# hkust-vgd/scanobjectnn

Hardware: AMD Instinct MI355X
Metric: point-clouds/sec fwd+bwd at B×2048×3, 15-cls (higher is better)
Workload: dtype f32

## Files before the change

### include/pcops.h

```cpp
#ifndef PCOPS_H
#define PCOPS_H

#ifdef __cplusplus
extern "C" {
#endif

typedef void *pcops_stream_t;

typedef struct pcops_rows {
    const void *blocks;
    const int *block_start;
    const int *rows;
} pcops_rows_t;

typedef enum pcops_status {
    PCOPS_OK = 0,
    PCOPS_ERR_NULL_POINTER = -1,
    PCOPS_ERR_BAD_SHAPE = -2,
    PCOPS_ERR_BAD_ARGUMENT = -3,
    PCOPS_ERR_UNSUPPORTED = -4,
    PCOPS_ERR_LAUNCH = -5
} pcops_status;

const char *pcops_strerror(int status);
// ... 230 lines not shown
int pcops_cloud_bias_rows(long long rows);
int pcops_cloud_bias_fwd(long long rows, int rows_per_group, int c, const float *Q, const float *Ctr, float *Y,
                         float *stats_partial, const float *stat_pivot, pcops_stream_t stream);
int pcops_cloud_bias_bwd(long long rows, int rows_per_group, int c, const float *G, const float *Y, const float *p, const float *q,
                         const float *t, float *dQ, float *dCtr, float *partial, pcops_stream_t stream);
int pcops_edge_first_rows(void);
int pcops_edge_first_supported(int b, int n, int m, int s, int c);
int pcops_edge_first_moments(int b, int n, int m, int s, const float *xyz, const int *idx, float *moments_partial,
                             float *edge_rows, pcops_stream_t stream);
int pcops_edge_first_wgrad(int b, int n, int m, int s, int c, const float *G, const float *xyz, const int *idx,
                           float *wpartial, pcops_stream_t stream);
int pcops_mlp_bwd_fused_edge_groups(long long M, int K, int N, int S, int gram);
int pcops_mlp_bwd_fused_edge(long long M, int K, int N, const float *Yprev, const float *a_scale, const float *a_shift,
                                  const float *Y, const float *p, const float *q, const float *t, const float *gpool,
                                  const unsigned char *argmax, int S, const float *W, float *partial, float *dW, float *db,
                                  float *stats_partial, const float *edge_rows, float *edge_stats, pcops_stream_t stream);

int pcops_mlp_bwd_fused_gw_groups(long long M, int K, int N, int S);
int pcops_mlp_bwd_fused_gw(long long M, int K, int N, const float *Yprev, const float *a_scale, const float *a_shift,
                           const float *Y, const float *p, const float *q, const float *t, const float *gpool,
                           const unsigned char *argmax, int S, const float *W, const float *bias, float *partial, float *dW,
                           float *db, float *Gprev, float *stats_partial, pcops_stream_t stream);
int pcops_mlp_bwd_fused_edge_gw(long long M, int K, int N, const float *Yprev, const float *a_scale, const float *a_shift,
                                const float *Y, const float *p, const float *q, const float *t, const float *gpool,
                                const unsigned char *argmax, int S, const float *W, const float *bias, float *partial,
                                float *dW, float *db, float *stats_partial, const float *edge_rows, float *edge_stats,
                                pcops_stream_t stream);
int pcops_edge_first_layer_grads(int P1, const float *wpartial, int P2, const float *moments_partial, int c, const float *W,
                                 const float *bias, const float *p, const float *q, const float *t, const float *sumG,
                                 const float *mean, long long rows, float *dW, float *dbias, pcops_stream_t stream);
int pcops_xyz_first_layer_grads(int P1, const float *xyz_stats, int P2, const float *moments, int C,
                                const float *Wxyz, const float *bias, const float *p, const float *q, const float *t,
                                const float *sumG, const float *mean, long long rows, float *dWxyz, float *dbias,
                                pcops_stream_t stream);

int pcops_adam_step(long long n, float *p, const float *g, float *m, float *v, float beta1, float beta2, float lr_t,
                    float epsilon, pcops_stream_t stream);
int pcops_gather_stack_rows_supported(int b, int n, int m, int s, int has_q, int nlayers, const int *widths);
int pcops_sa_scatter_rows_supported(int n, int m, int s, int c);
unsigned long long pcops_rows_max_blocks(int b, int m, int s);
int pcops_rows_plan(int b, int m, int s, const int *pts_cnt, void *blocks, int *block_start, int *rows,
                    pcops_stream_t stream);
int pcops_mlp_gemm_fwd_rows(int M, int K, int N, const float *X, int ldx, const float *pro_scale,
                            const float *pro_shift, const float *W, const float *bias, float *Y,
                            float *stats_partial, const float *stat_pivot, const pcops_rows_t *rows,
                            pcops_stream_t stream);
int pcops_mlp_gemm_fwd_xyz_rows(int M, int K, int N, const float *off4, const float *xyzw, const float *pro_scale,
                                const float *pro_shift, const float *W, const float *bias, float *Y,
                                float *stats_partial, const float *stat_pivot, const pcops_rows_t *rows,
                                pcops_stream_t stream);
int pcops_mlp_gemm_dgrad_rows(int M, int K, int Nout, const float *G, const float *Y, const float *p,
                              const float *q, const float *t, const float *gpool, const unsigned char *argmax,
                              int S, const float *pool_scale, const float *pool_shift, const float *Wt,
                              const float *Yprev, const float *prev_scale, const float *prev_shift, float *Gprev,
                              float *stats_partial, const pcops_rows_t *rows, pcops_stream_t stream);
int pcops_mlp_gemm_dgrad_xyz_rows(int M, int K, int Nout, const float *G, const float *Y, const float *p,
                                  const float *q, const float *t, const float *gpool, const unsigned char *argmax,
                                  int S, const float *pool_scale, const float *pool_shift, const float *Wt,
                                  const float *off4, const float *xyzw, const float *prev_scale,
                                  const float *prev_shift, float *Gprev, float *stats_partial, float *xyz_stats,
                                  const pcops_rows_t *rows, pcops_stream_t stream);
int pcops_mlp_wgrad_rows(long long M, int K, int N, const float *X, int ldx, const float *a_scale,
                         const float *a_shift, const float *G, const float *Y, const float *p, const float *q,
                         const float *t, const float *gpool, const unsigned char *argmax, int S,
                         const float *pool_scale, const float *pool_shift, float *partial, float *dW, float *db,
                         const pcops_rows_t *rows, pcops_stream_t stream);
int pcops_mlp_wgrad_xyz_rows(long long M, int K, int N, const float *off4, const float *xyzw, const float *a_scale,
                             const float *a_shift, const float *G, const float *Y, const float *p, const float *q,
                             const float *t, const float *gpool, const unsigned char *argmax, int S,
                             const float *pool_scale, const float *pool_shift, float *partial, float *dW, float *db,
                             const pcops_rows_t *rows, pcops_stream_t stream);
int pcops_mlp_gemm_fwd_pool_rows_supported(int M, int K, int N);
int pcops_mlp_gemm_fwd_pool_rows(int M, int K, int N, const float *X, int ldx, const float *pro_scale,
                                 const float *pro_shift, const float *W, const float *bias, const float *gamma,
                                 float *Y, float *stats_partial, const float *stat_pivot, float *ypart,
                                 unsigned char *ppart, const pcops_rows_t *rows, pcops_stream_t stream);
int pcops_mlp_pool_combine_rows(long long G, int C, const float *ypart, const unsigned char *ppart,
                                const float *gamma, const float *scale, const float *shift,
                                const pcops_rows_t *rows, float *out, unsigned char *argmax, float *ysel,
                                pcops_stream_t stream);
int pcops_mlp_bn_relu_maxpool_rows(long long G, int C, const float *Y, const float *scale, const float *shift,
                                   const pcops_rows_t *rows, float *out, unsigned char *argmax, float *ysel,
                                   pcops_stream_t stream);
int pcops_sa_gather_fwd_rows(int b, int n, int m, int s, int c, const float *Q, const float *Ctr, const float *xyz,
                             const float *new_xyz, const float *Wxyz, const float *bias, const int *idx, float *Y,
                             float *off4, float *stats_partial, const float *stat_pivot, float *moments,
                             const pcops_rows_t *rows, pcops_stream_t stream);
int pcops_sa_scatter_bwd_rows(int b, int n, int m, int s, int c, const float *G, const float *Y, const float *p,
                              const float *q, const float *t, const float *gpool, const unsigned char *argmax,
                              const float *pool_scale, const float *pool_shift, const int *idx, const float *xyz,
                              const float *new_xyz, float *dQ, float *dCtr, float *wpartial, float *dWxyz,
                              float *dbias, const float *fwd_Q, const float *fwd_Ctr, const float *fwd_Wxyz,
                              const float *fwd_bias, void *workspace, const pcops_rows_t *rows,
                              pcops_stream_t stream);

int pcops_edge_ld_supported(int b, int n, int m, int s, int c);
int pcops_edge_pool_fwd_ld(int b, int n, int m, int s, int c, const float *Q, int ldq, const float *Ctr, int ldc,
                           const int *idx, const float *gamma, float *SQ, float *qsel, unsigned char *arg,
                           float *stats_partial, const float *stat_pivot, pcops_stream_t stream);
int pcops_edge_pool_out_ld(long long groups, int c, const float *qsel, const float *Ctr, int ldc, const float *scale,
                           const float *shift, float *out, float *ysel, pcops_stream_t stream);
int pcops_edge_pool_out_ld2(long long groups, int c, const float *qsel, const float *Ctr, int ldc, const float *scale,
                            const float *shift, float *out, float *ysel, float *out2, int ld2, pcops_stream_t stream);
int pcops_edge_pool_bwd_ld(int b, int n, int m, int s, int c, const float *Q, int ldq, const float *Ctr, int ldc,
                           const int *idx, const float *gpool, const float *ysel, const float *SQ,
                           const unsigned char *arg, const float *scale, const float *shift, const float *p,
                           const float *q, const float *t, float *dQ, int lddq, float *dCtr, int lddc, void *workspace,
                           pcops_stream_t stream);
int pcops_sa_gather_fwd_ld(int b, int n, int m, int s, int c, const float *Q, int ldq, const float *Ctr, int ldc,
                           const int *idx, float *Y, float *stats_partial, const float *stat_pivot,
                           pcops_stream_t stream);
int pcops_sa_scatter_bwd_ld(int b, int n, int m, int s, int c, const float *G, const float *p, const float *q,
                            const float *t, const int *idx, const float *Q, int ldq, const float *Ctr, int ldc,
                            float *dQ, int lddq, float *dCtr, int lddc, void *workspace, pcops_stream_t stream);

int pcops_edge_weights_fwd(int c, int cp, int kp, const float *W1, const float *b1, float *Wcat, float *bcat,
                           pcops_stream_t stream);
int pcops_edge_weights_bwd(int c, int cp, const float *dWcat, const float *dbcat, float *dW1, float *db1,
                           pcops_stream_t stream);

int pcops_fc_bn_fwd(int R, int C, const float *x, const float *gamma, const float *beta, float *moving_mean,
                    float *moving_var, int training, float decay, float eps, int unbiased_moving_var, int relu,
                    float *y, float *save_mean, float *save_rstd, pcops_stream_t stream);
int pcops_fc_bn_bwd(int R, int C, const float *dy, const float *x, const float *y, const float *gamma,
                    const float *save_mean, const float *save_rstd, int training, int relu, float *dx,
                    float *dgamma, float *dbeta, pcops_stream_t stream);

int pcops_softmax_ce_blocks(int R);
int pcops_softmax_ce(int R, int C, const float *logits, const int *labels, float label_smoothing, float *loss,
                     float *dlogits, pcops_stream_t stream);
int pcops_three_nn_weights(int b, int n, const float *dist, float *weight, pcops_stream_t stream);

int pcops_transform3_fwd(int b, int n, const float *x, const float *T, float *out, pcops_stream_t stream);
int pcops_transform3_bwd(int b, int n, const float *x, const float *T, const float *grad_out, float *dT, float *dx,
                         pcops_stream_t stream);

int pcops_spider_taylor_fwd(long long rows, int t, const float *delta, const float *theta, const float *tbias, float *g,
                            pcops_stream_t stream);
unsigned long long pcops_spider_taylor_bwd_workspace_bytes(long long rows, int t);
int pcops_spider_taylor_bwd(long long rows, int t, const float *delta, const float *dg, float *dtheta, float *dtbias,
                            void *workspace, pcops_stream_t stream);
int pcops_spider_conv_fwd(int b, int n, int c, int k, int t, int o, const float *feat, const int *idx, const float *g,
                          const float *w, const float *bias, float *y, pcops_stream_t stream);
unsigned long long pcops_spider_conv_wgrad_workspace_bytes(int b, int n, int c, int k, int t, int o);
int pcops_spider_conv_wgrad(int b, int n, int c, int k, int t, int o, const float *feat, const int *idx, const float *g,
                            const float *dy, float *dw, float *dbias, void *workspace, pcops_stream_t stream);
int pcops_spider_conv_dgrad(int b, int n, int c, int k, int t, int o, const float *feat, const int *idx, const float *g,
                            const float *w, const float *dy, float *dfeat_grouped, float *dg, pcops_stream_t stream);

unsigned long long pcops_group_norm_relu_workspace_bytes(int b, int c);
int pcops_group_norm_relu_fwd(int b, int n, int c, int groups, float eps, const float *x, const float *gamma,
                              const float *beta, float *y, float *mean, float *rstd, pcops_stream_t stream);
int pcops_group_norm_relu_bwd(int b, int n, int c, int groups, const float *dout, const float *x, const float *y,
                              const float *gamma, const float *mean, const float *rstd, float *dx, float *dgamma,
                              float *dbeta, void *workspace, pcops_stream_t stream);

#ifdef __cplusplus
}
#endif
#endif
```

### scanobjectnn_amd/_lib.py

```python
import ctypes as C
import os
import weakref

import torch

_HERE = os.path.dirname(os.path.abspath(__file__))
LIB_PATH = os.environ.get("PCOPS_LIB") or os.path.join(_HERE, "libpcops.so")

_I, _F, _P, _U64, _LL = C.c_int, C.c_float, C.c_void_p, C.c_ulonglong, C.c_longlong
ABI_VERSION = 4

SIGNATURES = {
    "pcops_farthest_point_sample": ([_I, _I, _I, _P, _P, _P], True),
    "pcops_prob_sample": ([_I, _I, _I, _P, _P, _P, _P], True),
    "pcops_gather_point": ([_I, _I, _I, _P, _P, _P], True),
    "pcops_gather_point_grad": ([_I, _I, _I, _P, _P, _P], True),
    "pcops_query_ball_point": ([_I, _I, _I, _F, _I, _P, _P, _P, _P], True),
    "pcops_query_ball_point_multi": ([_I, _I, _I, _I, _P, _P, _P, _P, _P, _P], True),
    "pcops_group_point": ([_I, _I, _I, _I, _I, _P, _P, _P], True),
    "pcops_group_point_grad": ([_I, _I, _I, _I, _I, _P, _P, _P], True),
    "pcops_selection_sort": ([_I, _I, _I, _I, _P, _P, _P], True),
    "pcops_three_nn": ([_I, _I, _I, _P, _P, _P, _P], True),
    "pcops_three_interpolate": ([_I, _I, _I, _I, _P, _P, _P, _P], True),
    "pcops_three_interpolate_grad": ([_I, _I, _I, _I, _P, _P, _P, _P], True),
    "pcops_pairwise_distance": ([_I, _I, _I, _P, _P], True),
    "pcops_knn_topk": ([_I, _I, _I, _P, _P], True),
    "pcops_knn_graph": ([_I, _I, _I, _I, _P, _P], True),
    "pcops_knn_graph_seeded": ([_I, _I, _I, _I, _P, _P, _P], True),
    "pcops_edge_feature": ([_I, _I, _I, _I, _P, _P, _P], True),
    "pcops_edge_feature_grad": ([_I, _I, _I, _I, _P, _P, _P], True),
    "pcops_mlp_gemm_fwd": ([_I, _I, _I, _P, _I, _P, _P, _P, _P, _P, _P, _P], True),
    "pcops_mlp_bn_finalize": ([_I, _I, _LL, _P, _P, _P, _P, _P, _F, _F, _I, _P, _P, _P, _P, _P, _P], True),
    "pcops_mlp_bn_eval_coeffs": ([_I, _P, _P, _P, _P, _F, _P, _P], True),
    "pcops_mlp_bn_relu_maxpool": ([_LL, _I, _I, _P, _P, _P, _P, _P, _P], True),
    "pcops_mlp_gemm_fwd_pool": ([_I, _I, _I, _I, _P, _I, _P, _P, _P, _P, _P, _P, _P, _P, _P, _P], True),
    "pcops_mlp_pool_select": ([_LL, _I, _P, _P, _P, _P], True),
    "pcops_mlp_bn_relu_apply": ([_LL, _I, _P, _P, _P, _P], True),
    "pcops_mlp_relu_mask_stats": ([_LL, _I, _P, _P, _P, _P, _P, _P], True),
    "pcops_mlp_pool_bwd_stats": ([_LL, _I, _P, _P, _P, _P, _P, _P], True),
    "pcops_mlp_pool_bwd_stats_sum": ([_LL, _I, _P, _LL, _P, _LL, _P, _P, _P, _P, _P], True),
    "pcops_mlp_bn_bwd_coeffs": ([_I, _I, _LL, _P, _P, _P, _P, _P, _P, _P, _P, _P, _P], True),
    "pcops_mlp_gemm_dgrad": ([_I, _I, _I, _P, _P, _P, _P, _P, _P, _P, _I, _P, _P, _P, _P, _P, _P, _P, _P], True),
    "pcops_mlp_wgrad": ([_LL, _I, _I, _P, _I, _P, _P, _P, _P, _P, _P, _P, _P, _P, _I, _P, _P, _P, _P, _P], True),
    "pcops_mlp_transpose": ([_I, _I, _P, _P], True),
    "pcops_small_gemm": ([_I, _I, _I, _P, _I, _P, _I, _P, _I], True),
    "pcops_small_gemm_ex": ([_I, _I, _I, _P, _I, _I, _P, _I, _I, _P, _P, _I], True),
    "pcops_mlp_dy_apply": ([_LL, _I] + [_P] * 6, True),
    "pcops_small_gemm_colsum": ([_I, _I, _I, _P, _I, _I, _P, _I, _I, _P, _P, _I, _P], True),
    "pcops_small_gemm_pair": ([_P], True),
    "pcops_mlp_pool_top_prep": ([_I, _I] + [_P] * 8, True),
    "pcops_mlp_pool_top_finish": ([_I, _I, _LL] + [_P] * 10, True),
    "pcops_mlp_pool_top_addend": ([_I, _I, _I, _I] + [_P] * 9, True),
    "pcops_mlp_gemm_dgrad_top": ([_I, _I] + [_P] * 6 + [_LL] + [_P] * 3, True),
    "pcops_mlp_gram": ([_LL, _I, _P, _I, _P, _P, _P, _P, _P], True),
    "pcops_mlp_pool_top_wsparse": ([_I, _I, _I, _I] + [_P] * 11, True),
    "pcops_sa_gather_fwd": ([_I, _I, _I, _I, _I, _P, _P, _P, _P, _P, _P, _P, _P, _P, _P, _P, _P], True),
    "pcops_mlp_gemm_fwd_xyz": ([_I, _I, _I, _P, _P, _P, _P, _P, _P, _P, _P, _P], True),
    "pcops_mlp_gemm_dgrad_xyz": ([_I, _I, _I, _P, _P, _P, _P, _P, _P, _P, _I, _P, _P, _P, _P, _P, _P, _P, _P, _P, _P], True),
    "pcops_mlp_wgrad_xyz": ([_LL, _I, _I, _P, _P, _P, _P, _P, _P, _P, _P, _P, _P, _P, _I, _P, _P, _P, _P, _P], True),
    "pcops_edge_pool_fwd": ([_I, _I, _I, _I, _I, _P, _P, _P, _P, _P, _P, _P, _P, _P], True),
    "pcops_edge_pool_out": ([_LL, _I, _P, _P, _P, _P, _P, _P], True),
    "pcops_edge_pool_bwd": ([_I, _I, _I, _I, _I] + [_P] * 15, True),
    "pcops_xyz_first_layer_grads": ([_I, _P, _I, _P, _I, _P, _P, _P, _P, _P, _P, _P, _LL, _P, _P], True),
    "pcops_cloud_bias_fwd": ([_LL, _I, _I, _P, _P, _P, _P, _P], True),
    "pcops_cloud_bias_bwd": ([_LL, _I, _I, _P, _P, _P, _P, _P, _P, _P, _P], True),
    "pcops_edge_first_moments": ([_I, _I, _I, _I, _P, _P, _P, _P], True),
    "pcops_mlp_bwd_fused_edge": ([_LL, _I, _I, _P, _P, _P, _P, _P, _P, _P, _P, _P, _I, _P, _P, _P, _P, _P, _P, _P], True),
    "pcops_edge_first_wgrad": ([_I, _I, _I, _I, _I, _P, _P, _P, _P], True),
    "pcops_edge_first_layer_grads": ([_I, _P, _I, _P, _I, _P, _P, _P, _P, _P, _P, _P, _LL, _P, _P], True),
    "pcops_sa_scatter_bwd": ([_I, _I, _I, _I, _I] + [_P] * 22, True),
    "pcops_rows_plan": ([_I, _I, _I, _P, _P, _P, _P], True),
    "pcops_mlp_gemm_fwd_rows": ([_I, _I, _I, _P, _I, _P, _P, _P, _P, _P, _P, _P, _P], True),
    "pcops_mlp_gemm_fwd_xyz_rows": ([_I, _I, _I, _P, _P, _P, _P, _P, _P, _P, _P, _P, _P], True),
    "pcops_mlp_gemm_dgrad_rows": ([_I, _I, _I, _P, _P, _P, _P, _P, _P, _P, _I, _P, _P, _P, _P, _P, _P, _P, _P, _P], True),
    "pcops_mlp_gemm_dgrad_xyz_rows": ([_I, _I, _I, _P, _P, _P, _P, _P, _P, _P, _I, _P, _P, _P, _P, _P, _P, _P, _P, _P, _P, _P], True),
    "pcops_mlp_bwd_fused": ([_LL, _I, _I, _P, _P, _P, _P, _P, _P, _P, _P, _P, _P, _I, _P, _P, _P, _P, _P, _P], True),
    "pcops_mlp_bwd_fused_rows": ([_LL, _I, _I, _P, _P, _P, _P, _P, _P, _P, _P, _P, _P, _I, _P, _P, _P, _P, _P, _P, _P], True),
    "pcops_adam_step": ([_LL, _P, _P, _P, _P, _F, _F, _F, _F], True),
    "pcops_mlp_bwd_fused_gw": ([_LL, _I, _I] + [_P] * 9 + [_I] + [_P] * 7, True),
    "pcops_mlp_bwd_fused_edge_gw": ([_LL, _I, _I] + [_P] * 9 + [_I] + [_P] * 8, True),
    "pcops_mlp_bwd_fused_xyz_rows": ([_LL, _I, _I, _P, _P, _P, _P, _P, _P, _P, _P, _P, _P, _P, _I, _P, _P, _P, _P, _P, _P, _P], True),
    "pcops_mlp_wgrad_rows": ([_LL, _I, _I, _P, _I, _P, _P, _P, _P, _P, _P, _P, _P, _P, _I, _P, _P, _P, _P, _P, _P], True),
    "pcops_mlp_wgrad_xyz_rows": ([_LL, _I, _I, _P, _P, _P, _P, _P, _P, _P, _P, _P, _P, _P, _I, _P, _P, _P, _P, _P, _P], True),
    "pcops_mlp_bn_relu_maxpool_rows": ([_LL, _I, _P, _P, _P, _P, _P, _P, _P], True),
    "pcops_mlp_gemm_fwd_pool_rows": ([_I, _I, _I, _P, _I, _P, _P, _P, _P, _P, _P, _P, _P, _P, _P, _P], True),
    "pcops_mlp_pool_combine_rows": ([_LL, _I, _P, _P, _P, _P, _P, _P, _P, _P, _P], True),
    "pcops_sa_gather_fwd_rows": ([_I, _I, _I, _I, _I, _P, _P, _P, _P, _P, _P, _P, _P, _P, _P, _P, _P, _P], True),
    "pcops_sa_scatter_bwd_rows": ([_I, _I, _I, _I, _I] + [_P] * 23, True),
    "pcops_knn_point": ([_I, _I, _I, _I, _I, _P, _P, _P, _P], True),
    "pcops_knn_point_dist": ([_I, _I, _I, _I, _P, _P, _P], True),
    "pcops_scatter_rows_sorted": ([_I, _I, _I, _I, _I, _I, _P, _P, _P, _P, _I, _P], True),
    "pcops_edge_feature_grad_central": ([_I, _I, _I, _I, _P, _P], True),
    "pcops_edge_pool_fwd_ld": ([_I, _I, _I, _I, _I, _P, _I, _P, _I, _P, _P, _P, _P, _P, _P, _P], True),
    "pcops_edge_pool_out_ld": ([_LL, _I, _P, _P, _I, _P, _P, _P, _P], True),
    "pcops_edge_pool_out_ld2": ([_LL, _I, _P, _P, _I, _P, _P, _P, _P, _P, _I], True),
    "pcops_edge_pool_bwd_ld": ([_I, _I, _I, _I, _I, _P, _I, _P, _I] + [_P] * 10 + [_P, _I, _P, _I, _P], True),
    "pcops_sa_gather_fwd_ld": ([_I, _I, _I, _I, _I, _P, _I, _P, _I, _P, _P, _P, _P], True),
    "pcops_sa_scatter_bwd_ld": ([_I, _I, _I, _I, _I, _P, _P, _P, _P, _P, _P, _I, _P, _I, _P, _I, _P, _I, _P], True),
    "pcops_edge_weights_fwd": ([_I, _I, _I, _P, _P, _P, _P], True),
    "pcops_edge_weights_bwd": ([_I, _I, _P, _P, _P, _P], True),
    "pcops_transform3_fwd": ([_I, _I, _P, _P, _P], True),
    "pcops_transform3_bwd": ([_I, _I, _P, _P, _P, _P, _P], True),
    "pcops_fc_bn_fwd": ([_I, _I, _P, _P, _P, _P, _P, _I, _F, _F, _I, _I, _P, _P, _P], True),
    "pcops_fc_bn_bwd": ([_I, _I, _P, _P, _P, _P, _P, _P, _I, _I, _P, _P, _P], True),
    "pcops_softmax_ce": ([_I, _I, _P, _P, _F, _P, _P], True),
    "pcops_three_nn_weights": ([_I, _I, _P, _P], True),
    "pcops_spider_taylor_fwd": ([_LL, _I, _P, _P, _P, _P], True),
    "pcops_spider_taylor_bwd": ([_LL, _I, _P, _P, _P, _P, _P], True),
    "pcops_spider_conv_fwd": ([_I] * 6 + [_P] * 6, True),
    "pcops_spider_conv_wgrad": ([_I] * 6 + [_P] * 7, True),
    "pcops_spider_conv_dgrad": ([_I] * 6 + [_P] * 7, True),
    "pcops_group_norm_relu_fwd": ([_I, _I, _I, _I, _F] + [_P] * 6, True),
    "pcops_group_norm_relu_bwd": ([_I, _I, _I, _I] + [_P] * 10, True),
}
PLAIN = {
    "pcops_strerror": ([_I], C.c_char_p),
    "pcops_abi_version": ([], _I),
    "pcops_softmax_ce_blocks": ([_I], _I),
    "pcops_farthest_point_sample_workspace_bytes": ([_I, _I], _U64),
    "pcops_mlp_stats_rows": ([_I], _I),
    "pcops_mlp_reduce_workspace_bytes": ([_I], _U64),
    "pcops_mlp_gemm_fwd_pool_supported": ([_I, _I, _I, _I], _I),
    "pcops_mlp_xyz_supported": ([_I, _I, _I], _I),
    "pcops_mlp_bwd_stats_rows": ([_LL], _I),
    "pcops_mlp_bwd_pool_stats_rows": ([_LL], _I),
    "pcops_mlp_wgrad_splits": ([_LL, _I, _I], _I),
    "pcops_mlp_bwd_fused_groups": ([_LL, _I, _I, _I, _I], _I),
    "pcops_mlp_bwd_fused_gw_groups": ([_LL, _I, _I, _I], _I),
    "pcops_mlp_bwd_fused_edge_groups": ([_LL, _I, _I, _I, _I], _I),
    "pcops_gather_stack_rows_supported": ([_I, _I, _I, _I, _I, _I, _P], _I),
    "pcops_sa_scatter_rows_supported": ([_I, _I, _I, _I], _I),
    "pcops_sa_gather_stats_rows": ([_LL], _I),
    "pcops_sa_gather_fwd_stats_rows": ([_I] * 9, _I),
    "pcops_sa_scatter_rows": ([_I, _I], _I),
    "pcops_edge_pool_stats_rows": ([_LL], _I),
    "pcops_edge_pool_fwd_stats_rows": ([_I] * 5, _I),
    "pcops_edge_ld_supported": ([_I] * 5, _I),
    "pcops_edge_first_rows": ([], _I),
    "pcops_cloud_bias_supported": ([_LL, _I, _I], _I),
    "pcops_cloud_bias_rows": ([_LL], _I),
    "pcops_edge_first_supported": ([_I] * 5, _I),
    "pcops_sa_scatter_workspace_bytes": ([_I, _I, _I, _I], _U64),
    "pcops_rows_max_blocks": ([_I, _I, _I], _U64),
    "pcops_mlp_gemm_fwd_pool_rows_supported": ([_I, _I, _I], _I),
    "pcops_scatter_rows_workspace_bytes": ([_I, _I, _I], _U64),
    "pcops_knn_point_supported": ([_I], _I),
    "pcops_scatter_rows_sorted_max_ndst": ([], _I),
    "pcops_scatter_rows_sorted_supported": ([_I, _I], _I),
    "pcops_mlp_pool_top_supported": ([_I, _I, _I, _I], _I),
    "pcops_knn_graph_path": ([_I, _I, _I, _I, _P], _I),
    "pcops_last_launch_pipe": ([], _I),
    "pcops_last_launch_plan": ([_P, _I], _I),
    "pcops_set_option": ([_I, _I], _I),
    "pcops_get_option": ([_I], _I),
    "pcops_set_deterministic": ([_I], None),
    "pcops_get_deterministic": ([], _I),
    "pcops_spider_taylor_bwd_workspace_bytes": ([_LL, _I], _U64),
    "pcops_spider_conv_wgrad_workspace_bytes": ([_I] * 6, _U64),
    "pcops_group_norm_relu_workspace_bytes": ([_I, _I], _U64),
}


class GemmProblem(C.Structure):
    _fields_ = [("M", C.c_int), ("K", C.c_int), ("N", C.c_int), ("A", C.c_void_p), ("lda", C.c_int), ("transA", C.c_int),
                ("B", C.c_void_p), ("ldb", C.c_int), ("transB", C.c_int), ("bias", C.c_void_p), ("C", C.c_void_p),
                ("ldc", C.c_int), ("colsum", C.c_void_p)]


def small_gemm_pair(p0, p1):
    arr = (GemmProblem * 2)(GemmProblem(*p0), GemmProblem(*p1))
    lib = load()
    stream = torch.cuda.current_stream().cuda_stream
    shape = tuple(int(v) for v in p0[:3]) + tuple(int(v) for v in p1[:3])
    for h in _hooks:
        h("pcops_small_gemm_pair", "pre", shape)
    status = lib.pcops_small_gemm_pair(arr, stream)
    for h in _hooks:
        h("pcops_small_gemm_pair", "post", shape)
    if status != 0:
        raise PcopsError("pcops_small_gemm_pair failed: %s (status %d)" % (strerror(status), status))


class RowsT(C.Structure):
    _fields_ = [("blocks", C.c_void_p), ("block_start", C.c_void_p), ("rows", C.c_void_p)]


class Rows:
    by_struct = weakref.WeakValueDictionary()

    def __init__(self, pts_cnt, nsample):
        b, m = pts_cnt.shape
        lib = load()
        nb = int(lib.pcops_rows_max_blocks(b, m, int(nsample)))
        dev = pts_cnt.device
        self.blocks = torch.empty((nb, 4), dtype=torch.int32, device=dev)
        self.block_start = torch.empty(b * m + 1, dtype=torch.int32, device=dev)
        self.rows = torch.empty(1, dtype=torch.int32, device=dev)
        call("pcops_rows_plan", b, m, int(nsample), pts_cnt.data_ptr(), self.blocks.data_ptr(),
             self.block_start.data_ptr(), self.rows.data_ptr())
        self.struct = RowsT(self.blocks.data_ptr(), self.block_start.data_ptr(), self.rows.data_ptr())
        self.full_rows = b * m * int(nsample)
        Rows.by_struct[id(self.struct)] = self

    def num_rows(self):
        return int(self.rows.item())

    @property
    def ref(self):
        return C.byref(self.struct)


_lib = None


class PcopsError(RuntimeError):
    pass


def load():
    global _lib
    if _lib is not None:
        return _lib
    if not os.path.exists(LIB_PATH):
        raise PcopsError(
            "libpcops.so is missing (%s). Build it with `python -c 'import __graft_entry__ as g; "
            "g.build()'` or `make -C scanobjectnn_amd/csrc`. There is no CPU fallback." % LIB_PATH)
    lib = C.CDLL(LIB_PATH)
    for name, (argtypes, _) in SIGNATURES.items():
        fn = getattr(lib, name)
        fn.argtypes = list(argtypes) + [_P]
        fn.restype = _I
    for name, (argtypes, restype) in PLAIN.items():
# ... 99 lines not shown
```

### scanobjectnn_amd/csrc/mlp.hip

```cpp
#include <stdlib.h>

#include "common.h"
#include <type_traits>

#ifndef PCOPS_MLP_PART
#define PCOPS_MLP_PART (-1)
#endif
#define PCOPS_PART(p_) (PCOPS_MLP_PART < 0 || PCOPS_MLP_PART == (p_))
#define PCOPS_HIDDEN __attribute__((visibility("hidden")))

#ifndef PCOPS_BF_RM
#define PCOPS_BF_RM 1
#endif

namespace pcops_mlp {

typedef float f32x16 __attribute__((ext_vector_type(16)));
typedef float f32x4 __attribute__((ext_vector_type(4)));
typedef __bf16 bf16x8 __attribute__((ext_vector_type(8)));

typedef __bf16 bf16x2 __attribute__((ext_vector_type(2)));
typedef float f32x2 __attribute__((ext_vector_type(2)));
__device__ __forceinline__ void split3_pair(float a, float b, bf16x2 &h, bf16x2 &m, bf16x2 &l) {
    const f32x2 v = {a, b};
// ... 960 lines not shown
#pragma unroll 1
            for (int it = 0; it < nit; it += 2) {
                a1 = *reinterpret_cast<const float4 *>(arow + 8 * (it + 1));
#pragma unroll
                for (int nt = 0; nt < NT; ++nt) b1[nt] = bq[(2 * (it + 1)) * BN + 32 * nt];
                mfma16(a0, b0);
                const int nx = it + 2 < nit ? it + 2 : it + 1;
                a0 = *reinterpret_cast<const float4 *>(arow + 8 * nx);
#pragma unroll
                for (int nt = 0; nt < NT; ++nt) b0[nt] = bq[(2 * nx) * BN + 32 * nt];
                mfma16(a1, b1);
            }
            __builtin_amdgcn_fence(__ATOMIC_ACQUIRE, "wavefront");
            }
#ifdef PCOPS_PHASE_PROF
            {
                float sink_ = acc[NT - 1][15];
                asm volatile("" ::"v"(sink_));
                const unsigned long long n_ = PROF_T(); pf_mfma += n_ - pf_t; pf_t = n_;
            }
#endif
            }
            if (WST) {
                wstore((wt + 1) & 1);
                __syncthreads();
                ++wt;
            }
        }
        if (active) {
        if constexpr (BF3) {
#pragma unroll
            for (int i = 0; i < NT; ++i) acc[i] += sm[i];
        }
        if (POOL) pool_acc(acc, tile, sub, st);
        const long long row0 = tile * 32;
        const int erem = (int)((long long)M - row0 < 32 ? (long long)M - row0 : 32);
        const __amdgpu_buffer_rsrc_t rout = make_rsrc(a.Y + row0 * a.ldy, ((long long)M - row0) * a.ldy * 4);
        const bool ynt = a.nt_out != 0;
        const __amdgpu_buffer_rsrc_t rprev =
            make_rsrc(((EM == E_MASK || EM == E_MASKA) ? a.Yprev : a.Y) + row0 * a.ldy, ((long long)M - row0) * a.ldy * 4);
        auto epilogue = [&](auto full_) {
        constexpr bool FULL = decltype(full_)::value;
#pragma unroll
        for (int h = 0; h < EH; ++h) {
            const int ocq = h * BNH + ocl;
            const bool ocin = FULL || (n0 + ocq < N);
            const unsigned yvoff = ocin ? (unsigned)((lane / O4) * a.ldy + n0 + ocq) * 4u : kOOB;
            float4 py[is_mask(EM) ? NST : 1];
            float4 po[(EM == E_MASKX) ? NST : 1];
            if (EM == E_MASKX) {
                const __amdgpu_buffer_rsrc_t ro = make_rsrc(a.off4 + row0 * 4, ((long long)M - row0) * 16);
                const float4 xw0 = *reinterpret_cast<const float4 *>(&ecoef[2 * BN + ocq]);
                const float4 xw1 = *reinterpret_cast<const float4 *>(&ecoef[3 * BN + ocq]);
                const float4 xw2 = *reinterpret_cast<const float4 *>(&ecoef[4 * BN + ocq]);
                const float4 xb = *reinterpret_cast<const float4 *>(&ecoef[5 * BN + ocq]);
#pragma unroll
                for (int j = 0; j < NST; ++j) {
                    const float4 o = buf_load4(ro, (unsigned)(lane / O4) * 16u, (unsigned)j * (64 / O4) * 16u);
                    po[j] = o;
                    py[j] = make_float4(xyz_y(o, xw0.x, xw1.x, xw2.x, xb.x), xyz_y(o, xw0.y, xw1.y, xw2.y, xb.y),
                                        xyz_y(o, xw0.z, xw1.z, xw2.z, xb.z), xyz_y(o, xw0.w, xw1.w, xw2.w, xb.w));
                }
            }
            if (EM == E_MASK || EM == E_MASKA) {
#pragma unroll
                for (int j = 0; j < NST; ++j) py[j] = buf_load4(rprev, yvoff, (unsigned)j * yrowstep);
            }
            float4 pad[has_add(EM) ? NST : 1];
            if (has_add(EM)) {
                const __amdgpu_buffer_rsrc_t radd = make_rsrc(a.addend, a.add_bytes);
#pragma unroll
                for (int j = 0; j < NST; ++j) {
                    const int rr = (lane + 64 * j) / O4;
                    const int slot = (FULL || rr < erem) ? a.rowmap[row0 + rr] : -1;
                    const unsigned off = (slot >= 0 && ocin) ? ((unsigned)slot * (unsigned)a.add_ld + (unsigned)(n0 + ocq)) * 4u : kOOB;
                    pad[j] = buf_load4(radd, off, 0u);
                }
            }
            const float4 eb = *reinterpret_cast<const float4 *>(&ecoef[ocq]);
            const float4 em = *reinterpret_cast<const float4 *>(&ecoef[BN + ocq]);
            const float4 epv = EM == E_FWD ? *reinterpret_cast<const float4 *>(&ecoef[2 * BN + ocq])
                                           : make_float4(0.f, 0.f, 0.f, 0.f);
            float ew[2] = {1.f, 1.f};
            if (EM == E_FWD && compact) {
                const int nblk = (M + kBlk - 1) / kBlk;
#pragma unroll
                for (int hb = 0; hb < 2; ++hb) {
                    long long bi = tile * 2 + hb;
                    bi = bi < nblk ? bi : nblk - 1;
                    const RowBlock rb = uniform_block(a.blocks, bi);
                    ew[hb] = rb.w;
                }
            }
            __builtin_amdgcn_wave_barrier();
#pragma unroll
            for (int nt = 0; nt < NTH; ++nt)
#pragma unroll
                for (int v = 0; v < 16; ++v)
                    Aw[((v & 3) + 8 * (v >> 2) + 4 * (lane >> 5)) * LDW + 32 * nt + (lane & 31)] = acc[h * NTH + nt][v];
            __builtin_amdgcn_fence(__ATOMIC_RELEASE, "wavefront");
            __builtin_amdgcn_wave_barrier();
#pragma unroll
            for (int j = 0; j < NST; ++j) {
                if (FULL && j % 2 == 0) __builtin_amdgcn_sched_barrier(0);
                const int r = (lane + 64 * j) / O4;
                float4 o = *reinterpret_cast<const float4 *>(&Aw[r * LDW + ocl]);
                if (FULL || (r < erem && ocin)) {
                    if (EM == E_FWD) {
                        if (compact && j % (O4 / 4) == 0) {
                            const float w = lane < O4 ? ew[j / (O4 / 4)] : 1.f;
                            const float4 wo = make_float4(w * o.x, w * o.y, w * o.z, w * o.w);
                            s1[h][0] += wo.x; s1[h][1] += wo.y; s1[h][2] += wo.z; s1[h][3] += wo.w;
                            s2[h][0] = fmaf(wo.x, o.x, s2[h][0]); s2[h][1] = fmaf(wo.y, o.y, s2[h][1]);
                            s2[h][2] = fmaf(wo.z, o.z, s2[h][2]); s2[h][3] = fmaf(wo.w, o.w, s2[h][3]);
                        } else {
                        s1[h][0] += o.x; s1[h][1] += o.y; s1[h][2] += o.z; s1[h][3] += o.w;
                        s2[h][0] = fmaf(o.x, o.x, s2[h][0]); s2[h][1] = fmaf(o.y, o.y, s2[h][1]);
                        s2[h][2] = fmaf(o.z, o.z, s2[h][2]); s2[h][3] = fmaf(o.w, o.w, s2[h][3]);
                        }
                        if (POOL) {
                            o.x = fmaf(o.x, em.x, epv.x); o.y = fmaf(o.y, em.y, epv.y);
                            o.z = fmaf(o.z, em.z, epv.z); o.w = fmaf(o.w, em.w, epv.w);
                        } else {
                            o.x += epv.x; o.y += epv.y; o.z += epv.z; o.w += epv.w;
                        }
                    } else if (EM == E_PLAINA) {
                        const float4 vc = *reinterpret_cast<const float4 *>(&ecoef[2 * BN + ocq]);
                        o.x += pad[j].x + vc.x; o.y += pad[j].y + vc.y; o.z += pad[j].z + vc.z; o.w += pad[j].w + vc.w;
                    } else if (is_mask(EM)) {
                        const float4 yp = py[j];
                        if (EM == E_MASKA) {
                            const float4 vc = *reinterpret_cast<const float4 *>(&ecoef[2 * BN + ocq]);
                            o.x += pad[j].x + vc.x; o.y += pad[j].y + vc.y; o.z += pad[j].z + vc.z; o.w += pad[j].w + vc.w;
                        }
                        o.x = fmaf(yp.x, eb.x, em.x) > 0.f ? o.x : 0.f;
                        o.y = fmaf(yp.y, eb.y, em.y) > 0.f ? o.y : 0.f;
                        o.z = fmaf(yp.z, eb.z, em.z) > 0.f ? o.z : 0.f;
                        o.w = fmaf(yp.w, eb.w, em.w) > 0.f ? o.w : 0.f;
                        s1[h][0] += o.x; s1[h][1] += o.y; s1[h][2] += o.z; s1[h][3] += o.w;
                        s2[h][0] = fmaf(o.x, yp.x, s2[h][0]); s2[h][1] = fmaf(o.y, yp.y, s2[h][1]);
                        s2[h][2] = fmaf(o.z, yp.z, s2[h][2]); s2[h][3] = fmaf(o.w, yp.w, s2[h][3]);
                        if (EM == E_MASKX) {
                            const float4 of = po[j];
                            const float ov[4] = {o.x, o.y, o.z, o.w};
#pragma unroll
                            for (int e = 0; e < 4; ++e) {
                                sx[h][0][e] = fmaf(of.x, ov[e], sx[h][0][e]);
                                sx[h][1][e] = fmaf(of.y, ov[e], sx[h][1][e]);
                                sx[h][2][e] = fmaf(of.z, ov[e], sx[h][2][e]);
                            }
                        }
                    }
                }
                if ((EM != E_MASKX && !(EM == E_FWD && POOL)) || a.Y)
                    buf_store4(rout, yvoff, (unsigned)j * yrowstep, o, ynt);
            }
            __builtin_amdgcn_fence(__ATOMIC_ACQUIRE, "wavefront");
        }
        };
        if (EM != E_MASKX && erem == 32 && n0 + BN <= N) epilogue(std::true_type{});
        else epilogue(std::false_type{});
        }
#ifdef PCOPS_PHASE_PROF
        if (active) { const unsigned long long n_ = PROF_T(); pf_epi += n_ - pf_t; ++pf_tiles; }
#endif
        st = nst;
        sub = nsub;
        ++round;
    }
#ifdef PCOPS_PHASE_PROF
    if (lane == 0) {
        atomicAdd(&g_phase_prof[0], pf_stage);
        atomicAdd(&g_phase_prof[1], pf_mfma);
        atomicAdd(&g_phase_prof[2], pf_epi);
        atomicAdd(&g_phase_prof[3], PROF_T() - pf_start);
        atomicAdd(&g_phase_prof[4], pf_tiles);
        atomicAdd(&g_phase_prof[5], 1ull);
    }
#endif

    if (EM != E_PLAIN && EM != E_PLAINA && a.stats) {
#pragma unroll
        for (int h = 0; h < EH; ++h) {
#pragma unroll
            for (int e = 0; e < 4; ++e) {
#pragma unroll
                for (int off = 32; off >= O4; off >>= 1) {
                    s1[h][e] += __shfl_xor(s1[h][e], off, 64);
                    s2[h][e] += __shfl_xor(s2[h][e], off, 64);
                }
            }
            if (lane < O4) {
#pragma unroll
                for (int e = 0; e < 4; ++e) {
                    red[(wave * 2 + 0) * BN + h * BNH + ocl + e] = POOL ? s1[h][e] * ecoef[BN + h * BNH + ocl + e] : s1[h][e];
                    red[(wave * 2 + 1) * BN + h * BNH + ocl + e] = s2[h][e];
                }
            }
        }
        __syncthreads();
        for (int i = tid; i < 2 * BN; i += NTHR) {
            const int which = i / BN, c = i % BN;
            if (n0 + c < N) {
                float v = 0.f;
#pragma unroll
                for (int w = 0; w < WAVES; ++w) v += red[(w * 2 + which) * BN + c];
                a.stats[((long long)rowgrp * 2 + which) * N + n0 + c] = v;
            }
        }
    }
    if (EM == E_MASKX && a.xstats) {
#pragma unroll
        for (int i = 0; i < 3; ++i) {
            __syncthreads();
#pragma unroll
            for (int h = 0; h < EH; ++h) {
// ... 2318 lines not shown
        } else if constexpr (DW3) {
#pragma unroll
            for (int y = 0; y < TN; ++y) {
                const int sn = (cn * TN + y) * 32 + li, nn = 4 * (sn % D4) + sn / D4;
#pragma unroll
                for (int v = 0; v < 16; ++v) {
                    const int sk = ck * 32 + (v & 3) + 8 * (v >> 2) + 4 * half, kk = 4 * (sk % A4) + sk / A4;
                    if (kk < K && nn < N) out[(long long)kk * N + nn] = accw[y][v] + smw[y][v];
                }
            }
        } else {
#pragma unroll
        for (int y = 0; y < TN; ++y) {
            const int nn = (cn * TN + y) * 32 + li;
#pragma unroll
            for (int v = 0; v < 16; ++v) {
                const int kk = ck * 32 + (v & 3) + 8 * (v >> 2) + 4 * half;
                if (kk < K && nn < N) out[(long long)kk * N + nn] = accw[y][v];
            }
        }
        }
#pragma unroll
        for (int b = 0; b < 2; ++b) {
            s1[b] += __shfl_xor(s1[b], 16, 64); s1[b] += __shfl_xor(s1[b], 32, 64);
            s2[b] += __shfl_xor(s2[b], 16, 64); s2[b] += __shfl_xor(s2[b], 32, 64);
        }
#pragma unroll
        for (int b = 0; b < (NX ? 2 : 1); ++b)
#pragma unroll
            for (int i = 0; i < NX; ++i) {
                sx[b][i] += __shfl_xor(sx[b][i], 16, 64);
                sx[b][i] += __shfl_xor(sx[b][i], 32, 64);
            }
        __syncthreads();
        constexpr int NSR = 2 + (NX > 3 ? NX : 3);
        float *sst = buf + 256 * 4;
        if (lane < 16) {
#pragma unroll
            for (int b = 0; b < 2; ++b) {
                sst[(rh * NSR + 0) * KB + 32 * cbp + 16 * b + c16] = s1[b];
                sst[(rh * NSR + 1) * KB + 32 * cbp + 16 * b + c16] = s2[b];
                if (NX) {
#pragma unroll
                    for (int i = 0; i < NX; ++i) sst[(rh * NSR + 2 + i) * KB + 32 * cbp + 16 * b + c16] = sx[b][i];
                }
            }
        }
        if (a.dbpart) {
            const float *sdb = buf;
            for (int c = tid; c < NB; c += 256) {
                const int quad = c >> 2, e = c & 3;
                float sum = 0.f;
                for (int r = quad; r < 256; r += D4) sum += sdb[r * 4 + e];
                if (c < N) a.dbpart[(long long)grp * N + c] = sum;
            }
        }
        if constexpr (GW) {
            const float *sxs = buf + 2048;
            for (int c = tid; c < KB; c += 256) {
                const int quad = c >> 2, e = c & 3;
                float sum = 0.f;
                for (int r = quad; r < 256; r += A4) sum += sxs[r * 4 + e];
                if (c < K) a.xsum_part[(long long)grp * K + c] = sum;
            }
        }
        __syncthreads();
        for (int i = tid; i < (2 + NX) * KB; i += 256) {
            const int which = i / KB, c = i % KB;
            const float v = sst[which * KB + c] + sst[(NSR + which) * KB + c];
            if (c < K) {
                if (which < 2) a.gstats[((long long)grp * 2 + which) * K + c] = v;
                else a.xstats[((long long)grp * NX + which - 2) * K + c] = v;
            }
        }
    }
}

struct GramArgs {
    long long M;
    int K, ldx;
    const float *X, *asc, *ash;
    float *part;
    float *xpart;
};

constexpr int gram_blocks(int nbk) { return nbk * (nbk + 1) / 2; }
constexpr int gram_row_of(int u, int nbk) {
    int i = 0, left = u;
    while (left >= nbk - i) { left -= nbk - i; ++i; }
    return i;
}
constexpr int gram_col_of(int u, int nbk) {
    int i = 0, left = u;
    while (left >= nbk - i) { left -= nbk - i; ++i; }
    return i + left;
}

template <int U, int NBK>
struct GramBlk {
    static constexpr int i = gram_row_of(U, NBK), j = gram_col_of(U, NBK);
};
template <int NBK, int U0, typename AccT, int... B>
__device__ __forceinline__ void gram_mfma_step(AccT &acc, const float (&f)[NBK], std::integer_sequence<int, B...>) {
    ((acc[B] = __builtin_amdgcn_mfma_f32_32x32x2f32(f[GramBlk<U0 + B, NBK>::i], f[GramBlk<U0 + B, NBK>::j], acc[B], 0, 0, 0)), ...);
}
template <int NBK, int U0, typename AccT, int... B>
__device__ __forceinline__ void gram_store(const AccT &acc, float *out, int K, int half, int li,
                                           std::integer_sequence<int, B...>) {
    auto one = [&](auto b_) {
        constexpr int b = decltype(b_)::value;
        constexpr int bi = GramBlk<U0 + b, NBK>::i, bj = GramBlk<U0 + b, NBK>::j;
        const int nn = 32 * bj + li;
#pragma unroll
        for (int v = 0; v < 16; ++v) {
            const int kk = 32 * bi + (v & 3) + 8 * (v >> 2) + 4 * half;
            if (kk < K && nn < K) out[(long long)kk * K + nn] = acc[b][v];
        }
    };
    (one(std::integral_constant<int, B>{}), ...);
}

template <int NBK, bool BNRELU>
__global__ __launch_bounds__(512, 1) void gram_full_kernel(GramArgs a) {
    constexpr int KP = 32 * NBK, RS = 32, LD = KP + 4;
    constexpr int NU = gram_blocks(NBK), PER = (NU + 3) / 4;
    constexpr int K4 = KP / 4, NV = RS * K4 / 256;
    extern __shared__ __attribute__((aligned(16))) float lds[];
    const int tid = threadIdx.x, lane = tid & 63;
    const int wave = __builtin_amdgcn_readfirstlane(tid >> 6);
    const int K = a.K;
    const long long M = a.M;
    const int grp = blockIdx.x, ngrp = gridDim.x;
    float *coef = lds;
    float *buf = coef + 2 * KP;
    for (int e = tid; e < KP; e += 512) {
        coef[e] = (BNRELU && e < K) ? a.asc[e] : 0.f;
        coef[KP + e] = (BNRELU && e < K) ? a.ash[e] : 0.f;
    }
    __syncthreads();
    const long long nstripes = (M + RS - 1) / RS;
    const long long cnt = grp < nstripes ? (nstripes - grp + ngrp - 1) / ngrp : 0;

    if (wave >= 4) {
        const int pt = tid - 256;
        float4 px[NV];
        float cs[NV][4];
#pragma unroll
        for (int j = 0; j < NV; ++j) cs[j][0] = cs[j][1] = cs[j][2] = cs[j][3] = 0.f;
        auto issue = [&](long long stripe) {
            const long long row0 = stripe * RS;
            const __amdgpu_buffer_rsrc_t rx = make_rsrc(a.X + row0 * a.ldx, (M - row0) * a.ldx * 4);
#pragma unroll
            for (int j = 0; j < NV; ++j) {
                const int e = pt + 256 * j, r = e / K4, c = (e % K4) * 4;
                px[j] = buf_load4(rx, c < K ? (unsigned)(r * a.ldx + c) * 4u : kOOB, 0u);
            }
        };
        auto stage = [&](long long stripe, float *dst) {
            const long long row0 = stripe * RS;
#pragma unroll
            for (int j = 0; j < NV; ++j) {
                const int e = pt + 256 * j, r = e / K4, c = (e % K4) * 4;
                float4 x = px[j];
                if (BNRELU) {
                    const float4 sc = *reinterpret_cast<const float4 *>(&coef[c]);
                    const float4 sh = *reinterpret_cast<const float4 *>(&coef[KP + c]);
                    x.x = fmaxf(fmaf(x.x, sc.x, sh.x), 0.f); x.y = fmaxf(fmaf(x.y, sc.y, sh.y), 0.f);
                    x.z = fmaxf(fmaf(x.z, sc.z, sh.z), 0.f); x.w = fmaxf(fmaf(x.w, sc.w, sh.w), 0.f);
                    if (!(c < K && row0 + r < M)) x = make_float4(0.f, 0.f, 0.f, 0.f);
                }
                cs[j][0] += x.x; cs[j][1] += x.y; cs[j][2] += x.z; cs[j][3] += x.w;
                *reinterpret_cast<float4 *>(&dst[r * LD + c]) = x;
            }
        };
        if (cnt > 0) {
            issue(grp);
            stage(grp, buf);
            if (cnt > 1) issue(grp + ngrp);
        }
        __syncthreads();
        for (long long i = 0; i < cnt; ++i) {
            if (i + 1 < cnt) {
                stage(grp + (i + 1) * ngrp, buf + ((i + 1) & 1) * RS * LD);
                if (i + 2 < cnt) issue(grp + (i + 2) * ngrp);
            }
            __syncthreads();
        }
        float *scr = buf;
#pragma unroll
        for (int j = 0; j < NV; ++j)
            *reinterpret_cast<float4 *>(&scr[(pt + 256 * j) * 4]) = make_float4(cs[j][0], cs[j][1], cs[j][2], cs[j][3]);
        __syncthreads();
        for (int e = pt; e < K; e += 256) {
            float sum = 0.f;
            for (int idx = e >> 2; idx < 256 * NV; idx += K4) sum += scr[idx * 4 + (e & 3)];
            a.xpart[(long long)grp * K + e] = sum;
        }
        __syncthreads();
    } else {
        const int half = lane >> 5, li = lane & 31;
        auto run = [&](auto wv_) {
            constexpr int WV = decltype(wv_)::value;
            constexpr int U0 = WV * PER, U1 = (U0 + PER < NU) ? U0 + PER : NU;
            constexpr int NB_ = U1 > U0 ? U1 - U0 : 0;
            f32x16 acc[NB_ > 0 ? NB_ : 1];
#pragma unroll
            for (int b = 0; b < NB_; ++b)
#pragma unroll
                for (int v = 0; v < 16; ++v) acc[b][v] = 0.f;
            __syncthreads();
            for (long long i = 0; i < cnt; ++i) {
                const float *sb = buf + (i & 1) * RS * LD + half * LD + li;
                float fn[NBK];
#pragma unroll
                for (int c = 0; c < NBK; ++c) fn[c] = sb[32 * c];
#pragma unroll
                for (int it = 0; it < RS / 2; ++it) {
                    float f[NBK];
#pragma unroll
                    for (int c = 0; c < NBK; ++c) f[c] = fn[c];
                    if (it + 1 < RS / 2) {
#pragma unroll
                        for (int c = 0; c < NBK; ++c) fn[c] = sb[2 * (it + 1) * LD + 32 * c];
                    }
                    __builtin_amdgcn_sched_barrier(0);
                    gram_mfma_step<NBK, U0>(acc, f, std::make_integer_sequence<int, NB_>{});
                    __builtin_amdgcn_sched_barrier(0);
                }
                __syncthreads();
            }
            gram_store<NBK, U0>(acc, a.part + (long long)grp * K * K, K, half, li, std::make_integer_sequence<int, NB_>{});
            __syncthreads();
            __syncthreads();
        };
        if (wave == 0) run(std::integral_constant<int, 0>{});
        else if (wave == 1) run(std::integral_constant<int, 1>{});
        else if (wave == 2) run(std::integral_constant<int, 2>{});
        else run(std::integral_constant<int, 3>{});
    }
}

static __global__ __launch_bounds__(256) void mirror_lower_kernel(int K, float *__restrict__ g) {
    const int i = blockIdx.x, tid = threadIdx.x;
    for (int j = tid; j < i; j += 256) g[(long long)i * K + j] = g[(long long)j * K + i];
}

static bool gram_full_on() {
    static const bool on = [] {
        const char *e = getenv("PCOPS_GRAM_FULL");
        return !(e && e[0] == '0');
    }();
    return on;
}

// ... 488 lines not shown
            const int k = (i * 16 + q) * 4;
            if (i < kq && k < Kp) *reinterpret_cast<float4 *>(dst + k) = acc[i];
        }
    }
}

__global__ __launch_bounds__(256) void pool_top_wsparse_kernel(long long G, int S, int C, int Kp,
                                                               const float *__restrict__ gout,
                                                               const float *__restrict__ ysel,
                                                               const unsigned char *__restrict__ arg,
                                                               const float *__restrict__ sc, const float *__restrict__ sh,
                                                               const float *__restrict__ p,
                                                               const float *__restrict__ Yprev,
                                                               const float *__restrict__ psc, const float *__restrict__ psh,
                                                               float *__restrict__ Ssp, float *__restrict__ cfsum) {
    constexpr int KR = 8, U = 8;
    __shared__ float red[4][64 * KR + 1];
    const int lane = threadIdx.x & 63, wave = threadIdx.x >> 6;
    const int c = blockIdx.x;
    const float scc = sc[c], shc = sh[c], pc = p[c];
    const int kr = (Kp + 63) / 64;
    float asc[KR], ash[KR], acc[KR];
#pragma unroll
    for (int i = 0; i < KR; ++i) {
        const int k = lane + 64 * i;
        asc[i] = (k < Kp && psc) ? psc[k] : 1.f;
        ash[i] = (k < Kp && psc) ? psh[k] : 0.f;
        acc[i] = 0.f;
    }
    float csum = 0.f;
    const long long gq = (G + 3) / 4;
    const long long gend = (wave + 1) * gq < G ? (wave + 1) * gq : G;
    for (long long g0 = wave * gq; g0 < gend; g0 += 64) {
        const long long g = g0 + lane;
        float cf = 0.f;
        int row = 0;
        if (g < gend) {
            const long long e = g * C + c;
            cf = fmaf(ysel[e], scc, shc) > 0.f ? pc * gout[e] : 0.f;
            row = arg[e];
        }
        unsigned long long hits = __ballot(cf != 0.f);
        while (hits) {
            float w[U];
            long long r[U];
#pragma unroll
            for (int u = 0; u < U; ++u) {
                w[u] = 0.f;
                r[u] = 0;
                if (hits) {
                    const int l = __builtin_ctzll(hits);
                    hits &= hits - 1;
                    w[u] = __builtin_bit_cast(float, __builtin_amdgcn_readlane(__builtin_bit_cast(int, cf), l));
                    r[u] = (g0 + l) * S + __builtin_amdgcn_readlane(row, l);
                }
            }
#pragma unroll
            for (int i = 0; i < KR; ++i) {
                if (i >= kr) break;
                const int k = lane + 64 * i;
                float x[U];
#pragma unroll
                for (int u = 0; u < U; ++u) x[u] = (k < Kp) ? Yprev[r[u] * Kp + k] : 0.f;
#pragma unroll
                for (int u = 0; u < U; ++u) {
                    const float xv = psc ? fmaxf(fmaf(x[u], asc[i], ash[i]), 0.f) : x[u];
                    acc[i] = fmaf(w[u], xv, acc[i]);
                }
            }
#pragma unroll
            for (int u = 0; u < U; ++u) csum += w[u];
        }
    }
#pragma unroll
    for (int i = 0; i < KR; ++i) red[wave][lane + 64 * i] = acc[i];
    if (lane == 0) red[wave][64 * KR] = csum;
    __syncthreads();
    for (int k = threadIdx.x; k < Kp; k += 256)
        Ssp[(long long)k * C + c] = (red[0][k] + red[1][k]) + (red[2][k] + red[3][k]);
    if (threadIdx.x == 0)
        cfsum[c] = (red[0][64 * KR] + red[1][64 * KR]) + (red[2][64 * KR] + red[3][64 * KR]);
}

__device__ __forceinline__ void small_gemm_tile(int bx, int by, int M, int K, int N, const float *__restrict__ A, int lda,
                                                         const float *__restrict__ B, int ldb, float *__restrict__ C,
                                                         int ldc, int transA, int transB, const float *__restrict__ bias,
                                                         float *__restrict__ colsum) {
    __shared__ float As[4][32][17], Bs[4][16][33], red[4][32][33], cs[4][2][32];
    const int tid = threadIdx.x, lane = tid & 63, wave = tid >> 6;
    const int m0 = by * 32, n0 = bx * 32;
    const int kchunks = (K + 15) / 16;
    f32x16 acc;
#pragma unroll
    for (int v = 0; v < 16; ++v) acc[v] = 0.f;
    float ra[8], rb[8];
    auto fetch = [&](int ch) {
        const int k0 = ch * 16;
#pragma unroll
        for (int i = 0; i < 8; ++i) {
            const int e = lane + 64 * i;
            const int r = e >> 4, kk = e & 15;
            const long long ia = transA ? (long long)(k0 + kk) * lda + m0 + r : (long long)(m0 + r) * lda + k0 + kk;
            ra[i] = (ch < kchunks && m0 + r < M && k0 + kk < K) ? A[ia] : 0.f;
            const int kb = e >> 5, c = e & 31;
            const long long ib = transB ? (long long)(n0 + c) * ldb + k0 + kb : (long long)(k0 + kb) * ldb + n0 + c;
            rb[i] = (ch < kchunks && k0 + kb < K && n0 + c < N) ? B[ib] : 0.f;
        }
    };
    fetch(wave);
    const bool sums = colsum != nullptr && by == 0;
    float bsum = 0.f;
    for (int ch = wave; ch < kchunks; ch += 4) {
        __builtin_amdgcn_wave_barrier();
#pragma unroll
        for (int i = 0; i < 8; ++i) {
            const int e = lane + 64 * i;
            As[wave][e >> 4][e & 15] = ra[i];
            Bs[wave][e >> 5][e & 31] = rb[i];
        }
        if (sums) {
#pragma unroll
            for (int i = 0; i < 8; ++i) bsum += rb[i];
        }
        __builtin_amdgcn_fence(__ATOMIC_RELEASE, "wavefront");
        __builtin_amdgcn_wave_barrier();
        fetch(ch + 4);
#pragma unroll
        for (int st = 0; st < 8; ++st)
            acc = __builtin_amdgcn_mfma_f32_32x32x2f32(As[wave][lane & 31][2 * st + (lane >> 5)],
                                                       Bs[wave][2 * st + (lane >> 5)][lane & 31], acc, 0, 0, 0);
        __builtin_amdgcn_fence(__ATOMIC_ACQUIRE, "wavefront");
    }
#pragma unroll
    for (int v = 0; v < 16; ++v) red[wave][(v & 3) + 8 * (v >> 2) + 4 * (lane >> 5)][lane & 31] = acc[v];
    cs[wave][lane >> 5][lane & 31] = bsum;
    __syncthreads();
    if (sums && tid < 32 && n0 + tid < N)
        colsum[n0 + tid] = ((cs[0][0][tid] + cs[0][1][tid]) + (cs[1][0][tid] + cs[1][1][tid])) +
                           ((cs[2][0][tid] + cs[2][1][tid]) + (cs[3][0][tid] + cs[3][1][tid]));
    for (int e = tid; e < 32 * 32; e += 256) {
        const int r = e >> 5, c = e & 31;
        if (m0 + r < M && n0 + c < N)
            C[(long long)(m0 + r) * ldc + n0 + c] =
                ((red[0][r][c] + red[1][r][c]) + (red[2][r][c] + red[3][r][c])) + (bias ? bias[n0 + c] : 0.f);
    }
}

__global__ __launch_bounds__(256) void small_gemm_kernel(int M, int K, int N, const float *__restrict__ A, int lda,
                                                         const float *__restrict__ B, int ldb, float *__restrict__ C,
                                                         int ldc, int transA, int transB, const float *__restrict__ bias,
                                                         float *__restrict__ colsum) {
    small_gemm_tile(blockIdx.x, blockIdx.y, M, K, N, A, lda, B, ldb, C, ldc, transA, transB, bias, colsum);
}

struct SgProblem {
    int M, K, N, lda, ldb, ldc, transA, transB;
    const float *A, *B, *bias;
    float *C, *colsum;
};
__global__ __launch_bounds__(256) void small_gemm_pair_kernel(SgProblem p0, SgProblem p1, int tiles0, int gx0, int gx1) {
    const bool second = (int)blockIdx.x >= tiles0;
    const int t = second ? (int)blockIdx.x - tiles0 : (int)blockIdx.x, gx = second ? gx1 : gx0;
    small_gemm_tile(t % gx, t / gx, second ? p1.M : p0.M, second ? p1.K : p0.K, second ? p1.N : p0.N, second ? p1.A : p0.A,
                    second ? p1.lda : p0.lda, second ? p1.B : p0.B, second ? p1.ldb : p0.ldb, second ? p1.C : p0.C,
                    second ? p1.ldc : p0.ldc, second ? p1.transA : p0.transA, second ? p1.transB : p0.transB,
                    second ? p1.bias : p0.bias, second ? p1.colsum : p0.colsum);
}

#endif

template <int AM, int EM>
static int launch_gemm_ws_only(GemmArgs &a, hipStream_t st) {
    WsPlan pl;
    if (!(ws_enabled() && ws_plan(a, AM, &pl, ws_kind(EM)))) return PCOPS_ERR_UNSUPPORTED;
    int rc;
    if (AM == A_DYPOOL && a.blocks) rc = launch_gemm_ws<(AM == A_DYPOOL ? A_DYPOOLB : AM), EM>(a, pl, st);
    else if (AM == A_DYPOOL && a.S % 32 == 0) rc = launch_gemm_ws<(AM == A_DYPOOL ? A_DYPOOLU : AM), EM>(a, pl, st);
    else rc = launch_gemm_ws<AM, EM>(a, pl, st);
    return rc;
}

PCOPS_HIDDEN int wgrad_impl(WgradArgs &a, float *partial, float *dW, float *db, hipStream_t st);
PCOPS_HIDDEN int bwd_fused_launch(WgradArgs &a, bool xyz, int groups, float *partial, float *dW, float *db, hipStream_t st,
                                  bool side = false, const float *gw_bias = nullptr);
PCOPS_HIDDEN int gram_full_launch(GramArgs &g, int nbk, bool bnrelu, int gg, size_t lds, hipStream_t st);

static int wgrad_legacy_splits(long long M, int K, int N) {
    const int kb = (K + 63) / 64, nb = (N + 127) / 128;
    long long want = (1024 + (long long)kb * nb - 1) / ((long long)kb * nb);
    if (want < 1) want = 1;
    if (want > 512) want = 512;
    long long rows = (M + want - 1) / want;
    rows = ((rows + 7) / 8) * 8;
    if (rows < 8) rows = 8;
    return (int)((M + rows - 1) / rows);
}

#if PCOPS_PART(4)
int wgrad_impl(WgradArgs &a, float *partial, float *dW, float *db, hipStream_t st) {
    const long long M = a.M;
    const int K = a.K, N = a.N, ldx = a.ldx;
    const float *X = a.X, *G = a.G, *Y = a.Y, *gpool = a.gpool;
    const unsigned char *argmax = a.argmax;
    int splits;
    WsWgradPlan pl;
    PcWgradPlan pc;
    if (a.blocks && !(ws_enabled() && wgrad_pc_enabled() && wgrad_pc_plan(M, K, N, ldx, X, G, Y, gpool, argmax, &pc)))
        return PCOPS_ERR_UNSUPPORTED;
    const bool self = a.dmode == A_SELFD;
    if (self && !(ws_enabled() && wgrad_pc_enabled() && wgrad_pc_plan(M, K, N, ldx, X, G, Y, gpool, argmax, &pc, true)))
        return PCOPS_ERR_UNSUPPORTED;
    Bf3WgradPlan b3;
    pcops_note_pipe(0);
    if (ws_enabled() && wgrad_pc_enabled() && !self && a.amode != A_XYZ &&
        wgrad_bf3_plan(M, K, N, ldx, X, G, Y, gpool, argmax, &b3)) {
        pcops_note_pipe(1);
        pcops_note_plan(4, 1, 128, 0, a.blocks ? 4 : (a.dmode == A_DY ? 0 : (a.S % 32 == 0 ? 1 : 2)));
        splits = b3.groups;
        a.part = partial; a.dbpart = partial + (long long)splits * K * N;
        const dim3 grid(b3.groups, b3.kblocks, b3.nblocks);
        static const bool k96_on = [] { const char *e = getenv("PCOPS_WGRAD_BF3_K96"); return !(e && e[0] == '0'); }();
        const bool k96 = k96_on && K <= 96 && K % 4 == 0;
#define PCOPS_B3_LAUNCH(AM_, DM_)                                                                          \
    do {                                                                                                   \
        auto kern = (k96 && AM_ == A_BNRELU) ? wgrad_bf3_kernel<AM_, DM_, AM_ == A_BNRELU> : wgrad_bf3_kernel<AM_, DM_>;   \
        if (hipFuncSetAttribute(reinterpret_cast<const void *>(kern),                                      \
                                hipFuncAttributeMaxDynamicSharedMemorySize, 160 * 1024) != hipSuccess)     \
            return PCOPS_ERR_LAUNCH;                                                                       \
        hipLaunchKernelGGL(kern, grid, dim3(512), b3.lds, st, a);                                          \
    } while (0)
        if (a.amode == A_BNRELU && a.dmode == A_DY && a.blocks) PCOPS_B3_LAUNCH(A_BNRELU, A_DYW);
        else if (a.amode == A_PLAIN && a.dmode == A_DY && a.blocks) PCOPS_B3_LAUNCH(A_PLAIN, A_DYW);
        else if (a.amode == A_BNRELU && a.dmode != A_DY && a.blocks) PCOPS_B3_LAUNCH(A_BNRELU, A_DYPOOLB);
        else if (a.amode == A_PLAIN && a.dmode != A_DY && a.blocks) PCOPS_B3_LAUNCH(A_PLAIN, A_DYPOOLB);
        else if (a.amode == A_BNRELU && a.dmode == A_DY) PCOPS_B3_LAUNCH(A_BNRELU, A_DY);
        else if (a.amode == A_BNRELU && a.S % 32 == 0) PCOPS_B3_LAUNCH(A_BNRELU, A_DYPOOLU);
        else if (a.amode == A_BNRELU) PCOPS_B3_LAUNCH(A_BNRELU, A_DYPOOL);
        else if (a.dmode == A_DY) PCOPS_B3_LAUNCH(A_PLAIN, A_DY);
        else if (a.S % 32 == 0) PCOPS_B3_LAUNCH(A_PLAIN, A_DYPOOLU);
        else PCOPS_B3_LAUNCH(A_PLAIN, A_DYPOOL);
#undef PCOPS_B3_LAUNCH
    } else if (ws_enabled() && wgrad_pc_enabled() && wgrad_pc_plan(M, K, N, ldx, X, G, Y, gpool, argmax, &pc, self) &&
        (gpool || pc.tn == 4 || a.amode == A_XYZ || a.blocks || self ||
         !wgrad_ws_plan(M, K, N, ldx, X, G, Y, gpool, argmax, &pl))) {
        splits = pc.groups;
        a.part = partial; a.dbpart = partial + (long long)splits * K * N;
        const dim3 grid(pc.groups, pc.kblocks, pc.nblocks);
        pcops_note_plan(5, 0, 64 * pc.tn, 0, a.blocks ? 4 : (a.dmode == A_DY || self ? 0 : (a.S % 32 == 0 ? 1 : 2)));
#define PCOPS_PC_LAUNCH(TK_, TN_, AM_, DM_)                                                                \
    do {                                                                                                   \
        auto kern = wgrad_pc_kernel<TK_, TN_, AM_, DM_, K96_>;                                                \
        if (hipFuncSetAttribute(reinterpret_cast<const void *>(kern),                                      \
                                hipFuncAttributeMaxDynamicSharedMemorySize, 160 * 1024) != hipSuccess)     \
            return PCOPS_ERR_LAUNCH;                                                                       \
        hipLaunchKernelGGL(kern, grid, dim3(512), pc.lds, st, a);                                          \
    } while (0)
#define PCOPS_PC_MODES(TK_, TN_, K96V_)                                                                    \
    do {                                                                                                   \
        constexpr bool K96_ = K96V_;                                                                       \
        if (a.dmode == A_SELFD && a.amode == A_PLAIN) PCOPS_PC_LAUNCH(TK_, TN_, A_PLAIN, A_SELFD);         \
        else if (a.dmode == A_SELFD) PCOPS_PC_LAUNCH(TK_, TN_, A_BNRELU, A_SELFD);                         \
        else if (a.amode == A_XYZ && a.dmode == A_DY && a.blocks) PCOPS_PC_LAUNCH(TK_, TN_, A_XYZ, A_DYW); \
        else if (a.amode == A_BNRELU && a.dmode == A_DY && a.blocks) PCOPS_PC_LAUNCH(TK_, TN_, A_BNRELU, A_DYW); \
        else if (a.amode == A_PLAIN && a.dmode == A_DY && a.blocks) PCOPS_PC_LAUNCH(TK_, TN_, A_PLAIN, A_DYW);   \
        else if (a.amode == A_XYZ && a.dmode == A_DY) PCOPS_PC_LAUNCH(TK_, TN_, A_XYZ, A_DY);              \
        else if (a.amode == A_XYZ && a.blocks) PCOPS_PC_LAUNCH(TK_, TN_, A_XYZ, A_DYPOOLB);                \
        else if (a.amode == A_BNRELU && a.dmode != A_DY && a.blocks) PCOPS_PC_LAUNCH(TK_, TN_, A_BNRELU, A_DYPOOLB); \
        else if (a.amode == A_PLAIN && a.dmode != A_DY && a.blocks) PCOPS_PC_LAUNCH(TK_, TN_, A_PLAIN, A_DYPOOLB);   \
// ... 121 lines not shown
        } else {
            if (u) PCOPS_BFG_LAUNCH(2, A_DYPOOLU, false, false);
            else PCOPS_BFG_LAUNCH(2, A_DYPOOL, false, false);
        }
#undef PCOPS_BFG_LAUNCH
        int rcg = pcops_launch_status();
        if (rcg) return rcg;
        hipLaunchKernelGGL(bwd_fused_gw_finish_kernel, dim3(K, cdiv(N, 128)), dim3(128), 0, st, groups, K, N, a.part,
                           a.dbpart, a.gram_part, a.xsum_part, a.W, gw_bias, a.q, a.t, dW, db);
        return pcops_launch_status();
    }
#define PCOPS_BF_LAUNCH(TN_, DM_, X_)                                                                      \
    do {                                                                                                   \
        auto kern = dw3 ? bwd_fused_dw3_kernel<TN_, DM_, X_>()                                               \
                  : dx3 ? ((TN_ == 2 && nsk) ? bwd_fused_kernel<TN_, DM_, X_, TN_ == 2, true>                  \
                                              : bwd_fused_kernel<TN_, DM_, X_, false, true>)                    \
                        : ((TN_ == 2 && nsk) ? bwd_fused_kernel<TN_, DM_, X_, TN_ == 2> : bwd_fused_kernel<TN_, DM_, X_>);                                                      \
        if (hipFuncSetAttribute(reinterpret_cast<const void *>(kern),                                      \
                                hipFuncAttributeMaxDynamicSharedMemorySize, 160 * 1024) != hipSuccess)     \
            return PCOPS_ERR_LAUNCH;                                                                       \
        hipLaunchKernelGGL(kern, dim3(groups), dim3(512), lds, st, a);                                     \
    } while (0)
#define PCOPS_BF_MODES(TN_, X_)                                                                            \
    do {                                                                                                   \
        if (!pooled && a.blocks) PCOPS_BF_LAUNCH(TN_, A_DYW, X_);                                          \
        else if (a.blocks) PCOPS_BF_LAUNCH(TN_, A_DYPOOLB, X_);                                            \
        else if (!pooled) PCOPS_BF_LAUNCH(TN_, A_DY, X_);                                                  \
        else if (a.S % 32 == 0) PCOPS_BF_LAUNCH(TN_, A_DYPOOLU, X_);                                       \
        else PCOPS_BF_LAUNCH(TN_, A_DYPOOL, X_);                                                           \
    } while (0)
    if (side) {
#define PCOPS_BF_SIDE(TN_)                                                                                 \
    do {                                                                                                   \
        auto kern = dw3 ? bwd_fused_dw3_side_kernel<TN_>()                                                 \
                  : dx3 ? bwd_fused_kernel<TN_, A_DYPOOL, false, false, true, true>                        \
                        : bwd_fused_kernel<TN_, A_DYPOOL, false, false, false, true>;                      \
        if (hipFuncSetAttribute(reinterpret_cast<const void *>(kern),                                      \
                                hipFuncAttributeMaxDynamicSharedMemorySize, 160 * 1024) != hipSuccess)     \
            return PCOPS_ERR_LAUNCH;                                                                       \
        hipLaunchKernelGGL(kern, dim3(groups), dim3(512), lds, st, a);                                     \
    } while (0)
        if (tn == 1) PCOPS_BF_SIDE(1);
        else PCOPS_BF_SIDE(2);
#undef PCOPS_BF_SIDE
    } else
    if (tn == 1 && xyz) PCOPS_BF_MODES(1, true);
    else if (tn == 1) PCOPS_BF_MODES(1, false);
    else if (xyz) PCOPS_BF_MODES(2, true);
    else PCOPS_BF_MODES(2, false);
#undef PCOPS_BF_MODES
#undef PCOPS_BF_LAUNCH
    int rc = pcops_launch_status();
    if (rc) return rc;
    const long long L = (long long)K * N;
    hipLaunchKernelGGL(sum_partials2_kernel, dim3(cdiv(L, 64) + (db ? cdiv(N, 64) : 0)), dim3(1024), 0, st, groups, L,
                       partial, dW, (long long)N, a.dbpart, db);
    return pcops_launch_status();
}

int gram_full_launch(GramArgs &g, int nbk, bool bnrelu, int gg, size_t lds, hipStream_t st) {
#define PCOPS_GRAM_LAUNCH(NBK_)                                                                            \
    do {                                                                                                   \
        auto kern = bnrelu ? gram_full_kernel<NBK_, true> : gram_full_kernel<NBK_, false>;               \
        if (hipFuncSetAttribute(reinterpret_cast<const void *>(kern),                                      \
                                hipFuncAttributeMaxDynamicSharedMemorySize, 160 * 1024) != hipSuccess)     \
            return PCOPS_ERR_LAUNCH;                                                                       \
        hipLaunchKernelGGL(kern, dim3(gg), dim3(512), lds, st, g);                                         \
    } while (0)
        switch (nbk) {
            case 1: PCOPS_GRAM_LAUNCH(1); break;
            case 2: PCOPS_GRAM_LAUNCH(2); break;
            case 3: PCOPS_GRAM_LAUNCH(3); break;
            case 4: PCOPS_GRAM_LAUNCH(4); break;
            case 5: PCOPS_GRAM_LAUNCH(5); break;
            case 6: PCOPS_GRAM_LAUNCH(6); break;
            case 7: PCOPS_GRAM_LAUNCH(7); break;
            case 8: PCOPS_GRAM_LAUNCH(8); break;
            case 9: PCOPS_GRAM_LAUNCH(9); break;
            default: PCOPS_GRAM_LAUNCH(10); break;
        }
#undef PCOPS_GRAM_LAUNCH
    return PCOPS_OK;
}
#endif

#if PCOPS_PART(0)
extern "C" {

int pcops_mlp_stats_rows(int M) {
    const int tiles = (M + kBM - 1) / kBM;
    int tpb = 1;
    while (tiles / tpb > 512) tpb *= 2;
    return (tiles + tpb - 1) / tpb;
}

unsigned long long pcops_mlp_reduce_workspace_bytes(int N) {
    return (unsigned long long)kRedSlices * 2 * (unsigned long long)N * sizeof(double);
}

static int rows_ok(const pcops_rows_t *rows) {
    if (!rows) return PCOPS_OK;
    PCOPS_REQUIRE_PTR(rows->blocks); PCOPS_REQUIRE_PTR(rows->block_start); PCOPS_REQUIRE_PTR(rows->rows);
    if (reinterpret_cast<uintptr_t>(rows->blocks) & 15) return PCOPS_ERR_UNSUPPORTED;
    return PCOPS_OK;
}
#define PCOPS_ROWS(args_, rows_)                                                      \
    do {                                                                              \
        const int rrc_ = rows_ok(rows_);                                              \
        if (rrc_) return rrc_;                                                        \
        if (rows_) {                                                                  \
            (args_).blocks = static_cast<const RowBlock *>((rows_)->blocks);          \
            (args_).Mdev = (rows_)->rows;                                             \
        }                                                                             \
    } while (0)

int pcops_mlp_gemm_fwd_rows(int M, int K, int N, const float *X, int ldx, const float *pro_scale,
                            const float *pro_shift, const float *W, const float *bias, float *Y,
                            float *stats_partial, const float *stat_pivot, const pcops_rows_t *rows,
                            pcops_stream_t stream) {
    PCOPS_REQUIRE_SHAPE(M >= 0 && K >= 1 && N >= 1 && ldx >= K);
    if (M == 0) return PCOPS_OK;
    PCOPS_REQUIRE_PTR(X); PCOPS_REQUIRE_PTR(W); PCOPS_REQUIRE_PTR(Y);
    PCOPS_REQUIRE_ARG((pro_scale == nullptr) == (pro_shift == nullptr));
    if (pro_scale) PCOPS_REQUIRE_SHAPE(K % 4 == 0);
    GemmArgs a = {};
    a.M = M; a.K = K; a.N = N; a.X = X; a.ldx = ldx; a.v0 = pro_scale; a.v1 = pro_shift;
    a.W = W; a.bias = bias; a.Y = Y; a.ldy = N; a.stats = stats_partial; a.pivot = stats_partial ? stat_pivot : nullptr;
    PCOPS_ROWS(a, rows);
    if (pro_scale) return launch_gemm<A_BNRELU, E_FWD>(a, as_stream(stream));
    return launch_gemm<A_PLAIN, E_FWD>(a, as_stream(stream));
}

int pcops_mlp_gemm_fwd(int M, int K, int N, const float *X, int ldx, const float *pro_scale,
                       const float *pro_shift, const float *W, const float *bias, float *Y,
                       float *stats_partial, const float *stat_pivot, pcops_stream_t stream) {
    return pcops_mlp_gemm_fwd_rows(M, K, N, X, ldx, pro_scale, pro_shift, W, bias, Y, stats_partial, stat_pivot, nullptr,
                                   stream);
}

static int pool_s4_sub(int S) {
    if (S % 32 == 0 || S % 4 != 0 || S < 8 || S > 255) return 0;
    int l = S;
    while (l % 32 != 0) l += S;
    if (l > 256) return 0;
    const int inv = 65536 / S + 1;
    for (int r = 0; r <= l; ++r)
        if (((r * inv) >> 16) != r / S) return 0;
    return l / 32;
}
static bool pool_s4_enabled() {
    static const bool on = [] { const char *e = getenv("PCOPS_POOL_S4"); return !(e && e[0] == '0'); }();
    return on;
}
static void set_pool_group(GemmArgs &a, int S) {
    const int sub4 = pool_s4_sub(S);
    a.pool_sub = sub4 ? sub4 : S / 32;
    a.pool_s4 = sub4 ? S : 0;
    a.pool_inv = sub4 ? 65536 / S + 1 : 0;
}
static bool fwd_pool_shape_ok(int M, int K, int N, int S) {
    const int sub4 = pool_s4_enabled() ? pool_s4_sub(S) : 0;
    if (sub4) {
        if (M % (32 * sub4) != 0) return false;
    } else if (S < 32 || S > 256 || S % 32 != 0 || M % S != 0) {
        return false;
    }
    GemmArgs a = {};
    a.M = M; a.K = K; a.N = N; a.ldx = K; a.ldy = N;
    set_pool_group(a, S);
    WsPlan pl;
    if (!(ws_enabled() && ws_plan(a, A_BNRELU, &pl, 1))) return false;
    return !sub4 || pl.bf3;
}

int pcops_mlp_gemm_fwd_pool_supported(int M, int K, int N, int S) { return fwd_pool_shape_ok(M, K, N, S) ? 1 : 0; }

int pcops_mlp_gemm_fwd_pool(int M, int K, int N, int S, const float *X, int ldx, const float *pro_scale,
                            const float *pro_shift, const float *W, const float *bias, const float *gamma,
                            float *Y, float *stats_partial, const float *stat_pivot, float *ysel,
                            unsigned char *argsel, pcops_stream_t stream) {
    PCOPS_REQUIRE_SHAPE(M >= 1 && K >= 1 && N >= 1 && ldx >= K && S >= 1);
    PCOPS_REQUIRE_PTR(X); PCOPS_REQUIRE_PTR(W);
    PCOPS_REQUIRE_ARG((pro_scale == nullptr) == (pro_shift == nullptr));
    PCOPS_REQUIRE_PTR(gamma); PCOPS_REQUIRE_PTR(ysel); PCOPS_REQUIRE_PTR(argsel);
    if (!fwd_pool_shape_ok(M, K, N, S) || ldx != K) return PCOPS_ERR_UNSUPPORTED;
    if ((reinterpret_cast<uintptr_t>(ysel) & 15) || (reinterpret_cast<uintptr_t>(argsel) & 3))
        return PCOPS_ERR_UNSUPPORTED;
    GemmArgs a = {};
    a.M = M; a.K = K; a.N = N; a.X = X; a.ldx = ldx; a.v0 = pro_scale; a.v1 = pro_shift;
    a.W = W; a.bias = bias; a.Y = Y; a.ldy = N; a.stats = stats_partial; a.pivot = stats_partial ? stat_pivot : nullptr;
    set_pool_group(a, S);
    a.pgamma = gamma; a.ysel = ysel; a.psel = argsel;
    WsPlan pl;
    if (!ws_plan(a, A_BNRELU, &pl)) return PCOPS_ERR_UNSUPPORTED;
    if (!pro_scale) return launch_gemm<A_PLAIN, E_FWD>(a, as_stream(stream));
    return launch_gemm<A_BNRELU, E_FWD>(a, as_stream(stream));
}

int pcops_mlp_gemm_fwd_pool_rows(int M, int K, int N, const float *X, int ldx, const float *pro_scale,
                                 const float *pro_shift, const float *W, const float *bias, const float *gamma,
                                 float *Y, float *stats_partial, const float *stat_pivot, float *ypart,
                                 unsigned char *ppart, const pcops_rows_t *rows, pcops_stream_t stream) {
    PCOPS_REQUIRE_SHAPE(M >= 1 && K >= 1 && N >= 1 && ldx >= K);
    PCOPS_REQUIRE_PTR(X); PCOPS_REQUIRE_PTR(W); PCOPS_REQUIRE_PTR(Y); PCOPS_REQUIRE_PTR(pro_scale);
    PCOPS_REQUIRE_PTR(pro_shift); PCOPS_REQUIRE_PTR(gamma); PCOPS_REQUIRE_PTR(ypart); PCOPS_REQUIRE_PTR(ppart);
    PCOPS_REQUIRE_PTR(rows);
    if (ldx != K || (reinterpret_cast<uintptr_t>(ypart) & 15) || (reinterpret_cast<uintptr_t>(ppart) & 3))
        return PCOPS_ERR_UNSUPPORTED;
    GemmArgs a = {};
    a.M = M; a.K = K; a.N = N; a.X = X; a.ldx = ldx; a.v0 = pro_scale; a.v1 = pro_shift;
    a.W = W; a.bias = bias; a.Y = Y; a.ldy = N; a.stats = stats_partial; a.pivot = stats_partial ? stat_pivot : nullptr;
    a.pool_sub = 1; a.pgamma = gamma; a.ysel = ypart; a.psel = ppart;
    PCOPS_ROWS(a, rows);
    WsPlan pl;
    if (!(ws_enabled() && ws_plan(a, A_BNRELU, &pl))) return PCOPS_ERR_UNSUPPORTED;
    return launch_gemm<A_BNRELU, E_FWD>(a, as_stream(stream));
}

int pcops_mlp_gemm_fwd_pool_rows_supported(int M, int K, int N) {
    GemmArgs a = {};
    a.M = M; a.K = K; a.N = N; a.ldx = K; a.ldy = N; a.pool_sub = 1;
    WsPlan pl;
    return ws_enabled() && ws_plan(a, A_BNRELU, &pl) ? 1 : 0;
}

int pcops_mlp_pool_combine_rows(long long G, int C, const float *ypart, const unsigned char *ppart,
                                const float *gamma, const float *scale, const float *shift,
                                const pcops_rows_t *rows, float *out, unsigned char *argmax, float *ysel,
                                pcops_stream_t stream) {
    PCOPS_REQUIRE_SHAPE(G >= 0 && C >= 1);
    if (G == 0) return PCOPS_OK;
    PCOPS_REQUIRE_PTR(ypart); PCOPS_REQUIRE_PTR(ppart); PCOPS_REQUIRE_PTR(gamma); PCOPS_REQUIRE_PTR(scale);
    PCOPS_REQUIRE_PTR(shift); PCOPS_REQUIRE_PTR(out); PCOPS_REQUIRE_PTR(rows);
    const int rrc = rows_ok(rows);
    if (rrc) return rrc;
    const long long total = G * C;
    const unsigned grid = cdiv(total, 256) < 16384u ? cdiv(total, 256) : 16384u;
    hipLaunchKernelGGL(pool_combine_rows_kernel, dim3(grid), dim3(256), 0, as_stream(stream), total, C, ypart, ppart,
                       gamma, scale, shift, rows->block_start, out, argmax, ysel);
    return pcops_launch_status();
}

int pcops_mlp_pool_select(long long G, int C, const float *ysel, const float *scale, const float *shift,
                          float *out, pcops_stream_t stream) {
    PCOPS_REQUIRE_SHAPE(G >= 0 && C >= 1);
    if (G == 0) return PCOPS_OK;
    PCOPS_REQUIRE_PTR(ysel); PCOPS_REQUIRE_PTR(scale); PCOPS_REQUIRE_PTR(shift); PCOPS_REQUIRE_PTR(out);
    const long long total = G * C;
    const unsigned grid = cdiv(total, 256) < 16384u ? cdiv(total, 256) : 16384u;
    hipLaunchKernelGGL(pool_select_kernel, dim3(grid), dim3(256), 0, as_stream(stream), total, C, ysel, scale,
                       shift, out);
    return pcops_launch_status();
}

int pcops_mlp_bn_finalize(int P, int N, long long R, const float *stats_partial, const float *stat_pivot,
                          void *workspace, const float *gamma, const float *beta, float eps, float decay,
                          int unbiased_moving_var, float *moving_mean, float *moving_var, float *mean,
                          float *rstd, float *scale, float *shift, pcops_stream_t stream) {
    PCOPS_REQUIRE_SHAPE(P >= 1 && N >= 1 && R >= 1);
    PCOPS_REQUIRE_PTR(stats_partial); PCOPS_REQUIRE_PTR(workspace); PCOPS_REQUIRE_PTR(gamma);
    PCOPS_REQUIRE_PTR(beta); PCOPS_REQUIRE_PTR(mean); PCOPS_REQUIRE_PTR(rstd); PCOPS_REQUIRE_PTR(scale);
    PCOPS_REQUIRE_PTR(shift);
    PCOPS_REQUIRE_ARG((moving_mean == nullptr) == (moving_var == nullptr));
    hipStream_t st = as_stream(stream);
    if (P <= kFusedRows) {
        hipLaunchKernelGGL(bn_finalize_fused_kernel, dim3((N + 31) / 32), dim3(1024), 0, st, P, N, (double)R,
                           stats_partial, stat_pivot, gamma, beta, eps, decay, unbiased_moving_var, moving_mean, moving_var, mean,
                           rstd, scale, shift);
        return pcops_launch_status();
    }
    double *ws = static_cast<double *>(workspace);
    int rc = reduce_stats(P, N, stats_partial, ws, st);
    if (rc) return rc;
    hipLaunchKernelGGL(bn_finalize_kernel, dim3((N + 255) / 256), dim3(256), 0, st, N, (double)R, ws, stat_pivot,
                       gamma, beta, eps, decay, unbiased_moving_var, moving_mean, moving_var, mean, rstd, scale, shift);
    return pcops_launch_status();
}

int pcops_mlp_bn_eval_coeffs(int N, const float *gamma, const float *beta, const float *moving_mean,
                             const float *moving_var, float eps, float *scale, float *shift,
                             pcops_stream_t stream) {
    PCOPS_REQUIRE_SHAPE(N >= 1);
    PCOPS_REQUIRE_PTR(gamma); PCOPS_REQUIRE_PTR(beta); PCOPS_REQUIRE_PTR(moving_mean);
    PCOPS_REQUIRE_PTR(moving_var); PCOPS_REQUIRE_PTR(scale); PCOPS_REQUIRE_PTR(shift);
    hipLaunchKernelGGL(bn_eval_coeffs_kernel, dim3((N + 255) / 256), dim3(256), 0, as_stream(stream), N, gamma,
                       beta, moving_mean, moving_var, eps, scale, shift);
    return pcops_launch_status();
// ... 476 lines not shown
                         const float *t, const float *gpool, const unsigned char *argmax, int S,
                         const float *pool_scale, const float *pool_shift, float *partial, float *dW, float *db,
                         const pcops_rows_t *rows, pcops_stream_t stream) {
    PCOPS_REQUIRE_SHAPE(M >= 1 && K >= 1 && N >= 1 && ldx >= K);
    PCOPS_REQUIRE_PTR(X); PCOPS_REQUIRE_PTR(Y); PCOPS_REQUIRE_PTR(p); PCOPS_REQUIRE_PTR(q); PCOPS_REQUIRE_PTR(t);
    PCOPS_REQUIRE_PTR(partial); PCOPS_REQUIRE_PTR(dW);
    if (!gpool) PCOPS_REQUIRE_PTR(G);
    WgradArgs a = {};
    a.M = M; a.K = K; a.N = N;
    a.amode = a_scale ? A_BNRELU : A_PLAIN; a.X = X; a.ldx = ldx; a.asc = a_scale; a.ash = a_shift;
    a.dmode = gpool ? A_DYPOOL : A_DY; a.G = G; a.Y = Y; a.ldy = N; a.p = p; a.q = q; a.t = t;
    a.dsc = pool_scale; a.dsh = pool_shift; a.gpool = gpool; a.argmax = argmax; a.S = S > 0 ? S : 1;
    PCOPS_ROWS(a, rows);
    return wgrad_impl(a, partial, dW, db, as_stream(stream));
}

int pcops_mlp_wgrad_xyz(long long M, int K, int N, const float *off4, const float *xyzw, const float *a_scale,
                        const float *a_shift, const float *G, const float *Y, const float *p, const float *q,
                        const float *t, const float *gpool, const unsigned char *argmax, int S,
                        const float *pool_scale, const float *pool_shift, float *partial, float *dW, float *db,
                        pcops_stream_t stream) {
    return pcops_mlp_wgrad_xyz_rows(M, K, N, off4, xyzw, a_scale, a_shift, G, Y, p, q, t, gpool, argmax, S, pool_scale,
                                    pool_shift, partial, dW, db, nullptr, stream);
}

int pcops_mlp_wgrad_xyz_rows(long long M, int K, int N, const float *off4, const float *xyzw, const float *a_scale,
                             const float *a_shift, const float *G, const float *Y, const float *p, const float *q,
                             const float *t, const float *gpool, const unsigned char *argmax, int S,
                             const float *pool_scale, const float *pool_shift, float *partial, float *dW, float *db,
                             const pcops_rows_t *rows, pcops_stream_t stream) {
    PCOPS_REQUIRE_SHAPE(M >= 1 && K >= 1 && N >= 1);
    PCOPS_REQUIRE_PTR(off4); PCOPS_REQUIRE_PTR(xyzw); PCOPS_REQUIRE_PTR(a_scale); PCOPS_REQUIRE_PTR(a_shift);
    PCOPS_REQUIRE_PTR(Y); PCOPS_REQUIRE_PTR(p); PCOPS_REQUIRE_PTR(q); PCOPS_REQUIRE_PTR(t);
    PCOPS_REQUIRE_PTR(partial); PCOPS_REQUIRE_PTR(dW);
    if (!gpool) PCOPS_REQUIRE_PTR(G);
    if (reinterpret_cast<uintptr_t>(off4) & 15) return PCOPS_ERR_UNSUPPORTED;
    WgradArgs a = {};
    a.M = M; a.K = K; a.N = N;
    a.amode = A_XYZ; a.X = nullptr; a.ldx = K; a.asc = a_scale; a.ash = a_shift;
    a.off4 = off4; a.xw = xyzw; a.xw_ld = K;
    a.dmode = gpool ? A_DYPOOL : A_DY; a.G = G; a.Y = Y; a.ldy = N; a.p = p; a.q = q; a.t = t;
    a.dsc = pool_scale; a.dsh = pool_shift; a.gpool = gpool; a.argmax = argmax; a.S = S > 0 ? S : 1;
    PCOPS_ROWS(a, rows);
    return wgrad_impl(a, partial, dW, db, as_stream(stream));
}

static bool dgrad_top_plan(int M, int Kp, WsPlan *pl) {
    GemmArgs a = {};
    a.M = M; a.K = Kp; a.N = Kp; a.ldx = Kp; a.ldy = Kp;
    return ws_enabled() && Kp % 64 == 0 && Kp <= 512 && ws_plan(a, A_BNRELU, pl);
}

int pcops_mlp_pool_top_supported(int M, int Kp, int N, int S) {
    WsPlan pl;
    PcWgradPlan pc;
    if (S < 1 || S > 256 || M % S != 0 || N % 4 != 0 || N > 1024) return 0;
    if (!dgrad_top_plan(M, Kp, &pl)) return 0;
    if (!(wgrad_pc_enabled() && wgrad_pc_plan(M, Kp, Kp, Kp, nullptr, nullptr, nullptr, nullptr, nullptr, &pc, true))) return 0;
    const long long slots = (long long)(M / S) * (S < N ? S : N);
    return slots * Kp * 4 < (long long)kOOB ? 1 : 0;
}

int pcops_mlp_pool_top_addend(int M, int Kp, int N, int S, const float *gout, const float *ysel,
                            const unsigned char *argmax, const float *pool_scale, const float *pool_shift,
                            const float *p, const float *Wt, float *addend, int *rowmap, pcops_stream_t stream) {
    PCOPS_REQUIRE_SHAPE(M >= 1 && S >= 1 && S <= 256 && M % S == 0 && Kp % 4 == 0 && N >= 1 && N <= 65535);
    PCOPS_REQUIRE_PTR(gout); PCOPS_REQUIRE_PTR(ysel); PCOPS_REQUIRE_PTR(argmax); PCOPS_REQUIRE_PTR(pool_scale);
    PCOPS_REQUIRE_PTR(pool_shift); PCOPS_REQUIRE_PTR(p); PCOPS_REQUIRE_PTR(Wt); PCOPS_REQUIRE_PTR(addend);
    PCOPS_REQUIRE_PTR(rowmap);
    if (reinterpret_cast<uintptr_t>(Wt) & 15 || reinterpret_cast<uintptr_t>(addend) & 15) return PCOPS_ERR_UNSUPPORTED;
    if (N > 1024 || Kp > 512) return PCOPS_ERR_UNSUPPORTED;
    if (M / S <= 512)
        hipLaunchKernelGGL(pool_top_addend_kernel<1024>, dim3(M / S), dim3(1024), 0, as_stream(stream), S, N, Kp,
                           S < N ? S : N, gout, ysel, argmax, pool_scale, pool_shift, p, Wt, addend, rowmap);
    else
        hipLaunchKernelGGL(pool_top_addend_kernel<256>, dim3(M / S), dim3(256), 0, as_stream(stream), S, N, Kp,
                           S < N ? S : N, gout, ysel, argmax, pool_scale, pool_shift, p, Wt, addend, rowmap);
    return pcops_launch_status();
}

int pcops_mlp_gemm_dgrad_top(int M, int Kp, const float *Yprev, const float *prev_scale, const float *prev_shift,
                             const float *Mq, const float *vconst, const float *addend, long long addend_rows,
                             const int *rowmap, float *Gprev, float *stats_partial, pcops_stream_t stream) {
    PCOPS_REQUIRE_SHAPE(M >= 1 && Kp >= 1);
    PCOPS_REQUIRE_PTR(Yprev); PCOPS_REQUIRE_PTR(Mq);
    PCOPS_REQUIRE_PTR(vconst); PCOPS_REQUIRE_PTR(addend); PCOPS_REQUIRE_PTR(rowmap); PCOPS_REQUIRE_PTR(Gprev);
    PCOPS_REQUIRE_ARG((prev_scale == nullptr) == (prev_shift == nullptr));
    WsPlan pl;
    if (!dgrad_top_plan(M, Kp, &pl)) return PCOPS_ERR_UNSUPPORTED;
    GemmArgs a = {};
    a.M = M; a.K = Kp; a.N = Kp; a.X = Yprev; a.ldx = Kp; a.v0 = prev_scale; a.v1 = prev_shift;
    a.W = Mq; a.Y = Gprev; a.ldy = Kp; a.Yprev = Yprev; a.msc = prev_scale; a.msh = prev_shift;
    a.stats = stats_partial; a.addend = addend; a.rowmap = rowmap; a.add_ld = Kp; a.vconst = vconst;
    a.add_bytes = addend_rows * Kp * 4;
    if (addend_rows < 1 || a.add_bytes >= (long long)kOOB) return PCOPS_ERR_UNSUPPORTED;
    if (!prev_scale) {
        a.stats = nullptr;
        return launch_gemm_ws_only<A_PLAIN, E_PLAINA>(a, as_stream(stream));
    }
    return launch_gemm_ws_only<A_BNRELU, E_MASKA>(a, as_stream(stream));
}

int pcops_mlp_gram(long long M, int Kp, const float *Yprev, int ldx, const float *a_scale, const float *a_shift,
                   float *partial, float *gram, float *xsum, pcops_stream_t stream) {
    PCOPS_REQUIRE_SHAPE(M >= 1 && Kp >= 1 && ldx >= Kp);
    PCOPS_REQUIRE_PTR(Yprev); PCOPS_REQUIRE_PTR(partial); PCOPS_REQUIRE_PTR(gram);
    PCOPS_REQUIRE_ARG((a_scale == nullptr) == (a_shift == nullptr));
    const int gg = gram_full_groups(M, Kp, ldx, Yprev);
    pcops_note_pipe(0);
    if (gg > 0) {
        hipStream_t st = as_stream(stream);
        GramArgs g = {M, Kp, ldx, Yprev, a_scale, a_shift, partial, partial + (long long)gg * Kp * Kp};
        const int nbk = (Kp + 31) / 32;
        const size_t lds = (size_t)(2 * 32 * nbk + 2 * 32 * (32 * nbk + 4)) * sizeof(float);
        {
            const int rcl = gram_full_launch(g, nbk, a_scale != nullptr, gg, lds, st);
            if (rcl) return rcl;
        }
        int rc = pcops_launch_status();
        if (rc) return rc;
        const long long L = (long long)Kp * Kp;
        hipLaunchKernelGGL(sum_partials2_kernel, dim3(cdiv(L, 64) + (xsum ? cdiv(Kp, 64) : 0)), dim3(1024), 0, st, gg, L,
                           partial, gram, (long long)Kp, g.xpart, xsum);
        hipLaunchKernelGGL(mirror_lower_kernel, dim3(Kp), dim3(256), 0, st, Kp, gram);
        return pcops_launch_status();
    }
    WgradArgs a = {};
    a.M = M; a.K = Kp; a.N = Kp;
    a.amode = a_scale ? A_BNRELU : A_PLAIN; a.X = Yprev; a.ldx = ldx; a.asc = a_scale; a.ash = a_shift;
    a.dmode = A_SELFD; a.G = Yprev; a.Y = Yprev; a.ldy = ldx; a.p = a_scale; a.q = a_scale; a.t = a_shift; a.S = 1;
    return wgrad_impl(a, partial, gram, xsum, as_stream(stream));
}

int pcops_mlp_pool_top_wsparse(int M, int Kp, int N, int S, const float *gout, const float *ysel,
                               const unsigned char *argmax, const float *pool_scale, const float *pool_shift,
                               const float *p, const float *Yprev, const float *prev_scale, const float *prev_shift,
                               float *Ssp, float *cfsum, pcops_stream_t stream) {
    PCOPS_REQUIRE_SHAPE(M >= 1 && S >= 1 && S <= 256 && M % S == 0 && Kp >= 1 && Kp <= 512 && N >= 1);
    PCOPS_REQUIRE_PTR(gout); PCOPS_REQUIRE_PTR(ysel); PCOPS_REQUIRE_PTR(argmax); PCOPS_REQUIRE_PTR(pool_scale);
    PCOPS_REQUIRE_PTR(pool_shift); PCOPS_REQUIRE_PTR(p); PCOPS_REQUIRE_PTR(Yprev);
    PCOPS_REQUIRE_ARG((prev_scale == nullptr) == (prev_shift == nullptr));
    PCOPS_REQUIRE_PTR(Ssp); PCOPS_REQUIRE_PTR(cfsum);
    hipLaunchKernelGGL(pool_top_wsparse_kernel, dim3(N), dim3(256), 0, as_stream(stream), (long long)(M / S), S, N,
                       Kp, gout, ysel, argmax, pool_scale, pool_shift, p, Yprev, prev_scale, prev_shift, Ssp, cfsum);
    return pcops_launch_status();
}

int pcops_mlp_dy_apply(long long M, int N, const float *G, const float *Y, const float *p, const float *q, const float *t,
                       float *out, pcops_stream_t stream) {
    PCOPS_REQUIRE_SHAPE(M >= 0 && N >= 4 && N % 4 == 0);
    if (M == 0) return PCOPS_OK;
    PCOPS_REQUIRE_PTR(G); PCOPS_REQUIRE_PTR(Y); PCOPS_REQUIRE_PTR(p); PCOPS_REQUIRE_PTR(q); PCOPS_REQUIRE_PTR(t); PCOPS_REQUIRE_PTR(out);
    PCOPS_REQUIRE_ARG(((uintptr_t)G | (uintptr_t)Y | (uintptr_t)p | (uintptr_t)q | (uintptr_t)t | (uintptr_t)out) % 16 == 0);
    const long long total4 = M * (N / 4);
    const unsigned grid = (unsigned)(cdiv(total4, 256) < 8192 ? cdiv(total4, 256) : 8192);
    hipLaunchKernelGGL(dy_apply_kernel, dim3(grid), dim3(256), 0, as_stream(stream), total4, N / 4,
                       reinterpret_cast<const float4 *>(G), reinterpret_cast<const float4 *>(Y),
                       reinterpret_cast<const float4 *>(p), reinterpret_cast<const float4 *>(q),
                       reinterpret_cast<const float4 *>(t), reinterpret_cast<float4 *>(out));
    return pcops_launch_status();
}

int pcops_mlp_pool_top_prep(int Kp, int N, const float *W, const float *b, const float *q, const float *t, float *Wt,
                            float *Wq, float *u, float *v, pcops_stream_t stream) {
    PCOPS_REQUIRE_SHAPE(Kp >= 1 && N >= 1);
    PCOPS_REQUIRE_PTR(W); PCOPS_REQUIRE_PTR(b); PCOPS_REQUIRE_PTR(q); PCOPS_REQUIRE_PTR(t);
    PCOPS_REQUIRE_PTR(Wt); PCOPS_REQUIRE_PTR(Wq); PCOPS_REQUIRE_PTR(u);
    const int gx = (N + 31) / 32;
    hipLaunchKernelGGL(pool_top_prep_kernel, dim3(gx, (Kp + 31) / 32 + (v ? ((Kp + 7) / 8 + gx - 1) / gx : 0)), dim3(256), 0,
                       as_stream(stream), Kp, N, W, b, q, t, Wt, Wq, u, v);
    return pcops_launch_status();
}

int pcops_mlp_pool_top_finish(int Kp, int N, long long M, float *dW, const float *Ssp, const float *xsum, const float *u,
                              const float *cfsum, const float *q, const float *W, const float *b, const float *t,
                              float *db, pcops_stream_t stream) {
    PCOPS_REQUIRE_SHAPE(Kp >= 1 && N >= 1 && M >= 1);
    PCOPS_REQUIRE_PTR(dW); PCOPS_REQUIRE_PTR(Ssp); PCOPS_REQUIRE_PTR(xsum); PCOPS_REQUIRE_PTR(u); PCOPS_REQUIRE_PTR(cfsum);
    PCOPS_REQUIRE_PTR(q); PCOPS_REQUIRE_PTR(W); PCOPS_REQUIRE_PTR(b); PCOPS_REQUIRE_PTR(t); PCOPS_REQUIRE_PTR(db);
    hipLaunchKernelGGL(pool_top_finish_kernel, dim3((N + 255) / 256, 8 + (Kp + 7) / 8), dim3(256), 0, as_stream(stream), Kp, N,
                       (float)M, dW, Ssp, xsum, u, cfsum, q, W, b, t, db);
    return pcops_launch_status();
}

int pcops_small_gemm(int M, int K, int N, const float *A, int lda, const float *B, int ldb, float *C, int ldc,
                     pcops_stream_t stream) {
    return pcops_small_gemm_ex(M, K, N, A, lda, 0, B, ldb, 0, nullptr, C, ldc, stream);
}

int pcops_small_gemm_ex(int M, int K, int N, const float *A, int lda, int transA, const float *B, int ldb, int transB,
                        const float *bias, float *C, int ldc, pcops_stream_t stream) {
    return pcops_small_gemm_colsum(M, K, N, A, lda, transA, B, ldb, transB, bias, C, ldc, nullptr, stream);
}

int pcops_small_gemm_colsum(int M, int K, int N, const float *A, int lda, int transA, const float *B, int ldb, int transB,
                            const float *bias, float *C, int ldc, float *colsum, pcops_stream_t stream) {
    PCOPS_REQUIRE_SHAPE(M >= 1 && K >= 1 && N >= 1 && lda >= (transA ? M : K) && ldb >= (transB ? K : N) && ldc >= N);
    PCOPS_REQUIRE_PTR(A); PCOPS_REQUIRE_PTR(B); PCOPS_REQUIRE_PTR(C);
    pcops_note_pipe(0);
    hipLaunchKernelGGL(small_gemm_kernel, dim3((N + 31) / 32, (M + 31) / 32), dim3(256), 0, as_stream(stream), M, K, N, A,
                       lda, B, ldb, C, ldc, transA ? 1 : 0, transB ? 1 : 0, bias, colsum);
    return pcops_launch_status();
}

int pcops_small_gemm_pair(const pcops_gemm_problem_t *p, pcops_stream_t stream) {
    PCOPS_REQUIRE_PTR(p);
    SgProblem q[2];
    int tiles[2], gx[2];
    for (int i = 0; i < 2; ++i) {
        const pcops_gemm_problem_t &a = p[i];
        PCOPS_REQUIRE_SHAPE(a.M >= 1 && a.K >= 1 && a.N >= 1 && a.lda >= (a.transA ? a.M : a.K) && a.ldb >= (a.transB ? a.K : a.N) &&
                            a.ldc >= a.N);
        PCOPS_REQUIRE_PTR(a.A); PCOPS_REQUIRE_PTR(a.B); PCOPS_REQUIRE_PTR(a.C);
        q[i] = SgProblem{a.M, a.K, a.N, a.lda, a.ldb, a.ldc, a.transA ? 1 : 0, a.transB ? 1 : 0, a.A, a.B, a.bias, a.C, a.colsum};
        gx[i] = (a.N + 31) / 32;
        tiles[i] = gx[i] * ((a.M + 31) / 32);
    }
    pcops_note_pipe(0);
    hipLaunchKernelGGL(small_gemm_pair_kernel, dim3(tiles[0] + tiles[1]), dim3(256), 0, as_stream(stream), q[0], q[1], tiles[0],
                       gx[0], gx[1]);
    return pcops_launch_status();
}

#ifdef PCOPS_PHASE_PROF
int pcops_debug_phase_prof(unsigned long long *out) {
    if (hipDeviceSynchronize() != hipSuccess) return PCOPS_ERR_LAUNCH;
    if (hipMemcpyFromSymbol(out, HIP_SYMBOL(g_phase_prof), sizeof(unsigned long long) * 8) != hipSuccess) return PCOPS_ERR_LAUNCH;
    unsigned long long z[8] = {0, 0, 0, 0, 0, 0, 0, 0};
    if (hipMemcpyToSymbol(HIP_SYMBOL(g_phase_prof), z, sizeof(z)) != hipSuccess) return PCOPS_ERR_LAUNCH;
    return PCOPS_OK;
// ... 14 lines not shown
```

### scanobjectnn_amd/fused_mlp.py

```python
import os

import torch

from . import _lib
from . import dist as _dist


def _f32(n, dev):
    return torch.empty(n, dtype=torch.float32, device=dev)


class _VecArena:

    def __init__(self, widths, per_width, dev):
        total = sum(((n + 3) // 4 * 4) * per_width for n in widths)
        alloc = torch.empty if all(n % 4 == 0 for n in widths) else torch.zeros
        self.buf = alloc(total, dtype=torch.float32, device=dev)
        self.off = 0

    def take(self, n):
        n4 = (n + 3) // 4 * 4
        v = self.buf[self.off:self.off + n4]
        self.off += n4
        return v
# ... 15 lines not shown
        lib = _lib.load()
        rref = rows.ref if rows is not None else None
        identity = bool(int(pool) & 2)
        qc = bool(int(pool) & 4)
        direct = bool(int(pool) & 8)
        pool = bool(int(pool) & 1)
        gather = idx is not None
        need_grad = any(ctx.needs_input_grad)
        sync = training and _dist.sync_bn_active()
        dev = idx.device if gather else a0.device
        layers = [tensors[6 * i:6 * i + 6] for i in range(L)]
        if gather:
            B, M, _ = idx.shape
            Nsrc = a0.shape[1] if a0 is not None else xyz.shape[1]
            C1 = layers[0][2].shape[0]
            R, K0 = B * M * S, None
            if qc:
                assert ctr is None and rows is None and M == Nsrc and new_xyz is None
                assert direct or (xyz is None and wxyz is None and bias is None)
                assert not direct or (xyz is not None and wxyz is not None and tuple(wxyz.shape) == (6, C1) and L >= 2
                                      and not ctx.needs_input_grad[0])
                assert a0.shape[2] == 2 * C1 and a0.is_contiguous()
        else:
            R, K0 = a0.shape
        Ys, means, rstds, scales, shifts, Ws = [], [], [], [], [], []
        src, ld, sc_prev, sh_prev, K = a0, K0, None, None, K0
        vecs = _VecArena([l[2].shape[0] for l in layers], 4, dev)
        ws = _workspace(max(l[2].shape[0] for l in layers), dev) if training else None
        pooled_raw = pooled_parts = None
        pool_top = False
        virt = (gather and a0 is None and ctr is None and wxyz is not None and (L >= 3 or (L == 2 and not pool))
                and not sync and (training or not need_grad)
                and bool(lib.pcops_mlp_xyz_supported(R, C1, layers[1][0].shape[-1])))
        if rows is not None and gather and a0 is None and not virt:
            rows = rref = None
        off4 = xyzw = mom = None
        if virt:
            off4 = _f32((R, 4), dev)
            mom = _f32((lib.pcops_sa_gather_stats_rows(B * M), 9), dev) if training else None
            xyzw = torch.cat([wxyz.detach(), (bias.detach() if bias is not None
                                              else torch.zeros(C1, dtype=torch.float32, device=dev)).view(1, C1)]).contiguous()
        for li, (w, b, gamma, beta, mm, mv) in enumerate(layers):
            piv = mm.data_ptr() if (training and STAT_PIVOT) else None
            if li == 0 and gather and qc:
                N = C1
                Y = _f32((R, N), dev)
                P = lib.pcops_sa_gather_fwd_stats_rows(B, Nsrc, M, S, N, 1, 1, 0, 0)
                part = _f32((P, 2, N), dev) if training else None
                _lib.call("pcops_sa_gather_fwd_ld", B, Nsrc, M, S, N, a0.data_ptr(), 2 * N, a0.data_ptr() + 4 * N, 2 * N,
                          idx.data_ptr(), Y.data_ptr(), _p(part), piv)
                if direct and need_grad:
                    mom = _f32((lib.pcops_edge_first_rows(), 27), dev)
                    N1 = layers[1][0].shape[-1]
                    if (EDGE_DIRECT_FUSED and BWD_FUSED and L == 2 and pool
                            and lib.pcops_mlp_bwd_fused_edge_groups(R, N, N1, S, 0)):
                        ctx.edge_rows = _f32((R, 8), dev)
                    _lib.call("pcops_edge_first_moments", B, Nsrc, M, S, xyz.data_ptr(), idx.data_ptr(), mom.data_ptr(),
                              _p(getattr(ctx, "edge_rows", None)))
                W2 = None
            elif (li == 0 and gather and identity and CLOUD_BIAS and a0 is not None and ctr is not None and xyz is None
                    and wxyz is None and bias is None and rows is None and M == 1 and Nsrc == S and a0.is_contiguous()
                    and lib.pcops_cloud_bias_supported(R, S, C1)):
                N = C1
                Y = _f32((R, N), dev)
                P = lib.pcops_cloud_bias_rows(R)
                part = _f32((P, 2, N), dev) if training else None
                _lib.call("pcops_cloud_bias_fwd", R, S, N, a0.data_ptr(), ctr.data_ptr(), Y.data_ptr(), _p(part), piv)
                W2 = None
                ctx.cloud_bias = True
            elif li == 0 and gather:
                N = C1
                Y = None if virt else _f32((R, N), dev)
                other = wxyz is not None or bias is not None or off4 is not None
                P = lib.pcops_sa_gather_fwd_stats_rows(B, Nsrc, M, S, N, int(a0 is not None), int(ctr is not None),
                                                        int(other), int(rref is not None))
                part = _f32((P, 2, N), dev) if training else None
                _lib.call("pcops_sa_gather_fwd_rows", B, Nsrc, M, S, N, _p(a0), _p(ctr), _p(xyz), _p(new_xyz),
                          _p(wxyz), _p(bias), idx.data_ptr(), _p(Y), _p(off4), _p(part), piv, _p(mom), rref)
                W2 = None
            else:
                N = w.shape[-1]
                W2 = w.detach().reshape(-1, N)
                assert W2.shape[0] == K and W2.is_contiguous()
                Y = _f32((R, N), dev)
                P = lib.pcops_mlp_stats_rows(R)
                part = _f32((P, 2, N), dev) if training else None
                if li == 1 and virt:
                    _lib.call("pcops_mlp_gemm_fwd_xyz_rows", R, K, N, off4.data_ptr(), xyzw.data_ptr(), sc_prev.data_ptr(),
                              sh_prev.data_ptr(), W2.data_ptr(), b.data_ptr(), Y.data_ptr(), _p(part), piv, rref)
                elif (rows is not None and pool and li == L - 1 and sc_prev is not None and ld == K and FUSE_POOL_ROWS
                        and lib.pcops_mlp_gemm_fwd_pool_rows_supported(R, K, N)):
                    nbk = rows.blocks.shape[0]
                    pooled_parts = (_f32((nbk, N), dev), torch.empty((nbk, N), dtype=torch.uint8, device=dev))
                    _lib.call("pcops_mlp_gemm_fwd_pool_rows", R, K, N, src.data_ptr(), ld, sc_prev.data_ptr(),
                              sh_prev.data_ptr(), W2.data_ptr(), b.data_ptr(), gamma.data_ptr(), Y.data_ptr(),
                              _p(part), piv, pooled_parts[0].data_ptr(), pooled_parts[1].data_ptr(), rref)
                elif rows is not None:
                    _lib.call("pcops_mlp_gemm_fwd_rows", R, K, N, src.data_ptr(), ld, _p(sc_prev), _p(sh_prev),
                              W2.data_ptr(), b.data_ptr(), Y.data_ptr(), _p(part), piv, rref)
                elif (pool and li == L - 1 and ld == K and lib.pcops_mlp_gemm_fwd_pool_supported(R, K, N, S)
                        and (sc_prev is not None or li == 0)):
                    G = R // S
                    pooled_raw = (_f32((G, N), dev), torch.empty((G, N), dtype=torch.uint8, device=dev))
                    pool_top = need_grad and _pool_top_ok(lib, R, K, N, S, li, gather, K0, rows, virt and li == 1,
                                                          b is not None)
                    if not need_grad or pool_top:
                        Y = None
                    _lib.call("pcops_mlp_gemm_fwd_pool", R, K, N, S, src.data_ptr(), ld, _p(sc_prev),
                              _p(sh_prev), W2.data_ptr(), b.data_ptr(), gamma.data_ptr(), _p(Y),
                              _p(part), piv, pooled_raw[0].data_ptr(), pooled_raw[1].data_ptr())
                else:
                    _lib.call("pcops_mlp_gemm_fwd", R, K, N, src.data_ptr(), ld, _p(sc_prev), _p(sh_prev),
                              W2.data_ptr(), b.data_ptr(), Y.data_ptr(), _p(part), piv)
            scale, shift = vecs.take(N), vecs.take(N)
            if training:
                mean, rstd = vecs.take(N), vecs.take(N)
                Pf, Rf, piv_fin = P, R, piv
                if sync:
                    part, Rf = _dist.allreduce_stat_partials(part, R, mm if piv is not None else None)
                    Pf, piv_fin = part.shape[0], None
                _lib.call("pcops_mlp_bn_finalize", Pf, N, Rf, part.data_ptr(), piv_fin, ws.data_ptr(), gamma.data_ptr(),
                          beta.data_ptr(), float(eps), float(decay), int(unbiased), mm.data_ptr(), mv.data_ptr(),
                          mean.data_ptr(), rstd.data_ptr(), scale.data_ptr(), shift.data_ptr())
                means.append(mean)
                rstds.append(rstd)
            else:
                _lib.call("pcops_mlp_bn_eval_coeffs", N, gamma.data_ptr(), beta.data_ptr(), mm.data_ptr(),
                          mv.data_ptr(), float(eps), scale.data_ptr(), shift.data_ptr())
                if need_grad:
                    means.append(mm.detach().clone())
                    rstds.append(torch.rsqrt(mv.detach() + float(eps)))
            Ys.append(Y)
            scales.append(scale)
            shifts.append(shift)
            Ws.append(W2)
            src, ld, sc_prev, sh_prev, K = Y, N, scale, shift, N

        C = K
        argmax = ysel = None
        if pool:
            G = R // S
            out = _f32((G, C), dev)
            if pooled_parts is not None:
                argmax = torch.empty((G, C), dtype=torch.uint8, device=dev)
                ysel = _f32((G, C), dev)
                _lib.call("pcops_mlp_pool_combine_rows", G, C, pooled_parts[0].data_ptr(), pooled_parts[1].data_ptr(),
                          layers[-1][2].data_ptr(), scales[-1].data_ptr(), shifts[-1].data_ptr(), rref,
                          out.data_ptr(), argmax.data_ptr(), ysel.data_ptr())
            elif pooled_raw is not None:
                ysel, argmax = pooled_raw
                _lib.call("pcops_mlp_pool_select", G, C, ysel.data_ptr(), scales[-1].data_ptr(),
                          shifts[-1].data_ptr(), out.data_ptr())
            else:
                argmax = torch.empty((G, C), dtype=torch.uint8, device=dev) if (training or need_grad) else None
                ysel = _f32((G, C), dev) if (training or need_grad) else None
                if rows is not None:
                    _lib.call("pcops_mlp_bn_relu_maxpool_rows", G, C, Ys[-1].data_ptr(), scales[-1].data_ptr(),
                              shifts[-1].data_ptr(), rref, out.data_ptr(), _p(argmax), _p(ysel))
                else:
                    _lib.call("pcops_mlp_bn_relu_maxpool", G, S, C, Ys[-1].data_ptr(), scales[-1].data_ptr(),
                              shifts[-1].data_ptr(), out.data_ptr(), _p(argmax), _p(ysel))
        else:
            out = _f32((R, C), dev)
            _lib.call("pcops_mlp_bn_relu_apply", R, C, Ys[-1].data_ptr(), scales[-1].data_ptr(),
                      shifts[-1].data_ptr(), out.data_ptr())
        if training or need_grad:
            ctx.saved = (a0, ctr, idx, xyz, new_xyz, wxyz, bias, Ys, means, rstds, scales, shifts, Ws,
                         [l[2] for l in layers], argmax, ysel, off4, xyzw, mom)
            ctx.biases = [l[1] for l in layers]
            ctx.meta = (S, pool, L, R, K0, gather, identity, bool(training), bool(sync))
            ctx.qc = qc
            ctx.direct = gather and qc and direct
            ctx.rows = rows
            ctx.pool_top = pool_top
            if TRACE is not None:
                TRACE.append(ctx)
        return out

# ... 50 lines not shown
            grads[6 * l + 2] = dgamma
            grads[6 * l + 3] = dbeta
            pooled = pool and l == L - 1
            gp = gmask.data_ptr() if pooled else None
            am = argmax.data_ptr() if pooled else None
            psc = scales[l].data_ptr() if pooled else None
            psh = shifts[l].data_ptr() if pooled else None
            Gptr = None if (pooled or Gm is None) else Gm.data_ptr()

            if l == 0 and gather and virt:
                dwxyz = _f32((3, N), dev)
                dbias = _f32(N, dev) if bias is not None else None
                _lib.call("pcops_xyz_first_layer_grads", xstats.shape[0], xstats.data_ptr(), mom.shape[0], mom.data_ptr(),
                          N, wxyz.data_ptr(), _p(bias), p.data_ptr(), q.data_ptr(), t.data_ptr(), dbeta.data_ptr(),
                          means[0].data_ptr(), R, dwxyz.data_ptr(), _p(dbias))
                break
            if l == 0 and gather and getattr(ctx, "direct", False):
                B, M, _ = idx.shape
                if xstats is not None:
                    wpart, P1 = xstats, xstats.shape[0]
                else:
                    P1 = lib.pcops_edge_first_rows()
                    wpart = _f32((P1, 6, N), dev)
                    _lib.call("pcops_edge_first_wgrad", B, a0.shape[1], M, S, N, Gptr, xyz.data_ptr(), idx.data_ptr(),
                              wpart.data_ptr())
                dwxyz = _f32((6, N), dev)
                dbias = _f32(N, dev) if bias is not None else None
                _lib.call("pcops_edge_first_layer_grads", P1, wpart.data_ptr(), mom.shape[0], mom.data_ptr(), N,
                          wxyz.data_ptr(), _p(bias), p.data_ptr(), q.data_ptr(), t.data_ptr(), dbeta.data_ptr(),
                          means[0].data_ptr(), R, dwxyz.data_ptr(), _p(dbias))
                break
            if l == 0 and gather and getattr(ctx, "qc", False):
                B, M, _ = idx.shape
                Nsrc = a0.shape[1]
                d0 = _f32((B, Nsrc, 2 * N), dev)
                wsp = torch.empty(int(lib.pcops_sa_scatter_workspace_bytes(B, Nsrc, M, S)) // 4, dtype=torch.int32, device=dev)
                _lib.call("pcops_sa_scatter_bwd_ld", B, Nsrc, M, S, N, Gptr, p.data_ptr(), q.data_ptr(), t.data_ptr(),
                          idx.data_ptr(), a0.data_ptr(), 2 * N, a0.data_ptr() + 4 * N, 2 * N, d0.data_ptr(), 2 * N,
                          d0.data_ptr() + 4 * N, 2 * N, wsp.data_ptr())
                break
            if l == 0 and gather and getattr(ctx, "cloud_bias", False) and Gptr is not None:
                B, M, _ = idx.shape
                d0 = _f32((B, a0.shape[1], N), dev) if ctx.needs_input_grad[0] else None
                d1 = _f32((B, M, N), dev)
                scratch = _f32((lib.pcops_cloud_bias_rows(R), N), dev)
                _lib.call("pcops_cloud_bias_bwd", R, S, N, Gptr, Ys[0].data_ptr(), p.data_ptr(), q.data_ptr(), t.data_ptr(),
                          _p(d0), d1.data_ptr(), scratch.data_ptr())
                break
            if l == 0 and gather:
                B, M, _ = idx.shape
                Nsrc = a0.shape[1] if a0 is not None else xyz.shape[1]
                d0 = _f32((B, Nsrc, N), dev) if (a0 is not None and ctx.needs_input_grad[0]) else None
                d1 = _f32((B, M, N), dev) if ctr is not None else None
                dwxyz = _f32((3, N), dev) if wxyz is not None else None
                dbias = _f32(N, dev) if bias is not None else None
                wpart = _f32(lib.pcops_sa_scatter_rows(B, M) * 4 * N, dev) if (wxyz is not None or bias is not None) else None
                wsp = None
                d0_out = d0
                if d0 is not None and identity and not pooled:
                    if TAIL_FOLD and N % 4 == 0:
                        d0_out = _f32((B, Nsrc, N), dev)
                        _lib.call("pcops_mlp_dy_apply", B * Nsrc, N, Gm.data_ptr(), Ys[0].data_ptr(), p.data_ptr(),
                                  q.data_ptr(), t.data_ptr(), d0_out.data_ptr())
                    else:
                        d0_out = torch.addcmul(t[:N], Gm, p[:N]).addcmul_(Ys[0], q[:N]).view(B, Nsrc, N)
                    d0 = None
                if d0 is not None:
                    wsp = torch.empty(int(lib.pcops_sa_scatter_workspace_bytes(B, Nsrc, M, S)) // 4,
                                      dtype=torch.int32, device=dev)
                _lib.call("pcops_sa_scatter_bwd_rows", B, Nsrc, M, S, N, Gptr, _p(Ys[0]), p.data_ptr(),
                          q.data_ptr(), t.data_ptr(), gp, am, psc, psh, idx.data_ptr(),
                          _p(xyz) if wxyz is not None else None, _p(new_xyz) if wxyz is not None else None,
                          _p(d0), _p(d1), _p(wpart), _p(dwxyz), _p(dbias), _p(a0), _p(ctr), _p(wxyz), _p(bias),
                          _p(wsp), rref)
                d0 = d0_out
                break

            K = Ws[l].shape[0]
            xyz_prev = virt and l == 1
            if pooled and ctx.pool_top:
                prev = (Ys[l - 1], scales[l - 1], shifts[l - 1]) if l > 0 else (a0, None, None)
                Gm, part = _pool_top_backward(R, K, N, S, Ws[l], ctx.biases[l].detach(), p, q, t, grad_out, ysel,
                                              argmax, scales[l], shifts[l], prev[0], prev[1], prev[2], grads, l, dev,
                                              l > 0 or ctx.needs_input_grad[0])
                P = lib.pcops_mlp_stats_rows(R)
                if l == 0:
                    d0 = Gm
                continue
            fused_groups = 0
            if BWD_FUSED and l > 0 and Ws[l].data_ptr() % 16 == 0:
                fused_groups = lib.pcops_mlp_bwd_fused_groups(R, K, N, S if pooled else 0, 1 if pooled else 0)
            if fused_groups:
                edge_rows = getattr(ctx, "edge_rows", None) if (l == 1 and pooled and getattr(ctx, "direct", False)) else None
                if edge_rows is not None and lib.pcops_mlp_bwd_fused_edge_groups(R, K, N, S, 0) != fused_groups:
                    edge_rows = None
                gw = (pooled and rows is None and not xyz_prev and
                      (lib.pcops_mlp_bwd_fused_edge_groups(R, K, N, S, 1) if edge_rows is not None
                       else lib.pcops_mlp_bwd_fused_gw_groups(R, K, N, S)) == fused_groups)
                scratch = _f32(fused_groups * (K * N + N + ((K * K + K) if gw else 0)), dev)
                dW, db = _f32((K, N), dev), _f32(N, dev)
                P = fused_groups
                part = _f32((P, 2, K), dev)
                bl = ctx.biases[l]
                if edge_rows is not None:
                    xstats = _f32((P, 6, K), dev)
                    if gw:
                        _lib.call("pcops_mlp_bwd_fused_edge_gw", R, K, N, Ys[0].data_ptr(), scales[0].data_ptr(),
                                  shifts[0].data_ptr(), Ys[l].data_ptr(), p.data_ptr(), q.data_ptr(), t.data_ptr(), gp, am, S,
                                  Ws[l].data_ptr(), _p(bl), scratch.data_ptr(), dW.data_ptr(), db.data_ptr(), part.data_ptr(),
                                  edge_rows.data_ptr(), xstats.data_ptr())
                    else:
                        _lib.call("pcops_mlp_bwd_fused_edge", R, K, N, Ys[0].data_ptr(), scales[0].data_ptr(),
                                  shifts[0].data_ptr(), Ys[l].data_ptr(), p.data_ptr(), q.data_ptr(), t.data_ptr(), gp, am, S,
                                  Ws[l].data_ptr(), scratch.data_ptr(), dW.data_ptr(), db.data_ptr(), part.data_ptr(),
                                  edge_rows.data_ptr(), xstats.data_ptr())
                    grads[6 * l + 0] = dW
                    grads[6 * l + 1] = db
                    Gm = None
                    continue
                if gw:
                    Gprev = _f32((R, K), dev)
                    _lib.call("pcops_mlp_bwd_fused_gw", R, K, N, Ys[l - 1].data_ptr(), scales[l - 1].data_ptr(),
                              shifts[l - 1].data_ptr(), Ys[l].data_ptr(), p.data_ptr(), q.data_ptr(), t.data_ptr(),
                              gp, am, S, Ws[l].data_ptr(), _p(bl), scratch.data_ptr(), dW.data_ptr(), db.data_ptr(),
                              Gprev.data_ptr(), part.data_ptr())
                    grads[6 * l + 0] = dW
                    grads[6 * l + 1] = db
                    Gm = Gprev
                    continue
                if xyz_prev:
                    xstats = _f32((P, 3, K), dev)
                    _lib.call("pcops_mlp_bwd_fused_xyz_rows", R, K, N, off4.data_ptr(), xyzw.data_ptr(),
                              scales[0].data_ptr(), shifts[0].data_ptr(), Gptr, Ys[l].data_ptr(), p.data_ptr(),
                              q.data_ptr(), t.data_ptr(), gp, am, S, Ws[l].data_ptr(), scratch.data_ptr(),
                              dW.data_ptr(), db.data_ptr(), part.data_ptr(), xstats.data_ptr(), rref)
                    grads[6 * l + 0] = dW
                    grads[6 * l + 1] = db
                    Gm = None
                    continue
                Gprev = _f32((R, K), dev)
                _lib.call("pcops_mlp_bwd_fused_rows", R, K, N, Ys[l - 1].data_ptr(), scales[l - 1].data_ptr(),
                          shifts[l - 1].data_ptr(), Gptr, Ys[l].data_ptr(), p.data_ptr(), q.data_ptr(), t.data_ptr(),
                          gp, am, S, Ws[l].data_ptr(), scratch.data_ptr(), dW.data_ptr(), db.data_ptr(),
                          Gprev.data_ptr(), part.data_ptr(), rref)
                grads[6 * l + 0] = dW
                grads[6 * l + 1] = db
                Gm = Gprev
                continue
            if l == 0:
                src, ld, asc, ash = a0, K0, None, None
            elif not xyz_prev:
                src, ld, asc, ash = Ys[l - 1], Ys[l - 1].shape[1], scales[l - 1].data_ptr(), shifts[l - 1].data_ptr()
            splits = lib.pcops_mlp_wgrad_splits(R, K, N)
            scratch = _f32(splits * (K * N + N), dev)
            dW, db = _f32((K, N), dev), _f32(N, dev)
            if xyz_prev:
                _lib.call("pcops_mlp_wgrad_xyz_rows", R, K, N, off4.data_ptr(), xyzw.data_ptr(), scales[0].data_ptr(),
                          shifts[0].data_ptr(), Gptr, Ys[l].data_ptr(), p.data_ptr(), q.data_ptr(), t.data_ptr(), gp, am,
                          S, psc, psh, scratch.data_ptr(), dW.data_ptr(), db.data_ptr(), rref)
            else:
                _lib.call("pcops_mlp_wgrad_rows", R, K, N, src.data_ptr(), ld, asc, ash, Gptr, Ys[l].data_ptr(),
                          p.data_ptr(), q.data_ptr(), t.data_ptr(), gp, am, S, psc, psh, scratch.data_ptr(),
                          dW.data_ptr(), db.data_ptr(), rref)
            grads[6 * l + 0] = dW
            grads[6 * l + 1] = db
            if l > 0 or ctx.needs_input_grad[0]:
                Wt = _f32((N, K), dev)
                _lib.call("pcops_mlp_transpose", K, N, Ws[l].data_ptr(), Wt.data_ptr())
                Gprev = None if xyz_prev else _f32((R, K), dev)
                if xyz_prev:
                    P = lib.pcops_mlp_stats_rows(R)
                    part = _f32((P, 2, K), dev)
                    xstats = _f32((P, 3, K), dev)
                    _lib.call("pcops_mlp_gemm_dgrad_xyz_rows", R, N, K, Gptr, Ys[l].data_ptr(), p.data_ptr(), q.data_ptr(),
                              t.data_ptr(), gp, am, S, psc, psh, Wt.data_ptr(), off4.data_ptr(), xyzw.data_ptr(),
                              scales[0].data_ptr(), shifts[0].data_ptr(), None, part.data_ptr(), xstats.data_ptr(),
                              rref)
                elif l > 0:
                    P = lib.pcops_mlp_stats_rows(R)
                    part = _f32((P, 2, K), dev)
                    _lib.call("pcops_mlp_gemm_dgrad_rows", R, N, K, Gptr, Ys[l].data_ptr(), p.data_ptr(), q.data_ptr(),
                              t.data_ptr(), gp, am, S, psc, psh, Wt.data_ptr(), Ys[l - 1].data_ptr(),
                              scales[l - 1].data_ptr(), shifts[l - 1].data_ptr(), Gprev.data_ptr(),
                              part.data_ptr(), rref)
                else:
                    _lib.call("pcops_mlp_gemm_dgrad", R, N, K, Gptr, Ys[l].data_ptr(), p.data_ptr(), q.data_ptr(),
                              t.data_ptr(), gp, am, S, psc, psh, Wt.data_ptr(), None, None, None,
                              Gprev.data_ptr(), None)
                    d0 = Gprev
                Gm = Gprev

        out = [d0 if ctx.needs_input_grad[0] else None, d1, None, None, None, dwxyz, dbias,
               None, None, None, None, None, None, None, None]
        for i in range(L):
            out.extend(grads[6 * i:6 * i + 4])
            out.extend([None, None])
        return tuple(out)


def _pool_top_ok(lib, R, K, N, S, l, gather, K0, rows, xyz_prev, has_bias):
    return bool(POOL_TOP and rows is None and not xyz_prev and S >= 64 and N >= 2 * K
                and (l > 0 or (not gather and K0 == K)) and has_bias
                and lib.pcops_mlp_pool_top_supported(R, K, N, S))


def _pool_top_backward(R, K, N, S, W, b, p, q, t, grad_out, ysel, argmax, sc, sh, Yprev, psc, psh, grads, l, dev,
                       need_dx=True):
    lib = _lib.load()
    Wt = _f32((N, K), dev)
    if TAIL_FOLD:
        Wq, u = _f32((K, N), dev), _f32(N, dev)
        v = _f32(K, dev) if need_dx else None
        _lib.call("pcops_mlp_pool_top_prep", K, N, W.data_ptr(), b.data_ptr(), q.data_ptr(), t.data_ptr(), Wt.data_ptr(),
                  Wq.data_ptr(), u.data_ptr(), _p(v))
    else:
        _lib.call("pcops_mlp_transpose", K, N, W.data_ptr(), Wt.data_ptr())
        Wq = W * q[:N]
        u = torch.addcmul(t[:N], q[:N], b)
    Gprev = part = None
    splits = lib.pcops_mlp_wgrad_splits(R, K, K)
    scratch = _f32(splits * (K * K + K), dev)
    gram, xsum = _f32((K, K), dev), _f32(K, dev)
    _lib.call("pcops_mlp_gram", R, K, Yprev.data_ptr(), K, _p(psc), _p(psh), scratch.data_ptr(),
              gram.data_ptr(), xsum.data_ptr())
    dW = _f32((K, N), dev)
    paired = TAIL_FOLD and need_dx
    if paired:
        Mq = _f32((K, K), dev)
        _lib.small_gemm_pair((K, N, K, Wq.data_ptr(), N, 0, Wt.data_ptr(), K, 0, None, Mq.data_ptr(), K, None),
                             (K, K, N, gram.data_ptr(), K, 0, Wq.data_ptr(), N, 0, None, dW.data_ptr(), N, None))
    if need_dx:
        if not paired:
            Mq = _f32((K, K), dev)
            _lib.call("pcops_small_gemm", K, N, K, Wq.data_ptr(), N, Wt.data_ptr(), K, Mq.data_ptr(), K)
        if not TAIL_FOLD:
            v = _f32(K, dev)
            _lib.call("pcops_small_gemm", 1, N, K, u.data_ptr(), N, Wt.data_ptr(), K, v.data_ptr(), K)
        G = R // S
        addend = _f32((G * min(S, N), K), dev)
        rowmap = torch.empty(R, dtype=torch.int32, device=dev)
        _lib.call("pcops_mlp_pool_top_addend", R, K, N, S, grad_out.data_ptr(), ysel.data_ptr(), argmax.data_ptr(),
                  sc.data_ptr(), sh.data_ptr(), p.data_ptr(), Wt.data_ptr(), addend.data_ptr(), rowmap.data_ptr())
        Gprev = _f32((R, K), dev)
        part = _f32((lib.pcops_mlp_stats_rows(R), 2, K), dev) if psc is not None else None
        _lib.call("pcops_mlp_gemm_dgrad_top", R, K, Yprev.data_ptr(), _p(psc), _p(psh), Mq.data_ptr(),
                  v.data_ptr(), addend.data_ptr(), addend.shape[0], rowmap.data_ptr(), Gprev.data_ptr(), _p(part))
    Ssp, cfsum = _f32((K, N), dev), _f32(N, dev)
    _lib.call("pcops_mlp_pool_top_wsparse", R, K, N, S, grad_out.data_ptr(), ysel.data_ptr(), argmax.data_ptr(),
              sc.data_ptr(), sh.data_ptr(), p.data_ptr(), Yprev.data_ptr(), _p(psc), _p(psh),
              Ssp.data_ptr(), cfsum.data_ptr())
    if not paired:
        _lib.call("pcops_small_gemm", K, K, N, gram.data_ptr(), K, Wq.data_ptr(), N, dW.data_ptr(), N)
    if TAIL_FOLD:
        db = _f32(N, dev)
        _lib.call("pcops_mlp_pool_top_finish", K, N, R, dW.data_ptr(), Ssp.data_ptr(), xsum.data_ptr(), u.data_ptr(),
                  cfsum.data_ptr(), q.data_ptr(), W.data_ptr(), b.data_ptr(), t.data_ptr(), db.data_ptr())
        grads[6 * l + 0] = dW
        grads[6 * l + 1] = db
    else:
        xw = _f32(N, dev)
        _lib.call("pcops_small_gemm", 1, K, N, xsum.data_ptr(), K, W.data_ptr(), N, xw.data_ptr(), N)
        grads[6 * l + 0] = torch.addr(dW.add_(Ssp), xsum, u)
        grads[6 * l + 1] = cfsum + q[:N] * (xw + float(R) * b) + float(R) * t[:N]
    return Gprev, part


class _SmallLinear(torch.autograd.Function):

    @staticmethod
    def forward(ctx, x, w, b):
        R, K = x.shape
        N = w.shape[1]
        y = torch.empty((R, N), dtype=torch.float32, device=x.device)
        _lib.call("pcops_small_gemm_ex", R, K, N, x.data_ptr(), K, 0, w.data_ptr(), N, 0, _p(b), y.data_ptr(), N)
        ctx.save_for_backward(x, w)
        ctx.has_bias = b is not None
        return y

    @staticmethod
    @torch.autograd.function.once_differentiable
    def backward(ctx, gy):
        x, w = ctx.saved_tensors
        R, K = x.shape
        N = w.shape[1]
        gy = gy.contiguous()
        dx = dw = db = None
        want_db = ctx.has_bias and ctx.needs_input_grad[2]
        if TAIL_FOLD and ctx.needs_input_grad[0] and ctx.needs_input_grad[1]:
            dx = torch.empty((R, K), dtype=torch.float32, device=x.device)
            dw = torch.empty((K, N), dtype=torch.float32, device=x.device)
            db = torch.empty(N, dtype=torch.float32, device=x.device) if want_db else None
            _lib.small_gemm_pair((R, N, K, gy.data_ptr(), N, 0, w.data_ptr(), N, 1, None, dx.data_ptr(), K, None),
                                 (K, R, N, x.data_ptr(), K, 1, gy.data_ptr(), N, 0, None, dw.data_ptr(), N, _p(db)))
            return dx, dw, db
        if ctx.needs_input_grad[0]:
            dx = torch.empty((R, K), dtype=torch.float32, device=x.device)
            _lib.call("pcops_small_gemm_ex", R, N, K, gy.data_ptr(), N, 0, w.data_ptr(), N, 1, None, dx.data_ptr(), K)
        if ctx.needs_input_grad[1]:
            dw = torch.empty((K, N), dtype=torch.float32, device=x.device)
            if want_db and TAIL_FOLD:
                db = torch.empty(N, dtype=torch.float32, device=x.device)
            _lib.call("pcops_small_gemm_colsum", K, R, N, x.data_ptr(), K, 1, gy.data_ptr(), N, 0, None, dw.data_ptr(), N,
                      _p(db))
        if want_db and db is None:
            db = gy.sum(dim=0)
        return dx, dw, db


class _SplitRows(torch.autograd.Function):

    @staticmethod
    def forward(ctx, w, k):
        ctx.k, ctx.rows = int(k), w.shape[0]
        return w[:k], w[k:]

    @staticmethod
    def backward(ctx, ga, gb):
        k, n = ctx.k, ctx.rows
        if ga is None and gb is None:
            return None, None
        like = ga if ga is not None else gb
        if ga is None:
            ga = like.new_zeros((k,) + tuple(like.shape[1:]))
        if gb is None:
            gb = like.new_zeros((n - k,) + tuple(like.shape[1:]))
        return torch.cat([ga, gb], dim=0), None


def split_rows(w, k):
    if not TAIL_FOLD or not w.requires_grad:
        return w[:k], w[k:]
    return _SplitRows.apply(w, int(k))

# ... 291 lines not shown
        Nsrc, C = Q.shape[1], (Q.shape[2] // 2 if qc else Q.shape[2])
        dev = Q.device
        G = B * M
        P = lib.pcops_mlp_bwd_pool_stats_rows(G)
        part = _f32((P, 2, C), dev)
        if fold:
            grad_out = _f32((G, C), dev)
            gb = given[1] if len(given) == 2 else None
            _lib.call("pcops_mlp_pool_bwd_stats_sum", G, C, given[0].data_ptr(), lds_[0], _p(gb), lds_[1] if gb is not None else 0,
                      ysel.data_ptr(), scale.data_ptr(), shift.data_ptr(), part.data_ptr(), grad_out.data_ptr())
        else:
            grad_out = grad_out.contiguous()
            _lib.call("pcops_mlp_pool_bwd_stats", G, C, grad_out.data_ptr(), ysel.data_ptr(), scale.data_ptr(),
                      shift.data_ptr(), part.data_ptr(), None)
        vecs = _VecArena([C], 3, dev)
        p, q, t = vecs.take(C), vecs.take(C), vecs.take(C)
        dgamma, dbeta = _f32(C, dev), _f32(C, dev)
        ws = _workspace(C, dev)
        _lib.call("pcops_mlp_bn_bwd_coeffs", P, C, G * S, part.data_ptr(), ws.data_ptr(), gamma.data_ptr(),
                  mean.data_ptr(), rstd.data_ptr(), dgamma.data_ptr(), dbeta.data_ptr(), p.data_ptr(), q.data_ptr(),
                  t.data_ptr())
        if sync:
            gpart, Rg = _dist.allreduce_stat_partials(part, G * S)
            junk = _f32(2 * C, dev)
            _lib.call("pcops_mlp_bn_bwd_coeffs", gpart.shape[0], C, Rg, gpart.data_ptr(), ws.data_ptr(), gamma.data_ptr(),
                      mean.data_ptr(), rstd.data_ptr(), junk.data_ptr(), junk[C:].data_ptr(), p.data_ptr(),
                      q.data_ptr(), t.data_ptr())
        if not training:
            q.zero_()
            t.zero_()
        wsp = torch.empty(int(lib.pcops_sa_scatter_workspace_bytes(B, Nsrc, M, S)) // 4, dtype=torch.int32, device=dev)
        if qc:
            dQC = _f32((B, Nsrc, 2 * C), dev)
            _lib.call("pcops_edge_pool_bwd_ld", B, Nsrc, M, S, C, Q.data_ptr(), 2 * C, Q.data_ptr() + 4 * C, 2 * C,
                      idx.data_ptr(), grad_out.data_ptr(), ysel.data_ptr(), SQ.data_ptr(), arg.data_ptr(), scale.data_ptr(),
                      shift.data_ptr(), p.data_ptr(), q.data_ptr(), t.data_ptr(), dQC.data_ptr(), 2 * C,
                      dQC.data_ptr() + 4 * C, 2 * C, wsp.data_ptr())
            return dQC, None, None, dgamma, dbeta, None, None, None, None, None, None, None, None
        dQ, dCtr = _f32((B, Nsrc, C), dev), _f32((B, M, C), dev)
        _lib.call("pcops_edge_pool_bwd", B, Nsrc, M, S, C, Q.data_ptr(), Ctr.data_ptr(), idx.data_ptr(),
                  grad_out.data_ptr(), ysel.data_ptr(), SQ.data_ptr(), arg.data_ptr(), scale.data_ptr(), shift.data_ptr(),
                  p.data_ptr(), q.data_ptr(), t.data_ptr(), dQ.data_ptr(), dCtr.data_ptr(), wsp.data_ptr())
        return dQ, dCtr, None, dgamma, dbeta, None, None, None, None, None, None, None, None


def edge_conv_pool_supported(C, S):
    return C in (32, 64, 128) or C % 256 == 0 and S <= 256


def fused_supported(x, widths, bn, activation_relu):
    if not (bn and activation_relu and x.is_cuda and x.dtype == torch.float32):
        return False
    if any(w % 32 != 0 for w in widths):
        return False
    return True


def _flat(layer_tensors, first_gather):
    flat = []
    for i, (w, b, gamma, beta, mm, mv) in enumerate(layer_tensors):
        if i == 0 and first_gather:
            flat.extend([None, None, gamma, beta, mm, mv])
        else:
            flat.extend([w.reshape(-1, w.shape[-1]), b, gamma, beta, mm, mv])
    return flat


def mlp_stack(x, S, pool, training, decay, eps, unbiased, layer_tensors):
    x2d = x.reshape(-1, x.shape[-1]).contiguous()
    return FusedMLPStack.apply(x2d, None, None, None, None, None, None, int(S), bool(pool), bool(training),
                               float(decay), float(eps), bool(unbiased), None, len(layer_tensors),
                               *_flat(layer_tensors, False))


TRACE = None
STAT_PIVOT = os.environ.get("PCOPS_STAT_PIVOT", "1") != "0"
FUSE_POOL_ROWS = os.environ.get("PCOPS_FUSE_POOL_ROWS", "1") != "0"
BWD_FUSED = os.environ.get("PCOPS_BWD_FUSED", "1") != "0"
CLOUD_BIAS = os.environ.get("PCOPS_CLOUD_BIAS", "1") != "0"
CLOUD_POINT = os.environ.get("PCOPS_CLOUD_POINT", "1") != "0"
EDGE_DIRECT = os.environ.get("PCOPS_EDGE_DIRECT", "1") != "0"
EDGE_DIRECT_FUSED = os.environ.get("PCOPS_EDGE_DIRECT_FUSED", "1") != "0"
POOL_TOP = os.environ.get("PCOPS_POOL_TOP", "1") != "0"
TAIL_FOLD = os.environ.get("PCOPS_TAIL_FOLD", "1") != "0"
COMPACT_MIN_S = int(os.environ.get("PCOPS_COMPACT_MIN_S", "48"))
EDGE_QC = os.environ.get("PCOPS_EDGE_QC", "1") != "0"


def _compactable(idx, pool, L, widths, Q, Ctr, xyz, wxyz, identity_idx):
    B, M, S = idx.shape
    if not (COMPACT_MIN_S and pool and not identity_idx and Ctr is None and L >= 2 and S >= COMPACT_MIN_S):
        return False
    if B * M * S < 32768 or any(w % 32 for w in widths) or _dist.sync_bn_active():
        return False
    if Q is None and not (wxyz is not None and L >= 3):
        return False
    import ctypes
    n = Q.shape[1] if Q is not None else xyz.shape[1]
    arr = (ctypes.c_int * L)(*[int(w) for w in widths])
    return bool(_lib.load().pcops_gather_stack_rows_supported(B, n, M, S, 1 if Q is not None else 0, L, arr))


def edge_qc_supported(b, n, s, c):
    return bool(EDGE_QC and _lib.load().pcops_edge_ld_supported(int(b), int(n), int(n), int(s), int(c))
                and not _dist.sync_bn_active())


def edge_direct_supported(b, n, k, c_in, c1, n_layers, x):
    if not (EDGE_DIRECT and c_in == 3 and n_layers >= 2) or (torch.is_grad_enabled() and x.requires_grad):
        return False
    return bool(_lib.load().pcops_edge_first_supported(b, n, n, k, c1))


def gather_mlp_stack(idx, pool, training, decay, eps, unbiased, layer_tensors, Q=None, Ctr=None, xyz=None,
                     new_xyz=None, wxyz=None, bias=None, identity_idx=False, pts_cnt=None, QC=None, cat_slot=None,
                     direct=None):
    c = lambda t: t.contiguous() if t is not None else None
    S = idx.shape[2]
    if QC is not None:
        assert Q is None and Ctr is None and xyz is None and wxyz is None and bias is None
        if len(layer_tensors) == 1 and pool:
            _w, _b, gamma, beta, mm, mv = layer_tensors[0]
            if cat_slot is not None:
                return EdgeConvPool.apply(QC.contiguous(), None, idx.contiguous(), gamma, beta, mm, mv, bool(training),
                                          float(decay), float(eps), bool(unbiased), cat_slot[0], int(cat_slot[1]))
            return EdgeConvPool.apply(QC.contiguous(), None, idx.contiguous(), gamma, beta, mm, mv, bool(training),
                                      float(decay), float(eps), bool(unbiased))
        if direct is not None:
            x3, w1, b1 = direct
            assert not QC.requires_grad and not x3.requires_grad and len(layer_tensors) >= 2
            return FusedMLPStack.apply(QC.contiguous(), None, idx.contiguous(), x3.contiguous(), None, w1.contiguous(), b1,
                                       int(S), int(bool(pool)) | 4 | 8, bool(training), float(decay), float(eps),
                                       bool(unbiased), None, len(layer_tensors), *_flat(layer_tensors, True))
        return FusedMLPStack.apply(QC.contiguous(), None, idx.contiguous(), None, None, None, None, int(S),
                                   int(bool(pool)) | 4, bool(training), float(decay), float(eps), bool(unbiased), None,
                                   len(layer_tensors), *_flat(layer_tensors, True))
    if torch.is_grad_enabled() and any(t is not None and t.requires_grad for t in (xyz, new_xyz)):
        raise RuntimeError("gather_mlp_stack: xyz / new_xyz require grad; use the unfused grouped path "
                           "(pointnet_util falls back to it automatically)")
    if (len(layer_tensors) == 1 and pool and Q is not None and Ctr is not None and xyz is None and wxyz is None
            and bias is None and S <= 256 and edge_conv_pool_supported(Q.shape[-1], S)
            and 256 % (Q.shape[-1] // 4) == 0 and Q.shape[1] <= 16384):
        _w, _b, gamma, beta, mm, mv = layer_tensors[0]
        return EdgeConvPool.apply(c(Q), c(Ctr), idx.contiguous(), gamma, beta, mm, mv, bool(training), float(decay),
                                  float(eps), bool(unbiased))
    rows = None
    if pts_cnt is not None and _compactable(idx, pool, len(layer_tensors), [l[2].shape[0] for l in layer_tensors],
                                            Q, Ctr, xyz, wxyz, identity_idx):
        rows = _lib.Rows(pts_cnt.contiguous(), S)
    return FusedMLPStack.apply(c(Q), c(Ctr), idx.contiguous(), c(xyz.detach()) if xyz is not None else None,
                               c(new_xyz.detach()) if new_xyz is not None else None, c(wxyz), c(bias), int(S),
                               int(bool(pool)) | (2 if identity_idx else 0), bool(training), float(decay), float(eps),
                               bool(unbiased), rows, len(layer_tensors), *_flat(layer_tensors, True))
```

Measured before the change: 26750.

## Extend pool-top sparse backward to compacted row-block layout

Adds row-compacted variants of the pool-top backward path: addend, dgrad-top, Gram and sparse-wgrad kernels that take per-block row weights from the compact row descriptor. When that path is taken, the forward pass skips materialising the last-layer output Y. The aim is to let compacted grouped stacks use the algebraic Gram/sparse-argmax backward instead of the full dense backward. The cost is more kernel complexity, a weighted-row correction in the GEMM epilogue, and a new partial-sum workspace.

```diff
diff --git a/include/pcops.h b/include/pcops.h
--- a/include/pcops.h
+++ b/include/pcops.h
@@ -336,6 +336,23 @@
 int pcops_mlp_bn_relu_maxpool_rows(long long G, int C, const float *Y, const float *scale, const float *shift,
                                    const pcops_rows_t *rows, float *out, unsigned char *argmax, float *ysel,
                                    pcops_stream_t stream);
+int pcops_mlp_pool_top_rows_supported(int M, int Kp, int N, int S);
+unsigned long long pcops_mlp_pool_top_wsparse_rows_partial(int Kp, int N);
+int pcops_mlp_pool_top_addend_rows(int M, int Kp, int N, int S, const float *gout, const float *ysel,
+                                   const unsigned char *argmax, const float *pool_scale, const float *pool_shift,
+                                   const float *p, const float *Wt, float *addend, int *rowmap, const pcops_rows_t *rows,
+                                   pcops_stream_t stream);
+int pcops_mlp_gemm_dgrad_top_rows(int M, int Kp, const float *Yprev, const float *prev_scale, const float *prev_shift,
+                                  const float *Mq, const float *vconst, const float *addend, long long addend_rows,
+                                  const int *rowmap, float *Gprev, float *stats_partial, const pcops_rows_t *rows,
+                                  pcops_stream_t stream);
+int pcops_mlp_gram_rows(long long M, int Kp, const float *Yprev, int ldx, const float *a_scale, const float *a_shift,
+                        float *partial, float *gram, float *xsum, const pcops_rows_t *rows, pcops_stream_t stream);
+int pcops_mlp_pool_top_wsparse_rows(int M, int Kp, int N, int S, const float *gout, const float *ysel,
+                                    const unsigned char *argmax, const float *pool_scale, const float *pool_shift,
+                                    const float *p, const float *Yprev, const float *prev_scale, const float *prev_shift,
+                                    float *Ssp, float *cfsum, float *partial, const pcops_rows_t *rows,
+                                    pcops_stream_t stream);
 int pcops_sa_gather_fwd_rows(int b, int n, int m, int s, int c, const float *Q, const float *Ctr, const float *xyz,
                              const float *new_xyz, const float *Wxyz, const float *bias, const int *idx, float *Y,
                              float *off4, float *stats_partial, const float *stat_pivot, float *moments,
diff --git a/scanobjectnn_amd/_lib.py b/scanobjectnn_amd/_lib.py
--- a/scanobjectnn_amd/_lib.py
+++ b/scanobjectnn_amd/_lib.py
@@ -54,6 +54,10 @@
     "pcops_mlp_gemm_dgrad_top": ([_I, _I] + [_P] * 6 + [_LL] + [_P] * 3, True),
     "pcops_mlp_gram": ([_LL, _I, _P, _I, _P, _P, _P, _P, _P], True),
     "pcops_mlp_pool_top_wsparse": ([_I, _I, _I, _I] + [_P] * 11, True),
+    "pcops_mlp_pool_top_addend_rows": ([_I, _I, _I, _I] + [_P] * 10, True),
+    "pcops_mlp_gemm_dgrad_top_rows": ([_I, _I] + [_P] * 6 + [_LL] + [_P] * 4, True),
+    "pcops_mlp_gram_rows": ([_LL, _I, _P, _I, _P, _P, _P, _P, _P, _P], True),
+    "pcops_mlp_pool_top_wsparse_rows": ([_I, _I, _I, _I] + [_P] * 13, True),
     "pcops_sa_gather_fwd": ([_I, _I, _I, _I, _I, _P, _P, _P, _P, _P, _P, _P, _P, _P, _P, _P, _P], True),
     "pcops_mlp_gemm_fwd_xyz": ([_I, _I, _I, _P, _P, _P, _P, _P, _P, _P, _P, _P], True),
     "pcops_mlp_gemm_dgrad_xyz": ([_I, _I, _I, _P, _P, _P, _P, _P, _P, _P, _I, _P, _P, _P, _P, _P, _P, _P, _P, _P, _P], True),
@@ -148,6 +152,8 @@
     "pcops_scatter_rows_sorted_max_ndst": ([], _I),
     "pcops_scatter_rows_sorted_supported": ([_I, _I], _I),
     "pcops_mlp_pool_top_supported": ([_I, _I, _I, _I], _I),
+    "pcops_mlp_pool_top_rows_supported": ([_I, _I, _I, _I], _I),
+    "pcops_mlp_pool_top_wsparse_rows_partial": ([_I, _I], _U64),
     "pcops_knn_graph_path": ([_I, _I, _I, _I, _P], _I),
     "pcops_last_launch_pipe": ([], _I),
     "pcops_last_launch_plan": ([_P, _I], _I),
diff --git a/scanobjectnn_amd/csrc/mlp.hip b/scanobjectnn_amd/csrc/mlp.hip
--- a/scanobjectnn_amd/csrc/mlp.hip
+++ b/scanobjectnn_amd/csrc/mlp.hip
@@ -1066,7 +1066,7 @@
             const float4 epv = EM == E_FWD ? *reinterpret_cast<const float4 *>(&ecoef[2 * BN + ocq])
                                            : make_float4(0.f, 0.f, 0.f, 0.f);
             float ew[2] = {1.f, 1.f};
-            if (EM == E_FWD && compact) {
+            if ((EM == E_FWD || has_add(EM)) && compact) {
                 const int nblk = (M + kBlk - 1) / kBlk;
 #pragma unroll
                 for (int hb = 0; hb < 2; ++hb) {
@@ -1110,12 +1110,24 @@
                         }
                     } else if (EM == E_PLAINA) {
                         const float4 vc = *reinterpret_cast<const float4 *>(&ecoef[2 * BN + ocq]);
+                        if (compact && j % (O4 / 4) == 0) {
+                            const float w = lane < O4 ? ew[j / (O4 / 4)] : 1.f;
+                            o.x = w * (o.x + vc.x) + pad[j].x; o.y = w * (o.y + vc.y) + pad[j].y;
+                            o.z = w * (o.z + vc.z) + pad[j].z; o.w = w * (o.w + vc.w) + pad[j].w;
+                        } else {
                         o.x += pad[j].x + vc.x; o.y += pad[j].y + vc.y; o.z += pad[j].z + vc.z; o.w += pad[j].w + vc.w;
+                        }
                     } else if (is_mask(EM)) {
                         const float4 yp = py[j];
                         if (EM == E_MASKA) {
                             const float4 vc = *reinterpret_cast<const float4 *>(&ecoef[2 * BN + ocq]);
+                            if (compact && j % (O4 / 4) == 0) {
+                                const float w = lane < O4 ? ew[j / (O4 / 4)] : 1.f;
+                                o.x = w * (o.x + vc.x) + pad[j].x; o.y = w * (o.y + vc.y) + pad[j].y;
+                                o.z = w * (o.z + vc.z) + pad[j].z; o.w = w * (o.w + vc.w) + pad[j].w;
+                            } else {
                             o.x += pad[j].x + vc.x; o.y += pad[j].y + vc.y; o.z += pad[j].z + vc.z; o.w += pad[j].w + vc.w;
+                            }
                         }
                         o.x = fmaf(yp.x, eb.x, em.x) > 0.f ? o.x : 0.f;
                         o.y = fmaf(yp.y, eb.y, em.y) > 0.f ? o.y : 0.f;
@@ -3600,6 +3612,8 @@
     const float *X, *asc, *ash;
     float *part;
     float *xpart;
+    const RowBlock *blocks;
+    const int *Mdev;
 };
 
 constexpr int gram_blocks(int nbk) { return nbk * (nbk + 1) / 2; }
@@ -3638,7 +3652,7 @@
     (one(std::integral_constant<int, B>{}), ...);
 }
 
-template <int NBK, bool BNRELU>
+template <int NBK, bool BNRELU, bool ROWS = false>
 __global__ __launch_bounds__(512, 1) void gram_full_kernel(GramArgs a) {
     constexpr int KP = 32 * NBK, RS = 32, LD = KP + 4;
     constexpr int NU = gram_blocks(NBK), PER = (NU + 3) / 4;
@@ -3647,7 +3661,7 @@
     const int tid = threadIdx.x, lane = tid & 63;
     const int wave = __builtin_amdgcn_readfirstlane(tid >> 6);
     const int K = a.K;
-    const long long M = a.M;
+    const long long M = ROWS ? (long long)__builtin_amdgcn_readfirstlane(*a.Mdev) : a.M;
     const int grp = blockIdx.x, ngrp = gridDim.x;
     float *coef = lds;
     float *buf = coef + 2 * KP;
@@ -3676,6 +3690,16 @@
         };
         auto stage = [&](long long stripe, float *dst) {
             const long long row0 = stripe * RS;
+            float sw[2] = {1.f, 1.f};
+            if (ROWS) {
+                const long long nblk = (M + kBlk - 1) / kBlk;
+#pragma unroll
+                for (int hb = 0; hb < 2; ++hb) {
+                    long long bi = stripe * 2 + hb;
+                    bi = bi < nblk ? bi : nblk - 1;
+                    sw[hb] = sqrtf(uniform_block(a.blocks, bi).w);
+                }
+            }
 #pragma unroll
             for (int j = 0; j < NV; ++j) {
                 const int e = pt + 256 * j, r = e / K4, c = (e % K4) * 4;
@@ -3687,7 +3711,14 @@
                     x.z = fmaxf(fmaf(x.z, sc.z, sh.z), 0.f); x.w = fmaxf(fmaf(x.w, sc.w, sh.w), 0.f);
                     if (!(c < K && row0 + r < M)) x = make_float4(0.f, 0.f, 0.f, 0.f);
                 }
+                if (ROWS && (r & (kBlk - 1)) == 0) {
+                    const float w = sw[r / kBlk];
+                    x.x *= w; x.y *= w; x.z *= w; x.w *= w;
+                    cs[j][0] = fmaf(w, x.x, cs[j][0]); cs[j][1] = fmaf(w, x.y, cs[j][1]);
+                    cs[j][2] = fmaf(w, x.z, cs[j][2]); cs[j][3] = fmaf(w, x.w, cs[j][3]);
+                } else {
                 cs[j][0] += x.x; cs[j][1] += x.y; cs[j][2] += x.z; cs[j][3] += x.w;
+                }
                 *reinterpret_cast<float4 *>(&dst[r * LD + c]) = x;
             }
         };
@@ -4342,6 +4373,134 @@
         cfsum[c] = (red[0][64 * KR] + red[1][64 * KR]) + (red[2][64 * KR] + red[3][64 * KR]);
 }
 
+template <int KP>
+__global__ __launch_bounds__(1024) void pool_top_addend_rows_kernel(int G, int C, const float *__restrict__ gout,
+                                                                    const float *__restrict__ ysel,
+                                                                    const unsigned char *__restrict__ arg,
+                                                                    const float *__restrict__ sc, const float *__restrict__ sh,
+                                                                    const float *__restrict__ p, const float *__restrict__ Wt,
+                                                                    const int *__restrict__ block_start,
+                                                                    float *__restrict__ addend, int *__restrict__ rowmap) {
+    constexpr int LPR = KP / 4, RPP = 256 / LPR;
+    constexpr int MAXR = 128, MW = 8;
+    extern __shared__ __attribute__((aligned(16))) float lds[];
+    float *Ws = lds;
+    float *cf = Ws + (size_t)C * KP;
+    unsigned *mask = reinterpret_cast<unsigned *>(cf + 4 * 256);
+    const int tid = threadIdx.x, sub = tid >> 8, c = tid & 255;
+    for (int e = tid; e < C * (KP / 4); e += 1024)
+        reinterpret_cast<float4 *>(Ws)[e] = reinterpret_cast<const float4 *>(Wt)[e];
+    const float scc = c < C ? sc[c] : 0.f, shc = c < C ? sh[c] : 0.f, pc = c < C ? p[c] : 0.f;
+    float *mycf = cf + sub * 256;
+    unsigned *mymask = mask + sub * MAXR * MW;
+    const int q = c % LPR, rsub = c / LPR;
+    float v = 0.f;
+    int row = 0, base = 0, nrows = 0;
+    auto fetch = [&](long long g) {
+        v = 0.f; row = 0; base = 0; nrows = 0;
+        if (g < G) {
+            const int b0 = block_start[g];
+            base = kBlk * b0;
+            nrows = kBlk * (block_start[g + 1] - b0);
+            nrows = nrows < MAXR ? nrows : MAXR;
+            if (c < C) {
+                const long long e = g * C + c;
+                v = fmaf(ysel[e], scc, shc) > 0.f ? pc * gout[e] : 0.f;
+                row = arg[e];
+            }
+        }
+    };
+    fetch((long long)blockIdx.x * 4 + sub);
+    for (long long g0 = (long long)blockIdx.x * 4; g0 < G; g0 += (long long)gridDim.x * 4) {
+        const float cv = v;
+        const int crow = row, cbase = base, cnrows = nrows;
+        __syncthreads();
+        mycf[c] = cv;
+#pragma unroll
+        for (int i = 0; i < MAXR * MW / 256; ++i) mymask[c + 256 * i] = 0u;
+        __syncthreads();
+        if (cv != 0.f && crow < cnrows) atomicOr(&mymask[crow * MW + (c >> 5)], 1u << (c & 31));
+        __syncthreads();
+        fetch(g0 + (long long)gridDim.x * 4 + sub);
+        for (int r = rsub; r < cnrows; r += RPP) {
+            float4 acc = make_float4(0.f, 0.f, 0.f, 0.f);
+            bool any = false;
+#pragma unroll
+            for (int w = 0; w < MW; ++w) {
+                unsigned mm = mymask[r * MW + w];
+                any = any || mm != 0u;
+                while (mm) {
+                    const int ch = 32 * w + __builtin_ctz(mm);
+                    mm &= mm - 1u;
+                    const float cw = mycf[ch];
+                    const float4 wt = *reinterpret_cast<const float4 *>(&Ws[ch * KP + 4 * q]);
+                    acc.x = fmaf(cw, wt.x, acc.x); acc.y = fmaf(cw, wt.y, acc.y);
+                    acc.z = fmaf(cw, wt.z, acc.z); acc.w = fmaf(cw, wt.w, acc.w);
+                }
+            }
+            const long long ri = (long long)cbase + r;
+            if (any) *reinterpret_cast<float4 *>(&addend[ri * KP + 4 * q]) = acc;
+            if (q == 0) rowmap[ri] = any ? (int)ri : -1;
+        }
+    }
+}
+
+template <int KP>
+__global__ __launch_bounds__(256) void pool_top_wsparse_rows_kernel(int G, int C, int maxr, const float *__restrict__ gout,
+                                                                    const float *__restrict__ ysel,
+                                                                    const unsigned char *__restrict__ arg,
+                                                                    const float *__restrict__ sc, const float *__restrict__ sh,
+                                                                    const float *__restrict__ p,
+                                                                    const float *__restrict__ Yprev,
+                                                                    const float *__restrict__ psc, const float *__restrict__ psh,
+                                                                    const int *__restrict__ block_start,
+                                                                    float *__restrict__ part, float *__restrict__ part2) {
+    constexpr int LD = KP + 1, K4 = KP / 4;
+    extern __shared__ __attribute__((aligned(16))) float lds[];
+    float *Xs = lds;
+    const int tid = threadIdx.x, c = tid;
+    const float scc = c < C ? sc[c] : 0.f, shc = c < C ? sh[c] : 0.f, pc = c < C ? p[c] : 0.f;
+    const int k4 = tid % K4, r0 = tid / K4;
+    const float4 asc = *reinterpret_cast<const float4 *>(psc + 4 * k4), ash = *reinterpret_cast<const float4 *>(psh + 4 * k4);
+    float acc[KP];
+#pragma unroll
+    for (int k = 0; k < KP; ++k) acc[k] = 0.f;
+    float csum = 0.f;
+    for (int g = blockIdx.x; g < G; g += gridDim.x) {
+        const int b0 = block_start[g];
+        int nrows = kBlk * (block_start[g + 1] - b0);
+        nrows = nrows < maxr ? nrows : maxr;
+        const float *src = Yprev + (long long)kBlk * b0 * KP;
+        float cfv = 0.f;
+        int row = 0;
+        if (c < C) {
+            const long long e = (long long)g * C + c;
+            cfv = fmaf(ysel[e], scc, shc) > 0.f ? pc * gout[e] : 0.f;
+            row = arg[e];
+            if (row >= nrows) { row = 0; cfv = 0.f; }
+        }
+        __syncthreads();
+        for (int r = r0; r < nrows; r += 256 / K4) {
+            float4 x = *reinterpret_cast<const float4 *>(src + (long long)r * KP + 4 * k4);
+            x.x = fmaxf(fmaf(x.x, asc.x, ash.x), 0.f); x.y = fmaxf(fmaf(x.y, asc.y, ash.y), 0.f);
+            x.z = fmaxf(fmaf(x.z, asc.z, ash.z), 0.f); x.w = fmaxf(fmaf(x.w, asc.w, ash.w), 0.f);
+            float *d = &Xs[r * LD + 4 * k4];
+            d[0] = x.x; d[1] = x.y; d[2] = x.z; d[3] = x.w;
+        }
+        __syncthreads();
+        const float *xr = &Xs[row * LD];
+#pragma unroll
+        for (int k = 0; k < KP; ++k) acc[k] = fmaf(cfv, xr[k], acc[k]);
+        csum += cfv;
+    }
+    if (c < C) {
+        float *dst = part + (long long)blockIdx.x * KP * C + c;
+#pragma unroll
+        for (int k = 0; k < KP; ++k) dst[(long long)k * C] = acc[k];
+        part2[(long long)blockIdx.x * C + c] = csum;
+    }
+}
+
 __device__ __forceinline__ void small_gemm_tile(int bx, int by, int M, int K, int N, const float *__restrict__ A, int lda,
                                                          const float *__restrict__ B, int ldb, float *__restrict__ C,
                                                          int ldc, int transA, int transB, const float *__restrict__ bias,
@@ -4444,6 +4603,7 @@
 PCOPS_HIDDEN int bwd_fused_launch(WgradArgs &a, bool xyz, int groups, float *partial, float *dW, float *db, hipStream_t st,
                                   bool side = false, const float *gw_bias = nullptr);
 PCOPS_HIDDEN int gram_full_launch(GramArgs &g, int nbk, bool bnrelu, int gg, size_t lds, hipStream_t st);
+PCOPS_HIDDEN int gram_full_rows_launch(GramArgs &g, int nbk, int gg, size_t lds, hipStream_t st);
 
 static int wgrad_legacy_splits(long long M, int K, int N) {
     const int kb = (K + 63) / 64, nb = (N + 127) / 128;
@@ -4731,6 +4891,16 @@
 #undef PCOPS_GRAM_LAUNCH
     return PCOPS_OK;
 }
+
+int gram_full_rows_launch(GramArgs &g, int nbk, int gg, size_t lds, hipStream_t st) {
+    auto kern = nbk == 2 ? gram_full_kernel<2, true, true> : gram_full_kernel<4, true, true>;
+    if (nbk != 2 && nbk != 4) return PCOPS_ERR_UNSUPPORTED;
+    if (hipFuncSetAttribute(reinterpret_cast<const void *>(kern), hipFuncAttributeMaxDynamicSharedMemorySize, 160 * 1024) !=
+        hipSuccess)
+        return PCOPS_ERR_LAUNCH;
+    hipLaunchKernelGGL(kern, dim3(gg), dim3(512), lds, st, g);
+    return PCOPS_OK;
+}
 #endif
 
 #if PCOPS_PART(0)
@@ -4851,7 +5021,7 @@
                                  float *Y, float *stats_partial, const float *stat_pivot, float *ypart,
                                  unsigned char *ppart, const pcops_rows_t *rows, pcops_stream_t stream) {
     PCOPS_REQUIRE_SHAPE(M >= 1 && K >= 1 && N >= 1 && ldx >= K);
-    PCOPS_REQUIRE_PTR(X); PCOPS_REQUIRE_PTR(W); PCOPS_REQUIRE_PTR(Y); PCOPS_REQUIRE_PTR(pro_scale);
+    PCOPS_REQUIRE_PTR(X); PCOPS_REQUIRE_PTR(W); PCOPS_REQUIRE_PTR(pro_scale);
     PCOPS_REQUIRE_PTR(pro_shift); PCOPS_REQUIRE_PTR(gamma); PCOPS_REQUIRE_PTR(ypart); PCOPS_REQUIRE_PTR(ppart);
     PCOPS_REQUIRE_PTR(rows);
     if (ldx != K || (reinterpret_cast<uintptr_t>(ypart) & 15) || (reinterpret_cast<uintptr_t>(ppart) & 3))
@@ -5494,23 +5664,8 @@
 int pcops_mlp_gemm_dgrad_top(int M, int Kp, const float *Yprev, const float *prev_scale, const float *prev_shift,
                              const float *Mq, const float *vconst, const float *addend, long long addend_rows,
                              const int *rowmap, float *Gprev, float *stats_partial, pcops_stream_t stream) {
-    PCOPS_REQUIRE_SHAPE(M >= 1 && Kp >= 1);
-    PCOPS_REQUIRE_PTR(Yprev); PCOPS_REQUIRE_PTR(Mq);
-    PCOPS_REQUIRE_PTR(vconst); PCOPS_REQUIRE_PTR(addend); PCOPS_REQUIRE_PTR(rowmap); PCOPS_REQUIRE_PTR(Gprev);
-    PCOPS_REQUIRE_ARG((prev_scale == nullptr) == (prev_shift == nullptr));
-    WsPlan pl;
-    if (!dgrad_top_plan(M, Kp, &pl)) return PCOPS_ERR_UNSUPPORTED;
-    GemmArgs a = {};
-    a.M = M; a.K = Kp; a.N = Kp; a.X = Yprev; a.ldx = Kp; a.v0 = prev_scale; a.v1 = prev_shift;
-    a.W = Mq; a.Y = Gprev; a.ldy = Kp; a.Yprev = Yprev; a.msc = prev_scale; a.msh = prev_shift;
-    a.stats = stats_partial; a.addend = addend; a.rowmap = rowmap; a.add_ld = Kp; a.vconst = vconst;
-    a.add_bytes = addend_rows * Kp * 4;
-    if (addend_rows < 1 || a.add_bytes >= (long long)kOOB) return PCOPS_ERR_UNSUPPORTED;
-    if (!prev_scale) {
-        a.stats = nullptr;
-        return launch_gemm_ws_only<A_PLAIN, E_PLAINA>(a, as_stream(stream));
-    }
-    return launch_gemm_ws_only<A_BNRELU, E_MASKA>(a, as_stream(stream));
+    return pcops_mlp_gemm_dgrad_top_rows(M, Kp, Yprev, prev_scale, prev_shift, Mq, vconst, addend, addend_rows, rowmap, Gprev,
+                                         stats_partial, nullptr, stream);
 }
 
 int pcops_mlp_gram(long long M, int Kp, const float *Yprev, int ldx, const float *a_scale, const float *a_shift,
@@ -5558,6 +5713,141 @@
     return pcops_launch_status();
 }
 
+
+static const int kTopRowsWs = 512;
+
+int pcops_mlp_pool_top_rows_supported(int M, int Kp, int N, int S) {
+    if (!pcops_mlp_pool_top_supported(M, Kp, N, S)) return 0;
+    if (M < 65536 || S % kBlk != 0 || S > 128 || (Kp != 64 && Kp != 128) || N > 256 || N % 32 != 0) return 0;
+    if (!gram_full_groups(M, Kp, Kp, nullptr)) return 0;
+    return (long long)M * Kp * 4 < (long long)kOOB ? 1 : 0;
+}
+
+unsigned long long pcops_mlp_pool_top_wsparse_rows_partial(int Kp, int N) {
+    return (unsigned long long)kTopRowsWs * ((unsigned long long)Kp * N + N);
+}
+
+int pcops_mlp_pool_top_addend_rows(int M, int Kp, int N, int S, const float *gout, const float *ysel,
+                                   const unsigned char *argmax, const float *pool_scale, const float *pool_shift,
+                                   const float *p, const float *Wt, float *addend, int *rowmap, const pcops_rows_t *rows,
+                                   pcops_stream_t stream) {
+    if (!rows) return pcops_mlp_pool_top_addend(M, Kp, N, S, gout, ysel, argmax, pool_scale, pool_shift, p, Wt, addend, rowmap, stream);
+    PCOPS_REQUIRE_SHAPE(M >= 1 && S >= 1 && M % S == 0);
+    PCOPS_REQUIRE_PTR(gout); PCOPS_REQUIRE_PTR(ysel); PCOPS_REQUIRE_PTR(argmax); PCOPS_REQUIRE_PTR(pool_scale);
+    PCOPS_REQUIRE_PTR(pool_shift); PCOPS_REQUIRE_PTR(p); PCOPS_REQUIRE_PTR(Wt); PCOPS_REQUIRE_PTR(addend);
+    PCOPS_REQUIRE_PTR(rowmap);
+    { const int rrc = rows_ok(rows); if (rrc) return rrc; }
+    if (!pcops_mlp_pool_top_rows_supported(M, Kp, N, S)) return PCOPS_ERR_UNSUPPORTED;
+    if (reinterpret_cast<uintptr_t>(Wt) & 15 || reinterpret_cast<uintptr_t>(addend) & 15) return PCOPS_ERR_UNSUPPORTED;
+    const int G = M / S;
+    const size_t lds = ((size_t)N * Kp + 4 * 256 + 4 * 128 * 8) * sizeof(float);
+    const int grid = (G + 3) / 4 < 256 ? (G + 3) / 4 : 256;
+    hipStream_t st = as_stream(stream);
+#define PCOPS_ADDR_LAUNCH(KP_)                                                                              \
+    do {                                                                                                    \
+        auto kern = pool_top_addend_rows_kernel<KP_>;                                                       \
+        if (hipFuncSetAttribute(reinterpret_cast<const void *>(kern), hipFuncAttributeMaxDynamicSharedMemorySize, \
+                                160 * 1024) != hipSuccess)                                                  \
+            return PCOPS_ERR_LAUNCH;                                                                        \
+        hipLaunchKernelGGL(kern, dim3(grid), dim3(1024), lds, st, G, N, gout, ysel, argmax, pool_scale, pool_shift, p, \
+                           Wt, rows->block_start, addend, rowmap);                                          \
+    } while (0)
+    if (Kp == 64) PCOPS_ADDR_LAUNCH(64);
+    else PCOPS_ADDR_LAUNCH(128);
+#undef PCOPS_ADDR_LAUNCH
+    return pcops_launch_status();
+}
+
+int pcops_mlp_pool_top_wsparse_rows(int M, int Kp, int N, int S, const float *gout, const float *ysel,
+                                    const unsigned char *argmax, const float *pool_scale, const float *pool_shift,
+                                    const float *p, const float *Yprev, const float *prev_scale, const float *prev_shift,
+                                    float *Ssp, float *cfsum, float *partial, const pcops_rows_t *rows,
+                                    pcops_stream_t stream) {
+    if (!rows) return pcops_mlp_pool_top_wsparse(M, Kp, N, S, gout, ysel, argmax, pool_scale, pool_shift, p, Yprev, prev_scale, prev_shift, Ssp, cfsum, stream);
+    PCOPS_REQUIRE_SHAPE(M >= 1 && S >= 1 && M % S == 0);
+    PCOPS_REQUIRE_PTR(gout); PCOPS_REQUIRE_PTR(ysel); PCOPS_REQUIRE_PTR(argmax); PCOPS_REQUIRE_PTR(pool_scale);
+    PCOPS_REQUIRE_PTR(pool_shift); PCOPS_REQUIRE_PTR(p); PCOPS_REQUIRE_PTR(Yprev); PCOPS_REQUIRE_PTR(prev_scale);
+    PCOPS_REQUIRE_PTR(prev_shift); PCOPS_REQUIRE_PTR(Ssp); PCOPS_REQUIRE_PTR(cfsum); PCOPS_REQUIRE_PTR(partial);
+    { const int rrc = rows_ok(rows); if (rrc) return rrc; }
+    if (!pcops_mlp_pool_top_rows_supported(M, Kp, N, S)) return PCOPS_ERR_UNSUPPORTED;
+    if (reinterpret_cast<uintptr_t>(Yprev) & 15 || reinterpret_cast<uintptr_t>(prev_scale) & 15 ||
+        reinterpret_cast<uintptr_t>(prev_shift) & 15)
+        return PCOPS_ERR_UNSUPPORTED;
+    const int G = M / S;
+    const int grid = G < kTopRowsWs ? G : kTopRowsWs;
+    const size_t lds = (size_t)S * (Kp + 1) * sizeof(float);
+    float *part2 = partial + (long long)kTopRowsWs * Kp * N;
+    hipStream_t st = as_stream(stream);
+#define PCOPS_WSPR_LAUNCH(KP_)                                                                              \
+    do {                                                                                                    \
+        auto kern = pool_top_wsparse_rows_kernel<KP_>;                                                      \
+        if (hipFuncSetAttribute(reinterpret_cast<const void *>(kern), hipFuncAttributeMaxDynamicSharedMemorySize, \
+                                160 * 1024) != hipSuccess)                                                  \
+            return PCOPS_ERR_LAUNCH;                                                                        \
+        hipLaunchKernelGGL(kern, dim3(grid), dim3(256), lds, st, G, N, S, gout, ysel, argmax, pool_scale, pool_shift, p, \
+                           Yprev, prev_scale, prev_shift, rows->block_start, partial, part2);               \
+    } while (0)
+    if (Kp == 64) PCOPS_WSPR_LAUNCH(64);
+    else PCOPS_WSPR_LAUNCH(128);
+#undef PCOPS_WSPR_LAUNCH
+    int rc = pcops_launch_status();
+    if (rc) return rc;
+    const long long L = (long long)Kp * N;
+    hipLaunchKernelGGL(sum_partials2_kernel, dim3(cdiv(L, 64) + cdiv(N, 64)), dim3(1024), 0, st, grid, L, partial, Ssp,
+                       (long long)N, part2, cfsum);
+    return pcops_launch_status();
+}
+
+int pcops_mlp_gemm_dgrad_top_rows(int M, int Kp, const float *Yprev, const float *prev_scale, const float *prev_shift,
+                                  const float *Mq, const float *vconst, const float *addend, long long addend_rows,
+                                  const int *rowmap, float *Gprev, float *stats_partial, const pcops_rows_t *rows,
+                                  pcops_stream_t stream) {
+    PCOPS_REQUIRE_SHAPE(M >= 1 && Kp >= 1);
+    PCOPS_REQUIRE_PTR(Yprev); PCOPS_REQUIRE_PTR(Mq);
+    PCOPS_REQUIRE_PTR(vconst); PCOPS_REQUIRE_PTR(addend); PCOPS_REQUIRE_PTR(rowmap); PCOPS_REQUIRE_PTR(Gprev);
+    PCOPS_REQUIRE_ARG((prev_scale == nullptr) == (prev_shift == nullptr));
+    WsPlan pl;
+    if (!dgrad_top_plan(M, Kp, &pl)) return PCOPS_ERR_UNSUPPORTED;
+    GemmArgs a = {};
+    a.M = M; a.K = Kp; a.N = Kp; a.X = Yprev; a.ldx = Kp; a.v0 = prev_scale; a.v1 = prev_shift;
+    a.W = Mq; a.Y = Gprev; a.ldy = Kp; a.Yprev = Yprev; a.msc = prev_scale; a.msh = prev_shift;
+    a.stats = stats_partial; a.addend = addend; a.rowmap = rowmap; a.add_ld = Kp; a.vconst = vconst;
+    a.add_bytes = addend_rows * Kp * 4;
+    if (addend_rows < 1 || a.add_bytes >= (long long)kOOB) return PCOPS_ERR_UNSUPPORTED;
+    PCOPS_ROWS(a, rows);
+    if (!prev_scale) {
+        a.stats = nullptr;
+        return launch_gemm_ws_only<A_PLAIN, E_PLAINA>(a, as_stream(stream));
+    }
+    return launch_gemm_ws_only<A_BNRELU, E_MASKA>(a, as_stream(stream));
+}
+
+int pcops_mlp_gram_rows(long long M, int Kp, const float *Yprev, int ldx, const float *a_scale, const float *a_shift,
+                        float *partial, float *gram, float *xsum, const pcops_rows_t *rows, pcops_stream_t stream) {
+    if (!rows) return pcops_mlp_gram(M, Kp, Yprev, ldx, a_scale, a_shift, partial, gram, xsum, stream);
+    PCOPS_REQUIRE_SHAPE(M >= 1 && Kp >= 1 && ldx >= Kp);
+    PCOPS_REQUIRE_PTR(Yprev); PCOPS_REQUIRE_PTR(partial); PCOPS_REQUIRE_PTR(gram); PCOPS_REQUIRE_PTR(a_scale);
+    PCOPS_REQUIRE_PTR(a_shift);
+    { const int rrc = rows_ok(rows); if (rrc) return rrc; }
+    const int gg = gram_full_groups(M, Kp, ldx, Yprev);
+    if (gg <= 0 || (Kp != 64 && Kp != 128)) return PCOPS_ERR_UNSUPPORTED;
+    pcops_note_pipe(0);
+    hipStream_t st = as_stream(stream);
+    GramArgs g = {M, Kp, ldx, Yprev, a_scale, a_shift, partial, partial + (long long)gg * Kp * Kp,
+                  static_cast<const RowBlock *>(rows->blocks), rows->rows};
+    const int nbk = Kp / 32;
+    const size_t lds = (size_t)(2 * 32 * nbk + 2 * 32 * (32 * nbk + 4)) * sizeof(float);
+    const int rcl = gram_full_rows_launch(g, nbk, gg, lds, st);
+    if (rcl) return rcl;
+    int rc = pcops_launch_status();
+    if (rc) return rc;
+    const long long L = (long long)Kp * Kp;
+    hipLaunchKernelGGL(sum_partials2_kernel, dim3(cdiv(L, 64) + (xsum ? cdiv(Kp, 64) : 0)), dim3(1024), 0, st, gg, L,
+                       partial, gram, (long long)Kp, g.xpart, xsum);
+    hipLaunchKernelGGL(mirror_lower_kernel, dim3(Kp), dim3(256), 0, st, Kp, gram);
+    return pcops_launch_status();
+}
+
 int pcops_mlp_dy_apply(long long M, int N, const float *G, const float *Y, const float *p, const float *q, const float *t,
                        float *out, pcops_stream_t stream) {
     PCOPS_REQUIRE_SHAPE(M >= 0 && N >= 4 && N % 4 == 0);
diff --git a/scanobjectnn_amd/fused_mlp.py b/scanobjectnn_amd/fused_mlp.py
--- a/scanobjectnn_amd/fused_mlp.py
+++ b/scanobjectnn_amd/fused_mlp.py
@@ -121,18 +121,22 @@
                 N = w.shape[-1]
                 W2 = w.detach().reshape(-1, N)
                 assert W2.shape[0] == K and W2.is_contiguous()
-                Y = _f32((R, N), dev)
+                pool_rows = (rows is not None and pool and li == L - 1 and sc_prev is not None and ld == K
+                             and not (li == 1 and virt) and FUSE_POOL_ROWS
+                             and bool(lib.pcops_mlp_gemm_fwd_pool_rows_supported(R, K, N)))
+                if pool_rows:
+                    pool_top = need_grad and _pool_top_ok(lib, R, K, N, S, li, gather, K0, rows, False, b is not None)
+                Y = None if (pool_rows and pool_top) else _f32((R, N), dev)
                 P = lib.pcops_mlp_stats_rows(R)
                 part = _f32((P, 2, N), dev) if training else None
                 if li == 1 and virt:
                     _lib.call("pcops_mlp_gemm_fwd_xyz_rows", R, K, N, off4.data_ptr(), xyzw.data_ptr(), sc_prev.data_ptr(),
                               sh_prev.data_ptr(), W2.data_ptr(), b.data_ptr(), Y.data_ptr(), _p(part), piv, rref)
-                elif (rows is not None and pool and li == L - 1 and sc_prev is not None and ld == K and FUSE_POOL_ROWS
-                        and lib.pcops_mlp_gemm_fwd_pool_rows_supported(R, K, N)):
+                elif pool_rows:
                     nbk = rows.blocks.shape[0]
                     pooled_parts = (_f32((nbk, N), dev), torch.empty((nbk, N), dtype=torch.uint8, device=dev))
                     _lib.call("pcops_mlp_gemm_fwd_pool_rows", R, K, N, src.data_ptr(), ld, sc_prev.data_ptr(),
-                              sh_prev.data_ptr(), W2.data_ptr(), b.data_ptr(), gamma.data_ptr(), Y.data_ptr(),
+                              sh_prev.data_ptr(), W2.data_ptr(), b.data_ptr(), gamma.data_ptr(), _p(Y),
                               _p(part), piv, pooled_parts[0].data_ptr(), pooled_parts[1].data_ptr(), rref)
                 elif rows is not None:
                     _lib.call("pcops_mlp_gemm_fwd_rows", R, K, N, src.data_ptr(), ld, _p(sc_prev), _p(sh_prev),
@@ -349,7 +353,7 @@
                 prev = (Ys[l - 1], scales[l - 1], shifts[l - 1]) if l > 0 else (a0, None, None)
                 Gm, part = _pool_top_backward(R, K, N, S, Ws[l], ctx.biases[l].detach(), p, q, t, grad_out, ysel,
                                               argmax, scales[l], shifts[l], prev[0], prev[1], prev[2], grads, l, dev,
-                                              l > 0 or ctx.needs_input_grad[0])
+                                              l > 0 or ctx.needs_input_grad[0], rows)
                 P = lib.pcops_mlp_stats_rows(R)
                 if l == 0:
                     d0 = Gm
@@ -466,14 +470,19 @@
 
 
 def _pool_top_ok(lib, R, K, N, S, l, gather, K0, rows, xyz_prev, has_bias):
-    return bool(POOL_TOP and rows is None and not xyz_prev and S >= 64 and N >= 2 * K
+    if rows is not None:
+        return bool(POOL_TOP and POOL_TOP_ROWS and not xyz_prev and S >= 64 and N >= 2 * K and l > 0 and has_bias
+                    and not (BWD_FUSED and lib.pcops_mlp_bwd_fused_groups(R, K, N, S, 1))
+                    and lib.pcops_mlp_pool_top_rows_supported(R, K, N, S))
+    return bool(POOL_TOP and not xyz_prev and S >= 64 and N >= 2 * K
                 and (l > 0 or (not gather and K0 == K)) and has_bias
                 and lib.pcops_mlp_pool_top_supported(R, K, N, S))
 
 
 def _pool_top_backward(R, K, N, S, W, b, p, q, t, grad_out, ysel, argmax, sc, sh, Yprev, psc, psh, grads, l, dev,
-                       need_dx=True):
+                       need_dx=True, rows=None):
     lib = _lib.load()
+    rref = rows.ref if rows is not None else None
     Wt = _f32((N, K), dev)
     if TAIL_FOLD:
         Wq, u = _f32((K, N), dev), _f32(N, dev)
@@ -488,8 +497,12 @@
     splits = lib.pcops_mlp_wgrad_splits(R, K, K)
     scratch = _f32(splits * (K * K + K), dev)
     gram, xsum = _f32((K, K), dev), _f32(K, dev)
-    _lib.call("pcops_mlp_gram", R, K, Yprev.data_ptr(), K, _p(psc), _p(psh), scratch.data_ptr(),
-              gram.data_ptr(), xsum.data_ptr())
+    if rows is not None:
+        _lib.call("pcops_mlp_gram_rows", R, K, Yprev.data_ptr(), K, _p(psc), _p(psh), scratch.data_ptr(),
+                  gram.data_ptr(), xsum.data_ptr(), rref)
+    else:
+        _lib.call("pcops_mlp_gram", R, K, Yprev.data_ptr(), K, _p(psc), _p(psh), scratch.data_ptr(),
+                  gram.data_ptr(), xsum.data_ptr())
     dW = _f32((K, N), dev)
     paired = TAIL_FOLD and need_dx
     if paired:
@@ -504,18 +517,32 @@
             v = _f32(K, dev)
             _lib.call("pcops_small_gemm", 1, N, K, u.data_ptr(), N, Wt.data_ptr(), K, v.data_ptr(), K)
         G = R // S
-        addend = _f32((G * min(S, N), K), dev)
+        addend = _f32((R if rows is not None else G * min(S, N), K), dev)
         rowmap = torch.empty(R, dtype=torch.int32, device=dev)
-        _lib.call("pcops_mlp_pool_top_addend", R, K, N, S, grad_out.data_ptr(), ysel.data_ptr(), argmax.data_ptr(),
-                  sc.data_ptr(), sh.data_ptr(), p.data_ptr(), Wt.data_ptr(), addend.data_ptr(), rowmap.data_ptr())
         Gprev = _f32((R, K), dev)
         part = _f32((lib.pcops_mlp_stats_rows(R), 2, K), dev) if psc is not None else None
-        _lib.call("pcops_mlp_gemm_dgrad_top", R, K, Yprev.data_ptr(), _p(psc), _p(psh), Mq.data_ptr(),
-                  v.data_ptr(), addend.data_ptr(), addend.shape[0], rowmap.data_ptr(), Gprev.data_ptr(), _p(part))
+        if rows is not None:
+            _lib.call("pcops_mlp_pool_top_addend_rows", R, K, N, S, grad_out.data_ptr(), ysel.data_ptr(),
+                      argmax.data_ptr(), sc.data_ptr(), sh.data_ptr(), p.data_ptr(), Wt.data_ptr(), addend.data_ptr(),
+                      rowmap.data_ptr(), rref)
+            _lib.call("pcops_mlp_gemm_dgrad_top_rows", R, K, Yprev.data_ptr(), _p(psc), _p(psh), Mq.data_ptr(),
+                      v.data_ptr(), addend.data_ptr(), addend.shape[0], rowmap.data_ptr(), Gprev.data_ptr(), _p(part),
+                      rref)
+        else:
+            _lib.call("pcops_mlp_pool_top_addend", R, K, N, S, grad_out.data_ptr(), ysel.data_ptr(), argmax.data_ptr(),
+                      sc.data_ptr(), sh.data_ptr(), p.data_ptr(), Wt.data_ptr(), addend.data_ptr(), rowmap.data_ptr())
+            _lib.call("pcops_mlp_gemm_dgrad_top", R, K, Yprev.data_ptr(), _p(psc), _p(psh), Mq.data_ptr(),
+                      v.data_ptr(), addend.data_ptr(), addend.shape[0], rowmap.data_ptr(), Gprev.data_ptr(), _p(part))
     Ssp, cfsum = _f32((K, N), dev), _f32(N, dev)
-    _lib.call("pcops_mlp_pool_top_wsparse", R, K, N, S, grad_out.data_ptr(), ysel.data_ptr(), argmax.data_ptr(),
-              sc.data_ptr(), sh.data_ptr(), p.data_ptr(), Yprev.data_ptr(), _p(psc), _p(psh),
-              Ssp.data_ptr(), cfsum.data_ptr())
+    if rows is not None:
+        wpart = _f32(int(lib.pcops_mlp_pool_top_wsparse_rows_partial(K, N)), dev)
+        _lib.call("pcops_mlp_pool_top_wsparse_rows", R, K, N, S, grad_out.data_ptr(), ysel.data_ptr(), argmax.data_ptr(),
+                  sc.data_ptr(), sh.data_ptr(), p.data_ptr(), Yprev.data_ptr(), _p(psc), _p(psh),
+                  Ssp.data_ptr(), cfsum.data_ptr(), wpart.data_ptr(), rref)
+    else:
+        _lib.call("pcops_mlp_pool_top_wsparse", R, K, N, S, grad_out.data_ptr(), ysel.data_ptr(), argmax.data_ptr(),
+                  sc.data_ptr(), sh.data_ptr(), p.data_ptr(), Yprev.data_ptr(), _p(psc), _p(psh),
+                  Ssp.data_ptr(), cfsum.data_ptr())
     if not paired:
         _lib.call("pcops_small_gemm", K, K, N, gram.data_ptr(), K, Wq.data_ptr(), N, dW.data_ptr(), N)
     if TAIL_FOLD:
@@ -973,6 +1000,7 @@
 EDGE_DIRECT = os.environ.get("PCOPS_EDGE_DIRECT", "1") != "0"
 EDGE_DIRECT_FUSED = os.environ.get("PCOPS_EDGE_DIRECT_FUSED", "1") != "0"
 POOL_TOP = os.environ.get("PCOPS_POOL_TOP", "1") != "0"
+POOL_TOP_ROWS = os.environ.get("PCOPS_POOL_TOP_ROWS", "1") != "0"
 TAIL_FOLD = os.environ.get("PCOPS_TAIL_FOLD", "1") != "0"
 COMPACT_MIN_S = int(os.environ.get("PCOPS_COMPACT_MIN_S", "48"))
 EDGE_QC = os.environ.get("PCOPS_EDGE_QC", "1") != "0"
```

Result: faster. 27460, median of 6 (+2.6%).
